# phaistos-networks/Trinity

Hardware: AMD Instinct MI355X
Metric: queries/sec (higher is better)
Workload: dtype u32

## Files before the change

### trinity_amd/csrc/codec_streams.hpp

```cpp
#pragma once
#include "dev_stream.hpp"

constexpr int CODEC_GOOGLE = TRI_CODEC_GOOGLE;
constexpr int CODEC_LUCENE = TRI_CODEC_LUCENE;


__device__ __forceinline__ uint32_t ld32u(const uint8_t *p) {
        const uint32_t *q = (const uint32_t *)((uintptr_t)p & ~(uintptr_t)3);
        return __builtin_amdgcn_alignbyte(q[1], q[0], (uint32_t)((uintptr_t)p & 3u));
}

struct LValStream {
        const uint8_t *wp;
        const uint8_t *epos;
        const uint8_t *ehigh;
        uint64_t win;
        uint32_t width, mask, bitpos, k;
        uint32_t nexc, eb, ecur, next_j, j, sub;
        uint32_t equal_v;
        int mode;
        VbStream vb;

        __device__ __forceinline__ void init_group(const uint8_t *__restrict__ index, const uint32_t group_off, const uint32_t quarter) {
                const uint8_t *g = index + group_off;
                const uint32_t L = g[0];
                j = 0;
                sub = quarter;
                if (!L) {
                        mode = 1;
                        uint32_t len;
                        const uint64_t w = (uint64_t)ld32u(g + 1) | ((uint64_t)ld32u(g + 5) << 32);
                        equal_v = vb_decode(w, len);
                        return;
                }
                mode = 0;
                const uint32_t w0 = ld32u(g + 1);
                width = w0 & 0xffu;
                nexc = (w0 >> 8) & 0xffu;
                eb = (w0 >> 16) & 0xffu;
                mask = width >= 32 ? 0xffffffffu : ((1u << width) - 1u);
                wp = g + 1 + 4 * (1 + quarter * width);
                epos = g + 1 + 4 * (1 + 4 * width);
                ehigh = epos + 4 * ((nexc + 3) / 4);
                bitpos = 0;
                k = 2;
                win = width ? ((uint64_t)ld32u(wp) | ((uint64_t)ld32u(wp + 4) << 32)) : 0;
                ecur = 0;
                while (ecur < nexc && (uint32_t)(epos[ecur] >> 5) < quarter)
                        ++ecur;
                next_j = (ecur < nexc && (uint32_t)(epos[ecur] >> 5) == quarter) ? (epos[ecur] & 31u) : 255u;
        }
        __device__ __forceinline__ void init_tail(const uint8_t *__restrict__ index, const uint32_t off, const bool freqs) {
                mode = freqs ? 3 : 2;
                vb.init(index + off);
        }
        __device__ __forceinline__ uint32_t next() {
                if (mode == 1)
                        return equal_v;
                if (mode == 2) {
                        const uint32_t d = vb.next();
                        (void)vb.next();
                        return d;
                }
                if (mode == 3) {
                        (void)vb.next();
                        return vb.next();
                }
                uint32_t v = 0;
                if (width) {
                        const uint32_t sh = bitpos & 31u;
                        v = (uint32_t)(win >> sh) & mask;
                        const uint32_t nb = bitpos + width;
                        if ((nb >> 5) != (bitpos >> 5)) {
                                win = (win >> 32) | ((uint64_t)ld32u(wp + 4 * k) << 32);
                                ++k;
                        }
                        bitpos = nb;
                }
                if (j == next_j) {
                        const uint32_t eo = ecur * eb;
                        const uint64_t hw = (uint64_t)ld32u(ehigh + 4 * (eo >> 5)) | ((uint64_t)ld32u(ehigh + 4 * (eo >> 5) + 4) << 32);
                        const uint32_t high = (uint32_t)(hw >> (eo & 31u)) & (eb >= 32 ? 0xffffffffu : ((1u << eb) - 1u));
                        v |= width >= 32 ? 0u : (high << width);
                        ++ecur;
                        next_j = (ecur < nexc && (uint32_t)(epos[ecur] >> 5) == sub) ? (epos[ecur] & 31u) : 255u;
                }
                ++j;
                return v;
        }
};

__device__ __forceinline__ uint32_t lucene_group_bytes(const uint8_t *g) {
        const uint32_t L = g[0];
        if (L)
                return 1 + 4 * L;
        const uint32_t b0 = g[1];
        return 1 + (b0 < 0x80 ? 1 : b0 < 0xc0 ? 2 : b0 < 0xe0 ? 3 : b0 < 0xf0 ? 4 : 5);
}

template <int CODEC>
struct DeltaStream;
template <int CODEC>
struct FreqStream;

template <>
struct DeltaStream<CODEC_GOOGLE> {
        VbStream s;
        __device__ __forceinline__ void init(const uint8_t *__restrict__ index, const DevTerm &, const uint32_t, const uint32_t off) { s.init(index + off); }
        __device__ __forceinline__ uint32_t next() { return s.next(); }
};
template <>
struct FreqStream<CODEC_GOOGLE> {
        VbStream s;
        __device__ __forceinline__ void init(const uint8_t *__restrict__, const DevTerm &, const uint32_t, const uint32_t, const DeltaStream<CODEC_GOOGLE> &after_deltas) {
                s = after_deltas.s;
        }
        __device__ __forceinline__ uint32_t next() { return s.next(); }
};

template <>
struct DeltaStream<CODEC_LUCENE> {
        LValStream s;
        __device__ __forceinline__ void init(const uint8_t *__restrict__ index, const DevTerm &t, const uint32_t b, const uint32_t off) {
                if (b < t.npfor)
                        s.init_group(index, off, b & 3u);
                else
                        s.init_tail(index, off, false);
        }
        __device__ __forceinline__ uint32_t next() { return s.next(); }
};
template <>
struct FreqStream<CODEC_LUCENE> {
        LValStream s;
        __device__ __forceinline__ void init(const uint8_t *__restrict__ index, const DevTerm &t, const uint32_t b, const uint32_t off, const DeltaStream<CODEC_LUCENE> &) {
                if (b < t.npfor)
                        s.init_group(index, off + lucene_group_bytes(index + off), b & 3u);
                else
                        s.init_tail(index, off, true);
        }
        __device__ __forceinline__ uint32_t next() { return s.next(); }
};
```

### trinity_amd/csrc/dev_structs.hpp

```cpp
#pragma once
#include <cstdint>
#ifdef __HIPCC__
#define TRI_HD __host__ __device__
#else
#define TRI_HD
#endif

struct DevTerm {
        uint32_t documents;
        uint32_t first_block;
        uint32_t nblocks;
        uint32_t last_n;
        uint32_t win_off;
        uint32_t flags;
        uint32_t npfor;
        uint32_t pad;
};
constexpr uint32_t TERM_FULL_BLOCKS = 1u;
constexpr uint32_t TERM_SPARSE = 2u;

#define TRI_BLOCK_N(t, b, index, off) (((t).flags & TERM_FULL_BLOCKS) ? ((b) + 1 == (t).nblocks ? (t).last_n : 32u) : (uint32_t)(index)[(off)-1])
constexpr uint32_t WIN_MIN_BLOCKS = 128;

constexpr uint32_t QT_GROUP = 0x80000000u;
constexpr uint32_t QT_NOT = 0x40000000u;
constexpr uint32_t QT_TERM = 0x3fffffffu;
constexpr uint32_t MAX_QTERMS = 16;
struct DevQuery {
        uint32_t nterms;
        uint32_t term_base;
        uint64_t out_off;
        uint32_t out_cap;
        uint32_t qid;
        uint32_t first_task, ntasks;
        uint32_t score_base, nscore;
        uint32_t phrase_base, nphrases;
        uint32_t fused_idx, form;
};

constexpr uint32_t RESULT_DOCIDS = 0, RESULT_BITMAP = 1;
constexpr uint32_t MAX_PHRASE_TERMS = 16;
struct DevPhrase {
        uint32_t term_base;
        uint32_t nterms;
        double weight;
};

struct DevTask {
        uint32_t slot;
        uint32_t tile_begin;
        uint32_t tile_end;
        uint32_t kind;
        uint64_t out_off;
};
constexpr uint32_t CAND_QUEUES = 8;
constexpr uint32_t CAND_TICKET_STRIDE = 16;
constexpr uint32_t CAND_HEAVY_TILES = 3;
constexpr uint32_t TASK_CAND = 0;
constexpr uint32_t TASK_DENSE = 1;
constexpr uint32_t TASK_FUSED = 2;
constexpr uint32_t TASK_FUSED16 = 3;

constexpr uint32_t TASK_FUSED_GEN = 4;
constexpr uint32_t TASK_PLANES = 5;
constexpr uint32_t TASK_PLANES8 = 6;
constexpr uint32_t TASK_PSET = 7;
constexpr uint32_t TASK_PROBE = 8;
constexpr uint32_t TASK_TREE = 9;
constexpr uint32_t TASK_KINDS = 10;
constexpr uint32_t PSET_INLINE_TERMS = 4;
#ifndef TRI_PSET_TASK_WINDOWS
#define TRI_PSET_TASK_WINDOWS 4
#endif
constexpr uint32_t PSET_TASK_WINDOWS = TRI_PSET_TASK_WINDOWS;
struct DevPsetUnit {
        uint64_t out_off;
        uint32_t w_begin, w_end;
        uint32_t tix;
        uint32_t nterms;
        uint32_t term_base;
        uint32_t first;
        uint32_t tt[PSET_INLINE_TERMS];
        uint32_t row[PSET_INLINE_TERMS];
};
static_assert(sizeof(DevPsetUnit) == 64, "one cache-line half per unit");
constexpr uint32_t PSET_UNIT_FIRST = 1u, PSET_UNIT_BITMAP = 2u;
constexpr uint32_t PSET_UNIT_ROUND_SHIFT = 4, PSET_UNIT_ROUND_MASK = 15u;
constexpr uint32_t PSET_ROUND_DOCS = 16384, PSET_STAGE_DOCS = 1024;
constexpr uint32_t PSET_UNIT_SCATTER = 4u;
constexpr uint32_t TREE_MAX_NODES = 64;
constexpr uint32_t TREE_HDR_WORDS = 8;
constexpr uint32_t TREE_CHUNK_WORDS = 2048;
constexpr uint32_t TREE_ROW_PHRASE = 0x80000000u;
struct DevTreeNode {
        uint8_t op;
        uint8_t parent;
        uint8_t ord;
        uint8_t thr;
        uint32_t arg;
        uint32_t row;
        uint32_t score;
        uint32_t rmask;
        uint8_t kid0, kid1, pad0, pad1;
        uint64_t kids;
};
static_assert(sizeof(DevTreeNode) == 32, "eight words per node");
constexpr uint32_t TREE_WIDE_MAX_NODES = 1024;
constexpr uint32_t TREE_WIDE_STACK = 64;
constexpr uint32_t TREE_KIND_WIDE = 1;
constexpr uint32_t TREE_NO_PARENT = 0xffffu;
struct DevTreeNodeW {
        uint8_t op;
        uint8_t cbits;
        uint16_t parent;
        uint32_t arg, row, score, rmask;
        uint16_t ord;
        uint16_t nkids;
        uint16_t thr;
        uint8_t pop;
        uint8_t pcbits;
        uint32_t pad;
};
static_assert(sizeof(DevTreeNodeW) == sizeof(DevTreeNode), "a wide record's nodes are eight words each too");
constexpr uint32_t RICH_NARROW_TERMS = 16, RICH_WIDE_TERMS = 64;
struct DevRichWide {
        uint64_t cells;
        uint64_t slots;
        uint32_t stride, pad;
};
static_assert(sizeof(DevRichWide) == 24, "three 8-byte words per plan slot");
TRI_HD constexpr uint32_t tree_counter_planes(const uint32_t nkids) {
        uint32_t b = 0;
        while ((1u << b) <= nkids)
                ++b;
        return b;
}
TRI_HD constexpr bool task_onepass(const uint32_t kind) { return kind >= TASK_FUSED && kind <= TASK_PLANES8; }

constexpr uint32_t PL_W = 32768;
constexpr uint32_t PL_WORDS = PL_W / 32;
constexpr uint32_t PL_NONE = 0xffffffffu;
constexpr uint32_t PL_NESTED = 6;
constexpr uint32_t PL_LEVEL_WORDS = 3;
constexpr uint32_t PL_STORED = 4;
constexpr uint32_t PL_PLANES = PL_STORED + PL_LEVEL_WORDS;
constexpr uint32_t PL_HI = PL_PLANES - 1;
constexpr uint32_t PL_HI_LEVELS = PL_STORED - 1;
constexpr uint32_t PL_RANK_WORDS = 16;
constexpr uint32_t PL_RANK_DOCS = 256;
constexpr uint32_t BLK_HITS_PLAIN = 0x80000000u;
constexpr int TILE_BLOCKS = 256;
constexpr int TILE_CANDS = TILE_BLOCKS * 32;
constexpr uint32_t SPAN_BITS = 1u << 17;
constexpr uint32_t SPAN_WORDS = SPAN_BITS / 32;
constexpr uint32_t CELL_LOG2 = 10;
constexpr uint32_t CELL_DOCS = 1u << CELL_LOG2;
constexpr uint32_t CELLS_PER_SPAN = SPAN_BITS / CELL_DOCS;
#ifndef TRI_FUS_CELLS
#define TRI_FUS_CELLS 14
#endif
constexpr uint32_t FUS_CELLS = TRI_FUS_CELLS;
constexpr uint32_t FUS_W = FUS_CELLS * CELL_DOCS;
constexpr uint32_t PLK_MAX_SPARSE = 6;
constexpr uint32_t PLK_NS_SMALL = 5;
constexpr uint32_t TOPK_MAX = 256;
constexpr uint32_t FUS_MAX_SLOTS = 8;
constexpr uint32_t FUS_MAX_LEAVES = 16;
struct DevFused {
        uint32_t nslots;
        uint32_t fbits;
        uint32_t cap;
        uint32_t nreq;
        uint32_t term[FUS_MAX_SLOTS];
        uint32_t gmask[FUS_MAX_SLOTS];
        uint32_t gslots[FUS_MAX_SLOTS];
        uint32_t nmask;
        uint32_t hw;
        uint32_t mode;
        uint32_t nleaf;
        uint32_t tt[8];
        uint8_t leaf_slot[FUS_MAX_LEAVES];
        uint32_t ctt[FUS_MAX_LEAVES][8];
        uint32_t plane[FUS_MAX_SLOTS];
        uint32_t negslots;
};
constexpr uint32_t FUS_MODE_TT = 1;
constexpr uint32_t FUS_MODE_EMIT = 2;
```

### trinity_amd/csrc/host/plan_host.cpp

```cpp
#include "../planner.hpp"
#include "../lucene_enc_units.hpp"
#include "lucene_encoder.hpp"

#include <cstdlib>
#include <memory>
#include <mutex>

namespace {
        struct HostPlan {
                BatchPlan P;
                uint8_t *block = nullptr;
                ~HostPlan() { free(block); }
        };
        void put_err(char *err, size_t cap, const std::string &s) {
                if (err && cap) {
                        const size_t n = std::min(cap - 1, s.size());
                        memcpy(err, s.data(), n);
                        err[n] = 0;
                }
        }
}

extern "C" {
void *tri_host_index_build(const uint8_t *index, uint64_t len, const uint8_t *hits, uint64_t hits_len, int codec, const uint32_t *terms3, uint64_t nterms,
                           uint32_t docs_cnt, char *err, uint64_t errcap) {
        auto H = std::make_unique<HostIndex>();
        std::string e;
        static_assert(sizeof(tri_term) == 12, "tri_term is three u32");
        if (build_host_index(index, len, hits, hits_len, codec, reinterpret_cast<const tri_term *>(terms3), nterms, docs_cnt, *H, e) != TRI_OK) {
                put_err(err, errcap, e);
                return nullptr;
        }
        return H.release();
}
void tri_host_index_free(void *h) { delete static_cast<HostIndex *>(h); }

void *tri_host_plan(void *hindex, const uint32_t *prog, uint64_t prog_len, const uint32_t *queries2, uint64_t nq, uint32_t flags, uint32_t topk, int similarity,
                    unsigned threads, const char *const *opt_names, const uint64_t *opt_values, unsigned nopt, uint32_t cus, char *err, uint64_t errcap) {
        const HostIndex &H = *static_cast<HostIndex *>(hindex);
        PlanEnv env;
        env.cus = cus ? cus : 256;
        bool use_frag_cache = false;
        for (unsigned i = 0; i < nopt; ++i) {
                const std::string n = opt_names[i];
                if (n == "frag_cache") {
                        use_frag_cache = opt_values[i] != 0;
                        continue;
                }
                tri_options &o = env.opt;
                uint64_t *slot = n == "dense_min_postings" ? &o.dense_min_postings : n == "dense_task_cost" ? &o.dense_task_cost : n == "fused" ? &o.fused
                                 : n == "fused_task_cost" ? &o.fused_task_cost : n == "fused_freq_cap" ? &o.fused_freq_cap : n == "fused_halfwords" ? &o.fused_halfwords
                                 : n == "account_needed_bytes" ? &o.account_needed_bytes : n == "planes" ? &o.planes : n == "planes_split" ? &o.planes_split
                                 : n == "plane_div" ? &o.plane_div : n == "plane_max_bytes" ? &o.plane_max_bytes : n == "probe_max_blocks" ? &o.probe_max_blocks : n == "tree_max_bytes" ? &o.tree_max_bytes : n == "tree_max_nodes" ? &o.tree_max_nodes : n == "tree_wide_min_nodes" ? &o.tree_wide_min_nodes : n == "result_bitmaps" ? &o.result_bitmaps : n == "cand_task_cost" ? &o.cand_task_cost : n == "dense_window_cost" ? &o.dense_window_cost
                                 : n == "cand_xcd" ? &o.cand_xcd : n == "planes_order" ? &o.planes_order : n == "pset_order" ? &o.pset_order : n == "scatter_bitmap_slack" ? &o.scatter_bitmap_slack : n == "phrase_task_div" ? &o.phrase_task_div : n == "plane_amortize" ? &o.plane_amortize : n == "rich_max_terms" ? &o.rich_max_terms : nullptr;
                if (!slot) {
                        put_err(err, errcap, "unknown option " + n);
                        return nullptr;
                }
                *slot = opt_values[i];
        }
        PlanInput in;
        in.prog = prog;
        in.prog_len = prog_len;
        static_assert(sizeof(tri_query) == 8, "tri_query is two u32");
        in.queries = reinterpret_cast<const tri_query *>(queries2);
        in.nq = nq;
        in.flags = flags;
        in.topk = topk;
        in.similarity = similarity;
        auto hp = std::make_unique<HostPlan>();
        std::unique_ptr<HostPool> pool;
        if (threads > 1)
                pool = std::make_unique<HostPool>(threads);
        std::string e;
        static trip::FragCache g_frag_cache;
        static std::mutex g_frag_mu;
        std::unique_lock<std::mutex> frag_lock(g_frag_mu, std::defer_lock);
        if (use_frag_cache)
                frag_lock.lock();
        const int rc = plan_batch(
                H, env, in, pool.get(),
                [&](size_t bytes) {
                        hp->block = static_cast<uint8_t *>(aligned_alloc(64, (bytes + 63) & ~(size_t)63));
                        if (hp->block)
                                memset(hp->block, 0, bytes);
                        return hp->block;
                },
                hp->P, e, use_frag_cache ? &g_frag_cache : nullptr);
        if (rc != TRI_OK) {
                put_err(err, errcap, e);
                return nullptr;
        }
        return hp.release();
}
void tri_host_plan_free(void *p) { delete static_cast<HostPlan *>(p); }

void tri_host_plan_summary(void *p, uint64_t *out , double *ms ) {
        const BatchPlan &P = static_cast<HostPlan *>(p)->P;
        const uint64_t v[] = {P.block_bytes,       P.plan.size(),    P.qterms.size(),      P.tasks.size(),  P.fused.size(),       P.qplane.size(),    P.plane_terms.size(), P.sterms.size(),
                              P.sweights.size(),   P.phrases.size(), P.pterms.size(),      P.ptasks.size(), P.plan.off,           P.qterms.off,       P.tasks.off,          P.sched.off,
                              P.fused.off,         P.qplane.off,     P.plane_terms.off,    P.sterms.off,    P.sweights.off,       P.phrases.off,      P.pterms.off,         P.ptasks.off,
                              P.n_dense,           P.n_cand,         P.n_fused,            P.n_fused16,     P.n_fusedgen,         P.n_planes,         P.n_planes8,          P.plw,
                              P.sparse_cap,        P.out_capacity,   P.term_bytes,         P.term_bytes_dense, P.dense_queries,   P.cand_queries,     P.fused_queries,      P.planes_queries,
                              P.unsupported_queries, P.rich_R,       sizeof(DevQuery),     sizeof(DevTask), sizeof(DevFused),     sizeof(DevPhrase),  P.cand_needed_term_bytes, P.plane_decoded_bytes,
                              P.n_pset,            P.pset_queries,   P.n_probe,            P.probe_queries, P.units.size(),       P.units.off,        P.pset_sched.off,     sizeof(DevPsetUnit),
                              P.n_tree,            P.tree_queries,   P.tree.size(),        P.tree.off,      P.tree_terms.size(),  P.tree_terms.off,   P.tree_hidden.size(), P.tree_hidden.off,
                              P.cand_q.off};
        static_assert(sizeof v / sizeof v[0] == 65, "summary layout");
        memcpy(out, v, sizeof v);
        if (ms)
                memcpy(ms, P.plan_ms, sizeof P.plan_ms);
}
void tri_host_plan_rich_wide(void *p, uint64_t *out ) {
        const BatchPlan &P = static_cast<HostPlan *>(p)->P;
        const uint64_t v[] = {P.rich_wide.size(), P.rich_wide.off, P.rich_sched.off, P.n_rich_wide, P.rich_wide_cells, P.rich_wide_slots, sizeof(DevRichWide)};
        memcpy(out, v, sizeof v);
}
void tri_host_plan_last_unsupported(void *p, char *out, uint64_t cap) { put_err(out, cap, static_cast<HostPlan *>(p)->P.last_unsupported); }
const uint8_t *tri_host_plan_block(void *p) { return static_cast<HostPlan *>(p)->P.block; }
void tri_host_plan_query_maps(void *p, uint32_t *slot_of_query, int32_t *qstatus) {
        const BatchPlan &P = static_cast<HostPlan *>(p)->P;
        memcpy(slot_of_query, P.slot_of_query.data(), P.slot_of_query.size() * 4);
        memcpy(qstatus, P.qstatus.data(), P.qstatus.size() * 4);
}
}

extern "C" {
int tri_host_lucene_encode(const uint32_t *docs, const uint32_t *freqs, const uint16_t *pos, const uint64_t *term_first, uint64_t nterms, uint8_t *index_out, uint64_t icap,
                           uint64_t *ilen, uint8_t *hits_out, uint64_t hcap, uint64_t *hlen, uint32_t *terms3) {
        using namespace trinity_amd::Codecs;
        Lucene::IndexSession sess;
        Lucene::Encoder enc(&sess);
        uint64_t h = 0;
        for (uint64_t t = 0; t < nterms; ++t) {
                enc.begin_term();
                for (uint64_t p = term_first[t]; p < term_first[t + 1]; ++p) {
                        enc.begin_document(docs[p]);
                        for (uint32_t i = 0; i < freqs[p]; ++i)
                                enc.new_hit(pos[h++]);
                        enc.end_document();
                }
                trinity_amd::term_index_ctx tctx;
                enc.end_term(&tctx);
                terms3[3 * t] = tctx.documents, terms3[3 * t + 1] = tctx.offset, terms3[3 * t + 2] = tctx.size;
        }
        *ilen = sess.indexOut.size(), *hlen = sess.positionsOut.size();
        if (*ilen > icap || *hlen > hcap)
                return -1;
        if (*ilen)
                memcpy(index_out, sess.indexOut.data(), *ilen);
        if (*hlen)
                memcpy(hits_out, sess.positionsOut.data(), *hlen);
        return 0;
}
int tri_host_lucene_encode_units(const uint32_t *docs, const uint32_t *freqs, const uint16_t *pos, const uint64_t *term_first, uint64_t nterms, uint8_t *index_out, uint64_t icap,
                                 uint64_t *ilen, uint8_t *hits_out, uint64_t hcap, uint64_t *hlen, uint32_t *terms3) {
        const uint64_t np = term_first[nterms];
        std::vector<uint64_t> hit_off(np + 1, 0), dblk_first(nterms + 1, 0), hblk_first(nterms + 1, 0);
        for (uint64_t p = 0; p < np; ++p)
                hit_off[p + 1] = hit_off[p] + freqs[p];
        for (uint64_t t = 0; t < nterms; ++t) {
                dblk_first[t + 1] = dblk_first[t] + (term_first[t + 1] - term_first[t]) / LENC_BLOCK;
                hblk_first[t + 1] = hblk_first[t] + (hit_off[term_first[t + 1]] - hit_off[term_first[t]]) / LENC_BLOCK;
        }
        std::vector<uint32_t> hdelta(hit_off[np] + 1);
        LencArgs a{docs, freqs, pos, hit_off.data(), term_first, hdelta.data(), dblk_first.data(), hblk_first.data(), nterms};
        for (uint64_t p = 0; p < np; ++p)
                lenc_unit_hdelta(a, p, hdelta.data());
        const uint64_t nd = dblk_first[nterms], nh = hblk_first[nterms];
        std::vector<uint64_t> doff(nd + 1, 0), hoff(nh + 1, 0), term_off(nterms + 1, 0), hterm_off(nterms + 1, 0);
        std::vector<uint32_t> tail_d(nterms + 1), tail_h(nterms + 1);
        for (uint64_t g = 0; g < nd; ++g)
                doff[g + 1] = doff[g] + lenc_unit_dblk_size(a, g);
        for (uint64_t h = 0; h < nh; ++h)
                hoff[h + 1] = hoff[h] + lenc_unit_hblk_size(a, h);
        for (uint64_t t = 0; t < nterms; ++t)
                lenc_unit_tail_size(a, t, &tail_d[t], &tail_h[t]);
        LencPlace pl{doff.data(), hoff.data(), term_off.data(), hterm_off.data(), tail_d.data(), tail_h.data()};
        for (uint64_t t = 0; t < nterms; ++t) {
                term_off[t + 1] = term_off[t] + lenc_term_index_size(a, pl, t);
                hterm_off[t + 1] = hterm_off[t] + lenc_term_hits_size(a, pl, t);
        }
        *ilen = term_off[nterms], *hlen = hterm_off[nterms];
        if (*ilen > icap || *hlen > hcap)
                return -1;
        for (uint64_t g = 0; g < nd; ++g)
                lenc_unit_dblk_write(a, pl, g, index_out);
        for (uint64_t h = 0; h < nh; ++h)
                lenc_unit_hblk_write(a, pl, h, hits_out);
        for (uint64_t t = 0; t < nterms; ++t) {
                lenc_unit_term_write(a, pl, t, index_out, hits_out);
                terms3[3 * t] = (uint32_t)(term_first[t + 1] - term_first[t]), terms3[3 * t + 1] = (uint32_t)term_off[t], terms3[3 * t + 2] = lenc_term_index_size(a, pl, t);
        }
        return 0;
}
}

extern "C" {
void tri_host_pfor128_group(const uint32_t *v, uint8_t *a, uint32_t *alen, uint8_t *b, uint32_t *blen) {
        auto get = [&](uint32_t i) { return v[i]; };
        const Pfor128Plan p = pfor128_plan(get);
        uint8_t *e = pfor128_emit(get, p, a);
        *alen = (uint32_t)(e - a);
        if ((uint32_t)(e - a) != p.bytes)
                *alen = 0xffffffffu;
        std::vector<uint8_t> o;
        trinity_amd::Codecs::Lucene::ints_encode(v, o);
        memcpy(b, o.data(), o.size());
        *blen = (uint32_t)o.size();
}
uint32_t tri_host_fastpfor_encode(const uint32_t *v, uint32_t *out) {
        std::vector<uint32_t> w;
        trif::fastpfor_encode(v, w);
        memcpy(out, w.data(), w.size() * 4);
        return (uint32_t)w.size();
}
int tri_host_fastpfor_decode(const uint32_t *w, uint32_t L, uint32_t *v) { return trif::fastpfor_decode(w, L, v) ? 1 : 0; }
uint32_t tri_host_pool_cpus(uint32_t threads, int32_t *out, uint32_t cap) {
        HostPool pool(threads);
        const std::vector<int> &c = pool.pinned_cpus();
        for (size_t i = 0; i < c.size() && i < cap; ++i)
                out[i] = c[i];
        return (uint32_t)c.size();
}

uint32_t tri_host_cpu_budget() { return host_cpu_budget(); }

void tri_host_index_facts(void *h, uint64_t *info6, uint32_t *per_term3) {
        const HostIndex &H = *static_cast<HostIndex *>(h);
        info6[0] = H.info.postings, info6[1] = H.info.blocks, info6[2] = H.info.doc_bytes, info6[3] = H.info.hit_bytes, info6[4] = H.transcoded_groups, info6[5] = H.dev_index.size();
        for (size_t t = 0; t < H.terms.size(); ++t) {
                per_term3[3 * t] = H.terms[t].documents;
                per_term3[3 * t + 1] = H.terms[t].nblocks;
                per_term3[3 * t + 2] = H.terms[t].nblocks ? H.blk_last[H.terms[t].first_block + H.terms[t].nblocks - 1] : 0;
        }
}
}
```

### trinity_amd/csrc/k_match.hpp

```cpp
#pragma once
#include "codec_streams.hpp"

constexpr int AND_WG = 256;
constexpr int DENSE_WG = 512;
static_assert(TILE_BLOCKS == AND_WG, "the candidate kernel maps one 32-candidate row to each of its 256 lanes");

__device__ __forceinline__ uint32_t uni(uint32_t v) { return (uint32_t)__builtin_amdgcn_readfirstlane((int)v); }
#include "k_filter.hpp"

__device__ __forceinline__ uint32_t phys(uint32_t j) { return (j & ~31u) | ((j + (j >> 5)) & 31u); }

__device__ __forceinline__ uint32_t wave_excl_scan(uint32_t v, uint32_t &total) {
        uint32_t x = v;
        asm volatile("s_nop 1\n\t"
                     "v_add_u32_dpp %0, %0, %0 row_shr:1 row_mask:0xf bank_mask:0xf bound_ctrl:1\n\t"
                     "s_nop 1\n\t"
                     "v_add_u32_dpp %0, %0, %0 row_shr:2 row_mask:0xf bank_mask:0xf bound_ctrl:1\n\t"
                     "s_nop 1\n\t"
                     "v_add_u32_dpp %0, %0, %0 row_shr:4 row_mask:0xf bank_mask:0xf bound_ctrl:1\n\t"
                     "s_nop 1\n\t"
                     "v_add_u32_dpp %0, %0, %0 row_shr:8 row_mask:0xf bank_mask:0xf bound_ctrl:1\n\t"
                     "s_nop 1\n\t"
                     "v_add_u32_dpp %0, %0, %0 row_bcast:15 row_mask:0xa bank_mask:0xf\n\t"
                     "s_nop 1\n\t"
// ... 37 lines not shown
        uint32_t seg_tt[MAX_QTERMS];
        uint32_t seg_wlo[MAX_QTERMS];
        uint32_t seg_whi[MAX_QTERMS];
        uint32_t seg_plane[MAX_QTERMS];
        uint32_t nslow;
};
constexpr uint32_t DENSE_SLOW_CAP = DENSE_WG / 4;

template <int WG = AND_WG>
__device__ uint32_t wg_lower_bound(uint32_t *scan, const uint32_t *__restrict__ a, const uint32_t n, const uint32_t key) {
        const uint32_t tid = threadIdx.x;
        uint32_t lo = 0, hi = n;
        while (hi > lo) {
                const uint32_t len = hi - lo;
                const uint32_t step = (len + WG - 1) / WG;
                const uint32_t pos = lo + (tid + 1) * step - 1;
                const bool ge = pos >= hi ? true : a[pos] >= key;
                const uint64_t m = __ballot(ge);
                scan[tid >> 6] = m ? (tid & ~63u) + (uint32_t)__builtin_ctzll(m) : 0xffffffffu;
                __syncthreads();
                uint32_t first = 0xffffffffu;
#pragma unroll
                for (int wv = 0; wv < WG / 64; ++wv)
                        first = min(first, scan[wv]);
                first = uni(first);
                __syncthreads();
                if (first == 0xffffffffu)
                        return hi;
                const uint32_t nlo = lo + first * step;
                const uint32_t nhi = min(hi, lo + (first + 1) * step - 1);
                lo = nlo;
                hi = step == 1 ? nlo : nhi;
        }
        return lo;
}

typedef uint32_t u32x4_a4 __attribute__((ext_vector_type(4), aligned(4)));
__device__ __forceinline__ void block_bytes32_issue(const uint8_t *__restrict__ p, uint32_t (&r)[9]) {
        const uint8_t *q = p - ((uintptr_t)p & 3u);
        const u32x4_a4 A = *(const u32x4_a4 *)q, B = *(const u32x4_a4 *)(q + 16);
        r[0] = A.x, r[1] = A.y, r[2] = A.z, r[3] = A.w, r[4] = B.x, r[5] = B.y, r[6] = B.z, r[7] = B.w;
        r[8] = *(const uint32_t *)(q + 32);
}
__device__ __forceinline__ bool block_bytes32_finish(const uint8_t *__restrict__ p, const uint32_t (&r)[9], uint32_t (&v)[8]) {
        const uint32_t sk = (uint32_t)((uintptr_t)p & 3u);
#pragma unroll
        for (int i = 0; i < 8; ++i)
                v[i] = __builtin_amdgcn_alignbyte(r[i + 1], r[i], sk);
        return ((v[0] | v[1] | v[2] | v[3] | v[4] | v[5] | v[6] | (v[7] & 0x00ffffffu)) & 0x80808080u) == 0;
}
__device__ __forceinline__ bool load_block_bytes32(const uint8_t *__restrict__ p, uint32_t (&v)[8]) {
        uint32_t r[9];
        block_bytes32_issue(p, r);
        return block_bytes32_finish(p, r, v);
}

__device__ __forceinline__ uint32_t cand_gallop(const AndShared &sh, uint32_t ptr, const uint32_t C, const uint32_t doc) {
        uint32_t step = 1, lo = ptr;
        while (lo + step <= C && sh.cand[phys(lo + step - 1)] < doc) {
                lo += step;
                step <<= 1;
        }
        uint32_t hi = min(lo + step - 1, C);
        while (lo < hi) {
                const uint32_t mid = (lo + hi) >> 1;
                if (sh.cand[phys(mid)] < doc)
                        lo = mid + 1;
                else
                        hi = mid;
        }
        return lo;
}

template <int CODEC, bool PRE>
__device__ __forceinline__ void merge_block(AndShared &sh, const uint8_t *__restrict__ index, const DevTerm &t, const uint32_t b, const uint32_t off,
                                            const uint32_t n, const uint32_t prev, const uint32_t last, uint32_t ptr, uint32_t cv, const uint32_t C,
                                            const uint32_t (&raw)[9]) {
        uint32_t doc = prev;
        uint32_t v[8];
        if (CODEC == CODEC_GOOGLE && n == 32 && (PRE ? block_bytes32_finish(index + off, raw, v) : load_block_bytes32(index + off, v))) {
                uint32_t c[8];
#pragma unroll
                for (int i = 0; i < 8; ++i)
                        c[i] = ptr + i < C ? sh.cand[phys(ptr + i)] : 0xffffffffu;
                if (c[7] > last) {
                        uint32_t at = ptr;
#pragma unroll
                        for (int j = 0; j < 32; ++j) {
                                doc = j < 31 ? doc + ((v[j >> 2] >> ((j & 3) * 8)) & 0xffu) : last;
                                while (c[0] <= doc) {
                                        if (c[0] == doc)
                                                atomicOr(&sh.hit[at >> 5], 1u << (at & 31));
                                        ++at;
#pragma unroll
                                        for (int i = 0; i < 7; ++i)
                                                c[i] = c[i + 1];
                                        c[7] = 0xffffffffu;
                                }
                                if (c[0] > last)
                                        return;
                        }
                        return;
                }
#pragma unroll
                for (int j = 0; j < 32; ++j) {
                        doc = j < 31 ? doc + ((v[j >> 2] >> ((j & 3) * 8)) & 0xffu) : last;
                        if (cv <= doc) {
                                if (cv == doc)
                                        atomicOr(&sh.hit[ptr >> 5], 1u << (ptr & 31));
                                ptr = cand_gallop(sh, ptr + 1, C, doc);
                                cv = ptr < C ? sh.cand[phys(ptr)] : 0xffffffffu;
                                if (cv == doc)
                                        atomicOr(&sh.hit[ptr >> 5], 1u << (ptr & 31));
                                if (cv > last)
                                        return;
                        }
                }
                return;
        }
        DeltaStream<CODEC> s;
        s.init(index, t, b, off);
        for (uint32_t i = 0; i < n; ++i) {
                doc = (i + 1 < n) ? doc + s.next() : last;
                if (cv < doc) {
                        ptr = cand_gallop(sh, ptr + 1, C, doc);
                        cv = ptr < C ? sh.cand[phys(ptr)] : 0xffffffffu;
                }
                if (cv == doc)
                        atomicOr(&sh.hit[ptr >> 5], 1u << (ptr & 31));
                if (cv > last)
                        break;
        }
}

__device__ __forceinline__ uint32_t wave_lower_bound(const uint32_t *__restrict__ a, uint32_t lo, uint32_t hi, const uint32_t key) {
        const uint32_t lane = threadIdx.x & 63u;
        while (hi > lo) {
                const uint32_t len = hi - lo;
                const uint32_t step = (len + 63u) / 64u;
                const uint32_t pos = lo + (lane + 1) * step - 1;
                const bool ge = pos >= hi ? true : a[pos] >= key;
                const uint64_t m = __ballot(ge);
                if (m == 0)
                        return hi;
                const uint32_t first = (uint32_t)__builtin_ctzll(m);
                const uint32_t nlo = lo + first * step;
                const uint32_t nhi = min(hi, lo + (first + 1) * step - 1);
                lo = nlo;
                hi = step == 1 ? nlo : nhi;
        }
        return lo;
}

template <int CODEC>
__device__ void and_filter_tile(AndShared &sh, const uint8_t *__restrict__ index, const uint32_t *__restrict__ blk_last,
                                const uint32_t *__restrict__ blk_off, const uint32_t *__restrict__ win, const DevTerm t, const uint32_t C,
                                const uint32_t lcur_slot, const bool block_driven PROF_ARG) {
        const uint32_t tid = threadIdx.x;
        const uint32_t *bl = blk_last + t.first_block;
        const uint32_t *bo = blk_off + t.first_block;
        const uint32_t cmin = sh.cand[phys(0)], cmax = sh.cand[phys(C - 1)];

        if (block_driven) {
                uint32_t lcur = uni(sh.lcur[lcur_slot]);
                if (lcur == 0xffffffffu)
                        lcur = wg_lower_bound(sh.scan, bl, t.nblocks, cmin);
                for (;;) {
                        const uint32_t b = lcur + tid;
                        const bool below = b < t.nblocks && bl[b] < cmin;
                        const uint64_t m = __ballot(below);
                        const uint32_t lead = m == ~0ull ? 64u : (uint32_t)__builtin_ctzll(~m);
                        sh.scan[tid >> 6] = lead;
                        __syncthreads();
                        uint32_t adv = 0;
                        for (int w = 0; w < AND_WG / 64; ++w) {
                                adv += sh.scan[w];
                                if (sh.scan[w] != 64)
                                        break;
                        }
                        adv = uni(adv);
                        __syncthreads();
                        lcur += adv;
                        if (adv != AND_WG || lcur >= t.nblocks)
                                break;
                }
                sh.lcur[lcur_slot] = lcur;
                PROF_LAP(5);
                TRACE(10, lcur, t.nblocks);
                uint32_t nprev = 0, nlast = 0, noff = 0;
                {
                        const uint32_t b = lcur + tid;
                        if (b < t.nblocks) {
                                nprev = b ? bl[b - 1] : 0;
                                nlast = bl[b];
                                noff = bo[b];
                        }
                }
                for (uint32_t cb = lcur; cb < t.nblocks; cb += AND_WG) {
                        TRACE(11, cb, t.nblocks);
                        const uint32_t b = cb + tid;
                        bool beyond = true;
                        const uint32_t prev = nprev, last = nlast, off = noff;
                        uint32_t raw[9];
                        const bool full = CODEC == CODEC_GOOGLE && b < t.nblocks && prev < cmax && TRI_BLOCK_N(t, b, index, off) == 32;
                        if (full)
                                block_bytes32_issue(index + off, raw);
                        {
                                const uint32_t b2 = b + AND_WG;
                                if (b2 < t.nblocks) {
                                        nprev = bl[b2 - 1];
                                        nlast = bl[b2];
                                        noff = bo[b2];
                                }
                        }
                        if (b < t.nblocks) {
                                beyond = last >= cmax;
                                if (prev < cmax) {
                                        uint32_t lo = 0, hi = C;
                                        while (lo < hi) {
                                                const uint32_t mid = (lo + hi) >> 1;
                                                if (sh.cand[phys(mid)] <= prev)
                                                        lo = mid + 1;
                                                else
                                                        hi = mid;
                                        }
                                        uint32_t ptr = lo;
                                        uint32_t cv = ptr < C ? sh.cand[phys(ptr)] : 0xffffffffu;
                                        PROF_LAP(6);
                                        if (cv <= last) {
                                                if (full)
                                                        merge_block<CODEC, true>(sh, index, t, b, off, 32, prev, last, ptr, cv, C, raw);
                                                else
                                                        merge_block<CODEC, false>(sh, index, t, b, off, TRI_BLOCK_N(t, b, index, off), prev, last, ptr, cv, C, raw);
                                        }
                                        PROF_LAP(7);
                                }
                        }
                        sh.scan[4 + (tid >> 6)] = __ballot(beyond) != 0ull;
                        __syncthreads();
                        const uint32_t any_beyond = uni(sh.scan[4] | sh.scan[5] | sh.scan[6] | sh.scan[7]);
                        __syncthreads();
                        PROF_LAP(8);
                        if (any_beyond)
                                break;
                }
        } else {
                uint32_t carry = 0xffffffffu;
                uint32_t wcur = 0;
                for (uint32_t base = 0; base < C; base += AND_WG) {
                        TRACE(20, base, C);
                        const uint32_t j = base + tid;
                        uint32_t bj = 0xffffffffu;
                        uint32_t cv = 0;
                        const uint32_t wbase = base + (tid & ~63u);
                        uint32_t rlo = 0, rhi = 0;
                        if (t.win_off != 0xffffffffu) {
                                if (j < C) {
                                        const uint32_t c = sh.cand[phys(j)] >> CELL_LOG2;
                                        rlo = win[t.win_off + c];
                                        rhi = win[t.win_off + c + 1];
                                }
                        } else if (wbase < C) {
                                const uint32_t nval = min(64u, C - wbase);
                                const uint32_t klo = sh.cand[phys(wbase)], khi = sh.cand[phys(wbase + nval - 1)];
                                rlo = wave_lower_bound(bl, wcur, t.nblocks, klo);
                                rhi = wave_lower_bound(bl, rlo, t.nblocks, khi);
                                wcur = rlo;
                        }
                        if (j < C) {
                                cv = sh.cand[phys(j)];
                                uint32_t lo = rlo, hi = rhi;
                                while (lo < hi) {
                                        const uint32_t mid = (lo + hi) >> 1;
                                        if (bl[mid] < cv)
                                                lo = mid + 1;
                                        else
                                                hi = mid;
                                }
                                bj = lo;
                        }
                        uint32_t prevb = __shfl_up(bj, 1, 64);
                        if ((tid & 63u) == 0)
                                prevb = carry;
                        carry = __shfl(bj, 63, 64);
                        if (j < C && bj < t.nblocks && bj != prevb) {
                                const uint32_t prev = bj ? bl[bj - 1] : 0;
                                const uint32_t none[9] = {};
                                merge_block<CODEC, false>(sh, index, t, bj, bo[bj], TRI_BLOCK_N(t, bj, index, bo[bj]), prev, bl[bj], j, cv, C, none);
                        }
                }
        }
}

__device__ __forceinline__ void dense_visit(uint32_t *bm, const uint32_t rel) {
        uint32_t w, r, a;
        asm("v_lshrrev_b32 %0, 5, %1" : "=v"(w) : "v"(rel));
        asm("v_lshrrev_b32 %0, 10, %1" : "=v"(r) : "v"(rel));
        asm("v_add_lshl_u32 %0, %1, %2, 2" : "=v"(a) : "v"(w), "v"(r));
        atomicOr((uint32_t *)((uint8_t *)bm + a), 1u << (rel & 31u));
}
__device__ __forceinline__ void dense_visit_clamped(uint32_t *bm, const uint32_t rel, const uint32_t wbase) {
        atomicOr(&bm[bm_pad(min(rel >> 5, SPAN_WORDS) + wbase)], 1u << (rel & 31u));
}

template <int CODEC>
__device__ __forceinline__ void dense_block_stream(const uint8_t *__restrict__ index, const DevTerm &t, const uint32_t b, const uint32_t off,
                                                   const uint32_t n, const uint32_t prev, const uint32_t last, const uint32_t w0, uint32_t *bm,
// ... 404 lines not shown
                                        cur = uni(sh.seg_wlo[k]);
                                        here = cur != uni(sh.seg_whi[k]);
                                } else {
                                        cur = uni(sh.lcur[k]);
                                        if (cur < uni(t.nblocks) && bl[cur] < w * SPAN_BITS)
                                                cur = uni(wave_lower_bound(bl, cur, t.nblocks, w * SPAN_BITS));
                                        sh.lcur[k] = cur;
                                }
                                if (here)
                                        wnext = w;
                                else if (cur < uni(t.nblocks)) {
                                        const uint32_t first_possible = cur ? bl[cur - 1] + 1 : 1;
                                        wnext = min(wnext, max(w, first_possible / SPAN_BITS));
                                }
                        }
                        wnext = uni(wnext);
                        __syncthreads();
                        if (wnext == w || wnext >= task.tile_end) {
                                w = wnext;
                                break;
                        }
                        w = wnext;
                }
                if (w >= task.tile_end)
                        break;
                const uint32_t w0 = w * SPAN_BITS;
                const uint32_t wlast = w0 + (SPAN_BITS - 1);
                uint32_t ngroups = 0, g1 = q.nterms, g2 = q.nterms;
                bool galive = false, neg = false;
                for (uint32_t k = 0; k < q.nterms; ++k) {
                        const uint32_t tt = uni(sh.seg_tt[k]);
                        const DevTerm t = sh.seg_term[k];
                        const uint32_t nblocks = uni(t.nblocks);
                        const uint32_t *bl = blk_last + t.first_block;
                        if (tt & QT_GROUP) {
                                if (k && !galive)
                                        done = true;
                                if (ngroups == 1)
                                        g1 = k;
                                else if (ngroups == 2)
                                        g2 = k;
                                ++ngroups;
                                galive = false;
                                neg = tt & QT_NOT;
                        }
                        uint32_t b_lo, b_hi;
                        if (uni(sh.seg_plane[k]) != PL_NONE) {
                                galive = true;
                                sh.seg_lo[k] = 0;
                                sh.seg_cnt[k] = 0;
                                continue;
                        }
                        if (uni(t.win_off) != 0xffffffffu) {
                                b_lo = uni(sh.seg_wlo[k]);
                                b_hi = min(uni(sh.seg_whi[k]), nblocks - 1);
                        } else {
                                b_lo = uni(sh.lcur[k]);
                                if (b_lo < nblocks && bl[b_lo] < w0)
                                        b_lo = uni(wave_lower_bound(bl, b_lo, nblocks, w0));
                                b_hi = b_lo;
                                if (b_lo < nblocks) {
                                        b_hi = uni(wave_lower_bound(bl, b_lo, nblocks, wlast));
                                        if (b_hi >= nblocks)
                                                b_hi = nblocks - 1;
                                }
                        }
                        if (b_lo < nblocks)
                                galive = true;
                        sh.seg_lo[k] = b_lo;
                        sh.seg_cnt[k] = b_lo < nblocks ? b_hi - b_lo + 1 : 0;
                }
                sh.seg_cnt[q.nterms] = 0xffffffffu;
                if (!galive && !neg)
                        done = true;
                if (done)
                        break;
                PROF_LAP(1);
                __syncthreads();
                PROF_LAP(2);
                dense_pass<WG, CODEC>(sh, index, blk_last, blk_off, 0, g2, g1, w0, planes, plw PROF_PASS);
                for (uint32_t kb = g2; kb < q.nterms;) {
                        uint32_t ke = kb + 1;
                        while (ke < q.nterms && !(qterms[q.term_base + ke] & QT_GROUP))
                                ++ke;
                        for (uint32_t i = tid; i < BM_STRIDE; i += WG) {
                                sh.bm[i] &= sh.bm[BM_STRIDE + i];
                                sh.bm[BM_STRIDE + i] = 0;
                        }
                        __syncthreads();
                        dense_pass<WG, CODEC>(sh, index, blk_last, blk_off, kb, ke, kb, w0, planes, plw PROF_PASS);
                        kb = ke;
                }
                if (as_bitmap) {
                        for (; wdone < w; ++wdone)
                                dense_store_zero<WG>(qout + (size_t)(wdone - task.tile_begin) * SPAN_WORDS);
                        produced += dense_store<WG>(sh, w0, ngroups > 1, neg, masked, qout + (size_t)(w - task.tile_begin) * SPAN_WORDS);
                        wdone = w + 1;
                } else
                        produced += dense_expand<WG>(sh, w0, ngroups > 1, neg, masked, qout, produced PROF_PASS);
                ++w;
        }
        if (as_bitmap)
                for (; wdone < task.tile_end; ++wdone)
                        dense_store_zero<WG>(qout + (size_t)(wdone - task.tile_begin) * SPAN_WORDS);
        __syncthreads();
        if (uni(tid >> 6) == 0)
                *count_out = produced;
        PROF_LAP(8);
}

#ifndef TRI_DENSE_WAVES
#define TRI_DENSE_WAVES 8
#endif
template <int CODEC>
__global__ __launch_bounds__(DENSE_WG, TRI_DENSE_WAVES) void k_and_dense(const uint8_t *__restrict__ index, const uint32_t *__restrict__ blk_last,
                                                        const uint32_t *__restrict__ blk_off, const uint32_t *__restrict__ win,
                                                        const DevTerm *__restrict__ terms, const DevQuery *__restrict__ plan,
                                                        const DevTask *__restrict__ tasks, const uint32_t *__restrict__ sched,
                                                        const uint32_t *__restrict__ qterms, const uint32_t ntasks, uint32_t *__restrict__ ticket,
                                                        uint32_t *__restrict__ out, uint32_t *__restrict__ counts,
                                                        const uint32_t *__restrict__ masked, const uint32_t *__restrict__ qplane,
                                                        const uint32_t *__restrict__ planes, const uint32_t plw TRI_FILTER_ARG) {
        __shared__ DenseShared sh;
        const uint32_t wave = uni(threadIdx.x >> 6);
        PROF_DECL;
        PROF_START();
        for (;;) {
                if (wave == 0) {
                        const uint32_t old = atomicAdd(ticket, 1u);
                        sh.bcast[0] = uni(old) >> 6;
                }
                __syncthreads();
                const uint32_t ticket_no = uni(sh.bcast[0]);
                __syncthreads();
                if (ticket_no >= ntasks)
                        break;
                const uint32_t tix = sched[ticket_no];
                const DevTask task = tasks[tix];
                const DevQuery q = plan[task.slot];
                TRI_FILTER_TASK(task.slot);
                PROF_LAP(0);
                TASKTIME_DENSE(8 * ticket_no);
                dense_task<DENSE_WG, CODEC>(sh, index, blk_last, blk_off, win, terms, qterms, q, task, out, counts + tix, masked, qplane, planes, plw PROF_PASS);
                TASKTIME_DENSE(8 * ticket_no + 1);
        }
        PROF_LAP(9);
        PROF_FLUSH();
}

#ifndef TRI_AND_PROBES
#define TRI_AND_PROBES 8
#endif
constexpr int AND_PROBES = TRI_AND_PROBES;
template <int CODEC>
#ifndef TRI_AND_WAVES
#define TRI_AND_WAVES 4
#endif
__global__ __launch_bounds__(AND_WG, TRI_AND_WAVES) void k_and(const uint8_t *__restrict__ index, const uint32_t *__restrict__ blk_last,
                                                const uint32_t *__restrict__ blk_off, const uint32_t *__restrict__ win,
                                                const DevTerm *__restrict__ terms,
                                                const DevQuery *__restrict__ plan, const DevTask *__restrict__ tasks,
                                                const uint32_t *__restrict__ sched, const uint32_t *__restrict__ qterms,
                                                const uint32_t *__restrict__ cand_q, uint32_t *__restrict__ ticket,
                                                uint32_t *__restrict__ out, uint32_t *__restrict__ counts,
                                                const uint32_t *__restrict__ masked, const uint32_t *__restrict__ qplane,
                                                const uint32_t *__restrict__ planes, const uint32_t plw TRI_FILTER_ARG) {
        __shared__ AndShared sh;
        const uint32_t tid = threadIdx.x;
        const uint32_t wave = uni(tid >> 6);
        const uint32_t home = uni(__builtin_amdgcn_s_getreg(20 | (0 << 6) | (3 << 11))) % CAND_QUEUES;
        uint32_t qdone = 0;
        PROF_DECL;
        PROF_START();
        for (;;) {
                if (wave == 0) {
                        uint32_t got = 0xffffffffu;
                        for (uint32_t t = 0; t < CAND_QUEUES && got == 0xffffffffu; ++t) {
                                const uint32_t x = (home + t) % CAND_QUEUES;
                                if ((qdone >> x) & 1u)
                                        continue;
                                const uint32_t q0 = cand_q[x], qn = cand_q[x + 1] - q0;
                                const uint32_t old = uni(atomicAdd(ticket + x * CAND_TICKET_STRIDE, 1u)) >> 6;
                                if (old < qn)
                                        got = q0 + old;
                                else
                                        qdone |= 1u << x;
                        }
                        sh.bcast[0] = got;
                }
                __syncthreads();
                const uint32_t ticket_no = uni(sh.bcast[0]);
                __syncthreads();
                if (ticket_no == 0xffffffffu)
                        break;
                const uint32_t tix = sched[ticket_no];
                TASKTIME(8 * ticket_no);
                const DevTask task = tasks[tix];
                const uint32_t slot = task.slot;
                const DevQuery q = plan[slot];
                TRI_FILTER_TASK(slot);
                const DevTerm lead = terms[qterms[q.term_base] & QT_TERM];
                TRACE(1, slot, q.nterms);
                uint32_t *qout = out + task.out_off;
                uint32_t produced = 0;
                sh.lcur[tid & 15] = 0xffffffffu;
                const uint32_t tb_end = min(lead.nblocks, task.tile_end * TILE_BLOCKS);
                PROF_LAP(10);

                for (uint32_t tb = task.tile_begin * TILE_BLOCKS; tb < tb_end; tb += TILE_BLOCKS) {
                        const uint32_t nb = min((uint32_t)TILE_BLOCKS, lead.nblocks - tb);
                        uint32_t C = (tb + nb == lead.nblocks) ? (nb - 1) * 32 + lead.last_n : nb * 32;
                        if (tid < nb) {
                                const uint32_t b = tb + tid, gb = lead.first_block + b;
                                const uint32_t off = blk_off[gb];
                                const uint32_t n = TRI_BLOCK_N(lead, b, index, off);
                                const uint32_t last = blk_last[gb];
                                uint32_t doc = b ? blk_last[gb - 1] : 0;
#if defined(TRI_AND_EXP) && TRI_AND_EXP == 2
                                const uint32_t row = tid * 32, step = (last - doc) / 32u + 1u;
                                for (uint32_t i = 0; i + 1 < n; ++i) {
                                        doc += step;
                                        sh.cand[row | ((i + tid) & 31u)] = min(doc, last);
                                }
                                sh.cand[row | ((n - 1 + tid) & 31u)] = last;
                                (void)off;
#else
                                DeltaStream<CODEC> s;
                                s.init(index, lead, b, off);
                                const uint32_t row = tid * 32;
                                for (uint32_t i = 0; i + 1 < n; ++i) {
                                        doc += s.next();
                                        sh.cand[row | ((i + tid) & 31u)] = doc;
                                }
                                sh.cand[row | ((n - 1 + tid) & 31u)] = last;
#endif
                        }
                        __syncthreads();
                        PROF_LAP(11);
                        TASKTIME(8 * ticket_no + 2);
                        TRACE(2, slot, tb);

                        bool gneg = false;
                        for (uint32_t k = 1; k < q.nterms && C; ++k) {
                                const uint32_t tt = qterms[q.term_base + k];
                                const DevTerm t = terms[tt & QT_TERM];
                                if (tt & QT_GROUP) {
                                        sh.hit[tid] = 0;
                                        gneg = tt & QT_NOT;
                                }
                                __syncthreads();
#if defined(TRI_FORCE_CAND)
                                const bool bd = false;
#elif defined(TRI_FORCE_BLOCK)
                                const bool bd = true;
#else
                                const bool bd = t.nblocks <= lead.documents;
#endif
                                TRACE(3, slot, (k << 16) | (bd ? 1 : 0));
                                const uint32_t prow = qplane ? qplane[q.term_base + k] : PL_NONE;
                                if (prow != PL_NONE) {
                                        const uint32_t *pa = planes + (size_t)prow * plw;
                                        for (uint32_t j0 = tid; j0 < C; j0 += AND_WG * AND_PROBES) {
                                                uint32_t doc[AND_PROBES], w[AND_PROBES];
#pragma unroll
                                                for (int u = 0; u < AND_PROBES; ++u) {
                                                        const uint32_t j = j0 + u * AND_WG;
                                                        doc[u] = j < C ? sh.cand[phys(j)] : 0u;
                                                }
#pragma unroll
                                                for (int u = 0; u < AND_PROBES; ++u)
#if defined(TRI_AND_EXP) && TRI_AND_EXP == 1
                                                        w[u] = pa[(doc[u] >> 5) & 0x3ffu];
#else
                                                        w[u] = pa[doc[u] >> 5];
#endif
#pragma unroll
                                                for (int u = 0; u < AND_PROBES; ++u) {
                                                        const uint32_t j = j0 + u * AND_WG;
                                                        if (j < C && ((w[u] >> (doc[u] & 31u)) & 1u))
                                                                atomicOr(&sh.hit[j >> 5], 1u << (j & 31u));
                                                }
                                        }
                                } else
                                and_filter_tile<CODEC>(sh, index, blk_last, blk_off, win, t, C, k - 1, bd PROF_PASS);
                                TRACE(4, slot, C);
                                __syncthreads();
                                TASKTIME(8 * ticket_no + 2 + min(k, 5u));
                                PROF_LAP(bd ? 12 : 13);
                                const bool lastterm = k + 1 == q.nterms;
                                if (!lastterm && !(qterms[q.term_base + k + 1] & QT_GROUP))
                                        continue;
                                uint32_t bits = sh.hit[tid];
                                if (gneg) {
                                        const uint32_t left = C > tid * 32 ? C - tid * 32 : 0u;
                                        bits = ~bits & (left >= 32 ? 0xffffffffu : ((1u << left) - 1u));
                                }
                                if (masked && lastterm)
                                        for (uint32_t m = bits; m;) {
                                                const uint32_t kbit = __builtin_ctz(m);
                                                m &= m - 1;
                                                const uint32_t doc = sh.cand[phys(tid * 32 + kbit)];
                                                if ((masked[doc >> 5] >> (doc & 31u)) & 1u)
                                                        bits &= ~(1u << kbit);
                                        }
                                const uint32_t cnt = __popc(bits);
                                uint32_t wtot;
                                uint32_t ex = wave_excl_scan(cnt, wtot);
                                sh.scan[tid >> 6] = wtot;
                                __syncthreads();
                                uint32_t wbase = 0, total = 0;
                                for (int w = 0; w < AND_WG / 64; ++w) {
                                        if (w < (int)(tid >> 6))
                                                wbase += sh.scan[w];
                                        total += sh.scan[w];
                                }
                                ex += wbase;
                                if (lastterm) {
                                        uint32_t m = bits, o = produced + ex;
                                        while (m) {
                                                const uint32_t kbit = __builtin_ctz(m);
                                                m &= m - 1;
                                                qout[o++] = sh.cand[phys(tid * 32 + kbit)];
                                        }
                                } else {
                                        uint32_t vals[32];
#pragma unroll
                                        for (int kk = 0; kk < 32; ++kk)
                                                vals[kk] = sh.cand[(tid * 32) | ((kk + tid) & 31u)];
                                        __syncthreads();
                                        uint32_t o = ex;
#pragma unroll
                                        for (int kk = 0; kk < 32; ++kk)
                                                if ((bits >> kk) & 1u) {
                                                        sh.cand[phys(o)] = vals[kk];
                                                        ++o;
                                                }
                                }
                                C = uni(total);
                                __syncthreads();
                        }
                        if (q.nterms == 1) {
                                if (!masked) {
                                        for (uint32_t j = tid; j < C; j += AND_WG)
                                                qout[produced + j] = sh.cand[phys(j)];
                                } else {
                                        const uint32_t left = C > tid * 32 ? C - tid * 32 : 0u;
                                        uint32_t bits = left >= 32 ? 0xffffffffu : ((1u << left) - 1u);
                                        for (uint32_t m = bits; m;) {
                                                const uint32_t kbit = __builtin_ctz(m);
                                                m &= m - 1;
                                                const uint32_t doc = sh.cand[phys(tid * 32 + kbit)];
                                                if ((masked[doc >> 5] >> (doc & 31u)) & 1u)
                                                        bits &= ~(1u << kbit);
                                        }
                                        uint32_t wtot;
                                        uint32_t ex = wave_excl_scan(__popc(bits), wtot);
                                        sh.scan[tid >> 6] = wtot;
                                        __syncthreads();
                                        uint32_t wbase = 0, total = 0;
                                        for (int w = 0; w < AND_WG / 64; ++w) {
                                                if (w < (int)(tid >> 6))
                                                        wbase += sh.scan[w];
                                                total += sh.scan[w];
                                        }
                                        uint32_t o = produced + ex + wbase;
                                        for (uint32_t m = bits; m;) {
                                                const uint32_t kbit = __builtin_ctz(m);
                                                m &= m - 1;
                                                qout[o++] = sh.cand[phys(tid * 32 + kbit)];
                                        }
                                        C = uni(total);
                                }
                        }
                        produced += C;
                        __syncthreads();
                        PROF_LAP(14);
                }
                if (wave == 0)
                        counts[tix] = produced;
                TASKTIME(8 * ticket_no + 1);
                TRACE(5, slot, produced);
        }
        PROF_LAP(15);
        PROF_FLUSH();
        TRACE(6, 0, 0);
}
```

### trinity_amd/csrc/planner.hpp

```cpp
#pragma once
#include "planner_lower.hpp"
#include "planner_tasks.hpp"

namespace trip {
        struct RowQ {
                uint8_t n = 0, q[CAND_QUEUES] = {}, sub[CAND_QUEUES] = {};
        };
        struct LapTimer {
                const bool on;
                std::chrono::steady_clock::time_point t0 = std::chrono::steady_clock::now();
                std::string line;
                void lap(const char *what) {
                        if (!on)
                                return;
                        char buf[64];
                        snprintf(buf, sizeof buf, " %s %.3f", what, ms_since(t0));
                        line += buf;
                }
        };

        struct PlanState {
                const HostIndex &ix;
                const PlanEnv &env;
                const tri_options &opt;
                HostPool *pool;
                BatchPlan &P;
                std::string &err;
                Ctx C;
                LapTimer dbg;
                FragCache *cache = nullptr;
                std::vector<Frag> frags;
                SectionCounts n;
                uint64_t cand_queries_all = 0;
                std::vector<uint64_t> benefit, cand_row;
                std::vector<uint32_t> tree_terms;
                std::vector<uint32_t> chosen;
                std::vector<uint32_t> row_of_rank;
                bool cand_rows = false;
                std::vector<RowQ> rowq;
                uint32_t pset_ranges = 0;
                uint32_t cand_first = 0, cand_qat[CAND_QUEUES] = {};
                std::vector<uint32_t> unit_of_task;
                ~PlanState() {
                        if (!cache)
                                return;
                        if (cache->frags.size() < frags.size())
                                cache->frags.resize(frags.size());
                        for (size_t k = 0; k < frags.size(); ++k)
                                cache->frags[k] = std::move(frags[k]);
                }
                template <class Fn>
                void run(Fn &&fn) {
                        if (pool && frags.size() > 1)
                                pool->run((unsigned)frags.size(), fn);
                        else
                                for (unsigned k = 0; k < frags.size(); ++k)
                                        fn(k);
                }
                int first_error() {
                        for (Frag &f : frags)
                                if (f.rc != TRI_OK) {
                                        err = f.err;
                                        return f.rc;
                                }
                        return TRI_OK;
                }
                template <class Fn>
                int run_pass(const char *name, const char *doing, Fn &&fn) {
                        run([&](unsigned k) {
                                Frag &f = frags[k];
                                try {
                                        f.rc = fn(f);
                                } catch (const std::bad_alloc &) {
                                        f.rc = herr(f.err, TRI_ERR_NOMEM, "tri_batch_create: out of host memory while %s", doing);
                                } catch (...) {
                                        f.rc = herr(f.err, TRI_ERR_INVALID, "tri_batch_create: unexpected exception while %s", doing);
                                }
                        });
                        dbg.lap(name);
                        return first_error();
                }
        };

        inline void eligible_planes(PlanState &S) {
                const HostIndex &ix = S.ix;
                const tri_options &opt = S.opt;
                S.P.plw = ((ix.max_doc >> 17) + 2u) * (SPAN_BITS / 32u);
                S.C.plw = S.P.plw;
                if (opt.planes && opt.plane_div && !ix.df_sorted.empty()) {
                        const uint64_t min_df = std::max<uint64_t>(1, ix.info.docs_cnt / opt.plane_div);
                        const size_t n = (size_t)(std::partition_point(ix.df_sorted.begin(), ix.df_sorted.end(), [&](uint32_t d) { return d && d >= min_df; }) - ix.df_sorted.begin());
                        const uint64_t row_bytes = (uint64_t)PL_PLANES * S.P.plw * 4;
                        S.C.n_ok = (uint32_t)std::min<uint64_t>(n, std::max<uint64_t>(1, opt.plane_max_bytes / std::max<uint64_t>(1, row_bytes)));
                }
        }

        inline void take_fragments(PlanState &S, FragCache *cache) {
                const size_t nq = S.C.in.nq;
                const unsigned nthreads = S.pool ? std::min<unsigned>(S.pool->size(), (unsigned)std::max<size_t>(1, nq / 512)) : 1u;
                const size_t nfrag = nthreads <= 1 ? 1 : std::min<size_t>(2 * nthreads, std::max<size_t>(1, nq / 256));
                S.frags.resize(nfrag);
                S.cache = cache;
                for (size_t k = 0; k < nfrag; ++k) {
                        if (cache && k < cache->frags.size()) {
                                S.frags[k] = std::move(cache->frags[k]);
                                S.frags[k].recycle();
                        }
                        S.frags[k].q_lo = nq * k / nfrag;
                        S.frags[k].q_hi = nq * (k + 1) / nfrag;
                }
        }

        inline void settle_batch_knobs(PlanState &S) {
                const tri_options &opt = S.opt;
                const PlanEnv &env = S.env;
                Ctx &C = S.C;
                uint64_t onepass_queries = 0, fused_postings = 0, phrase_queries = 0;
                for (const Frag &f : S.frags) {
                        onepass_queries += f.onepass_queries;
                        fused_postings += f.fused_postings;
                        phrase_queries += f.phrase_queries;
                }
                C.phrase_task_div = opt.phrase_task_div ? opt.phrase_task_div : !phrase_queries ? 1 : phrase_queries <= 8ull * env.cus ? 4 : phrase_queries <= 16ull * env.cus ? 2 : 1;
                C.planes_split = opt.planes_split ? opt.planes_split : (2 * onepass_queries >= 4ull * (uint64_t)env.cus * env.plk_wgs_per_cu ? 2 : 3) ;
                C.fused_task_cost = opt.fused_task_cost;
                if (!C.fused_task_cost) {
                        const uint64_t want_tasks = 2ull * (uint64_t)env.cus * env.fus_wgs_per_cu;
                        C.fused_task_cost = std::min<uint64_t>(8u << 20, std::max<uint64_t>(256u << 10, fused_postings / std::max<uint64_t>(1, want_tasks)));
                }
        }

        inline int place_fragments(PlanState &S) {
                BatchPlan &P = S.P;
                SectionCounts &n = S.n;
                const uint32_t n_ok = S.C.n_ok;
                uint64_t off = 0;
                S.benefit.assign(n_ok, 0), S.cand_row.assign(n_ok, 0);
                for (Frag &f : S.frags) {
                        f.b_plan = n.plan, f.b_qterms = n.qterms, f.b_sterms = n.sterms, f.b_phrases = n.phrases, f.b_pterms = n.pterms, f.b_tasks = n.tasks, f.b_fused = n.fused,
                        f.b_ptasks = n.ptasks, f.b_off = off, f.b_units = n.units, f.b_tree = n.tree, f.b_hidden = n.tree_hidden;
                        n.plan += f.tmp.size(), n.qterms += f.qterms.size(), n.sterms += f.sterms.size(), n.phrases += f.phrases.size(), n.pterms += f.pterms.size(),
                                n.tasks += f.tasks.size(), n.fused += f.fused.size(), n.ptasks += f.ptasks.size(), n.units += f.units.size(), n.tree += f.treepool.size(),
                                n.tree_hidden += f.n_hidden, off += f.off;
                        S.tree_terms.insert(S.tree_terms.end(), f.tree_terms.begin(), f.tree_terms.end());
                        P.merge(f);
                        for (uint32_t r = 0; r < n_ok; ++r)
                                S.benefit[r] += f.benefit[r], S.cand_row[r] += f.cand_row[r];
                        for (const size_t qi : f.left_out) {
                                P.qstatus[qi] = TRI_ERR_UNSUPPORTED;
                                ++P.unsupported_queries;
                        }
                        if (!f.left_out.empty())
                                P.last_unsupported = f.err;
                }
                S.cand_queries_all = P.cand_queries + P.probe_queries;
                if (n.qterms > 0xfffffff0ull || n.sterms > 0xfffffff0ull || n.tasks > 0xfffffff0ull || n.pterms > 0xfffffff0ull)
                        return herr(S.err, TRI_ERR_UNSUPPORTED, "tri_batch_create: the batch exceeds 2^32 terms or tasks: split it");
                P.out_capacity = off;
                if (P.rich_wide_queries)
                        n.rich_wide = n.plan, n.rich_sched = n.tasks;
                std::sort(S.tree_terms.begin(), S.tree_terms.end());
                S.tree_terms.erase(std::unique(S.tree_terms.begin(), S.tree_terms.end()), S.tree_terms.end());
                n.tree_terms = S.tree_terms.size();
                P.tree_scratch_bytes = ((uint64_t)n.tree_terms * PL_PLANES + n.tree_hidden + P.tree_queries) * P.plw * 4;
                if (P.tree_scratch_bytes > S.opt.tree_max_bytes)
                        return herr(S.err, TRI_ERR_NOMEM, "tri_batch_create: the batch's %llu tree queries need %llu bytes of bitmap scratch (%zu distinct term leaves, %zu phrase leaves; option tree_max_bytes = %llu): split the batch",
                                    (unsigned long long)P.tree_queries, (unsigned long long)P.tree_scratch_bytes, n.tree_terms, n.tree_hidden, (unsigned long long)S.opt.tree_max_bytes);
                return TRI_OK;
        }

        inline void choose_planes(PlanState &S) {
                const HostIndex &ix = S.ix;
                const uint32_t n_ok = S.C.n_ok;
                std::vector<uint32_t> rank_term(n_ok, UINT32_MAX);
                std::vector<uint8_t> forced(n_ok, 0);
                for (const Frag &f : S.frags) {
                        for (const QUse &u : f.quses)
                                rank_term[ix.df_rank[u.term]] = u.term;
                        for (const QUse &u : f.suses)
                                rank_term[ix.df_rank[u.term]] = u.term;
                        for (const FUse &u : f.fuses)
                                rank_term[ix.df_rank[u.term]] = u.term, forced[ix.df_rank[u.term]] = 1;
                }
                for (uint32_t r = 0; r < n_ok; ++r)
                        if (rank_term[r] != UINT32_MAX && (forced[r] || S.benefit[r] * std::max<uint64_t>(1, S.opt.plane_amortize) >= ix.terms[rank_term[r]].documents))
                                S.chosen.push_back(rank_term[r]);
                std::sort(S.chosen.begin(), S.chosen.end());
                S.row_of_rank.assign(n_ok, PL_NONE);
                for (const uint32_t term : S.chosen) {
                        S.row_of_rank[ix.df_rank[term]] = ix.df_rank[term];
                        S.P.plane_decoded_bytes += ix.docbytes[term];
                }
                S.P.plane_rows = n_ok;
                S.n.plane_terms = S.chosen.size();
                S.n.qplane = S.chosen.empty() ? 0 : S.n.qterms;
                S.n.splane = (S.chosen.empty() || !S.C.scored) ? 0 : S.n.sterms;
                S.n.sweights = S.C.scored ? S.n.sterms : 0;
        }

        inline void assign_cand_rows(PlanState &S) {
                const BatchPlan &P = S.P;
                const uint32_t n_ok = S.C.n_ok;
                const std::vector<uint64_t> &cand_row = S.cand_row;
                S.pset_ranges = ((S.ix.max_doc >> 17) + 1u + PSET_TASK_WINDOWS - 1) / PSET_TASK_WINDOWS;
                S.cand_rows = S.opt.cand_xcd && !S.chosen.empty() && S.cand_queries_all && P.cand_lead_docs >= CAND_ROWS_MIN_LEAD * S.cand_queries_all && P.cand_terms <= 3 * S.cand_queries_all;
                S.rowq.assign(S.cand_rows ? n_ok : 0, RowQ{});
                if (S.cand_rows) {
                        uint64_t total = 0, load[CAND_QUEUES] = {};
                        uint32_t placed[CAND_QUEUES] = {};
                        std::vector<uint32_t> rows;
                        for (uint32_t r = 0; r < n_ok; ++r)
                                if (cand_row[r] && S.row_of_rank[r] != PL_NONE)
                                        rows.push_back(r), total += cand_row[r];
                        std::sort(rows.begin(), rows.end(), [&](uint32_t a, uint32_t b) { return cand_row[a] != cand_row[b] ? cand_row[a] > cand_row[b] : a < b; });
                        const uint64_t cap = std::max<uint64_t>(1, total / (2 * CAND_QUEUES));
                        for (const uint32_t r : rows) {
                                RowQ &z = S.rowq[r];
                                z.n = (uint8_t)std::min<uint64_t>(CAND_QUEUES, (cand_row[r] + cap - 1) / cap);
                                for (uint32_t k = 0; k < z.n; ++k) {
                                        const uint32_t x = (uint32_t)(std::min_element(load, load + CAND_QUEUES) - load);
                                        load[x] += cand_row[r] / z.n;
                                        z.q[k] = (uint8_t)x;
                                        z.sub[k] = (uint8_t)(CAND_COST_SUBS + placed[x]++ % (CAND_SUBS - CAND_COST_SUBS - 1));
                                }
                        }
                }
                if (S.dbg.on) {
                        char buf[96];
                        snprintf(buf, sizeof buf, " [cand queries %llu lead docs %llu terms %llu rows %d]", (unsigned long long)S.cand_queries_all, (unsigned long long)P.cand_lead_docs, (unsigned long long)P.cand_terms, (int)S.cand_rows);
                        S.dbg.line += buf;
                }
        }

        inline int layout_block(PlanState &S, const std::function<uint8_t *(size_t)> &alloc_block) {
                BatchPlan &P = S.P;
                P.block_bytes = layout_sections(P, S.n);
                S.dbg.lap("sums+planes+layout");
                P.block = alloc_block(P.block_bytes);
                S.dbg.lap("alloc_block");
                if (!P.block)
                        return herr(S.err, TRI_ERR_NOMEM, "tri_batch_create: no host memory for the plan (%zu bytes)", P.block_bytes);
                point_sections(P, S.n);
                std::copy(S.tree_terms.begin(), S.tree_terms.end(), P.tree_terms.p);
                S.unit_of_task.assign(S.n.units ? S.n.tasks : 0, 0u);
                std::copy(S.chosen.begin(), S.chosen.end(), P.plane_terms.p);
                S.dbg.lap("spans");
                return TRI_OK;
        }

        inline int fill_fragment(PlanState &S, Frag &f) {
                const HostIndex &ix = S.ix;
                BatchPlan &P = S.P;
                const std::vector<uint32_t> &row_of_rank = S.row_of_rank;
                for (size_t i = 0; i < f.tmp.size(); ++i) {
                        DevQuery q = f.tmp[i].q;
                        q.term_base += (uint32_t)f.b_qterms;
                        q.score_base += (uint32_t)f.b_sterms;
                        q.phrase_base += (uint32_t)f.b_phrases;
                        q.first_task += (uint32_t)f.b_tasks;
                        q.out_off += f.b_off;
                        if (f.tmp[i].fuse)
                                q.fused_idx += (uint32_t)f.b_fused;
                        if (f.tmp[i].tree)
                                q.fused_idx += (uint32_t)f.b_tree;
                        if (f.tmp[i].hidden) {
                                q.qid = 0xffffffffu;
                                P.tree_hidden[f.b_hidden + f.tmp[i].hidden_ord] = (uint32_t)(f.b_plan + i);
                        } else
                                P.slot_of_query[q.qid] = (uint32_t)(f.b_plan + i);
                        P.plan[f.b_plan + i] = q;
                }
                if (!f.treepool.empty()) {
                        memcpy(&P.tree[f.b_tree], f.treepool.data(), f.treepool.size() * 4);
                        for (size_t i = 0; i < f.tmp.size(); ++i) {
                                if (!f.tmp[i].tree)
                                        continue;
                                uint32_t *rec = &P.tree[f.b_tree + f.tmp[i].q.fused_idx];
                                DevTreeNode *tn = reinterpret_cast<DevTreeNode *>(rec + TREE_HDR_WORDS);
                                for (uint32_t k = 0; k < rec[0]; ++k)
                                        if (tn[k].op == TRI_OP_TERM)
                                                tn[k].row = (uint32_t)(std::lower_bound(P.tree_terms.begin(), P.tree_terms.end(), tn[k].arg) - P.tree_terms.begin());
                                        else if (tn[k].op == TRI_OP_PHRASE) {
                                                tn[k].arg += (uint32_t)f.b_plan;
                                                tn[k].row += (uint32_t)f.b_hidden;
                                        }
                        }
                }
                for (size_t i = 0; i < f.tasks.size(); ++i) {
                        DevTask t = f.tasks[i];
                        t.slot += (uint32_t)f.b_plan;
                        t.out_off += f.b_off;
                        P.tasks[f.b_tasks + i] = t;
                }
                if (!f.qterms.empty())
                        memcpy(&P.qterms[f.b_qterms], f.qterms.data(), f.qterms.size() * 4);
                if (!f.sterms.empty())
                        memcpy(&P.sterms[f.b_sterms], f.sterms.data(), f.sterms.size() * 4);
                if (S.C.scored && !f.sweights.empty())
                        memcpy(&P.sweights[f.b_sterms], f.sweights.data(), f.sweights.size() * 8);
                for (size_t i = 0; i < f.phrases.size(); ++i) {
                        DevPhrase ph = f.phrases[i];
                        ph.term_base += (uint32_t)f.b_pterms;
                        P.phrases[f.b_phrases + i] = ph;
                }
                if (!f.pterms.empty())
                        memcpy(&P.pterms[f.b_pterms], f.pterms.data(), f.pterms.size() * 4);
                for (size_t i = 0; i < f.ptasks.size(); ++i)
                        P.ptasks[f.b_ptasks + i] = f.ptasks[i] + (uint32_t)f.b_tasks;
                for (size_t i = 0; i < f.fused.size(); ++i)
                        P.fused[f.b_fused + i] = f.fused[i];
                for (const FUse &u : f.fuses)
                        P.fused[f.b_fused + u.fidx].plane[u.slot] = row_of_rank[ix.df_rank[u.term]];
                for (size_t i = 0; i < f.units.size(); ++i) {
                        DevPsetUnit u = f.units[i];
                        u.out_off += f.b_off;
                        u.tix += (uint32_t)f.b_tasks;
                        u.term_base += (uint32_t)f.b_qterms;
                        const bool is_probe = f.tasks[f.units[i].tix].kind == TASK_PROBE;
                        bool rows = true;
                        for (uint32_t k = is_probe ? 1u : 0u; k < u.nterms; ++k) {
                                const uint32_t term = (k < PSET_INLINE_TERMS ? u.tt[k] : f.qterms[f.units[i].term_base + k]) & QT_TERM;
                                const uint32_t rank = ix.df_rank[term];
                                const uint32_t row = rank < row_of_rank.size() ? row_of_rank[rank] : PL_NONE;
                                rows &= row != PL_NONE;
                                if (k < PSET_INLINE_TERMS)
                                        u.row[k] = row;
                                if (row == PL_NONE && (u.first & PSET_UNIT_SCATTER) && u.w_begin == 0)
                                        f.pscatter_docs += ix.terms[term].documents;
                        }
                        if (is_probe && !rows) {
                                P.tasks[u.tix].kind = TASK_CAND;
                                if (u.first & PSET_UNIT_FIRST) {
                                        ++f.probe_demoted;
                                        f.probe_demoted_bytes += distinct_docbytes(ix, &f.qterms[f.units[i].term_base], u.nterms, f.S.seen);
                                }
                        }
                        P.units[f.b_units + i] = u;
                        S.unit_of_task[u.tix] = (uint32_t)(f.b_units + i);
                }
                if (S.n.splane) {
                        std::fill(&P.splane.p[f.b_sterms], &P.splane.p[f.b_sterms] + f.sterms.size(), PL_NONE);
                        for (const QUse &u : f.suses)
                                P.splane[f.b_sterms + u.qpos] = row_of_rank[ix.df_rank[u.term]];
                }
                if (S.n.qplane) {
                        std::fill(&P.qplane.p[f.b_qterms], &P.qplane.p[f.b_qterms] + f.qterms.size(), PL_NONE);
                        for (const QUse &u : f.quses)
                                P.qplane[f.b_qterms + u.qpos] = row_of_rank[ix.df_rank[u.term]];
                }
                return TRI_OK;
        }

        inline uint32_t key_planes_order(const PlanState &S, const Frag &f, const size_t i, const DevTask &tk) {
                const DevQuery &q = S.P.plan[tk.slot];
                const DevFused &z = S.P.fused[q.fused_idx];
                uint32_t minrow = PL_NONE;
                for (uint32_t sidx = 0; sidx < z.nslots; ++sidx)
                        minrow = std::min(minrow, z.plane[sidx]);
                const uint32_t ord = (uint32_t)(f.b_tasks + i) - q.first_task, per = SCHED_NB / 4;
                return SCHED_RANK[tk.kind] * SCHED_NB + (S.opt.planes_order == 2 ? std::min(minrow, per - 1) * 4 + std::min(ord, 3u) : std::min(ord, 3u) * per + std::min(minrow, per - 1));
        }
        inline uint32_t key_pset_order(const PlanState &S, const Frag &f, const size_t i) {
                const uint32_t range = (uint32_t)(f.tcost[i] & 0xffffffffull) / PSET_TASK_WINDOWS;
                const uint32_t rb = S.pset_ranges <= PSET_RANGE_BKS ? std::min(range, PSET_RANGE_BKS - 1) : (uint32_t)std::min<uint64_t>((uint64_t)range * PSET_RANGE_BKS / S.pset_ranges, PSET_RANGE_BKS - 1);
                return PSET_KEY0 + rb * PSET_SUBS + pset_sub((uint32_t)(f.tcost[i] >> 32));
        }
        inline uint32_t key_cand_rows(const PlanState &S, const Frag &f, const size_t i, const DevTask &tk) {
                const DevQuery &q = S.P.plan[tk.slot];
                uint32_t row = PL_NONE;
                for (uint32_t k = 1; k < q.nterms && row == PL_NONE; ++k)
                        row = S.P.qplane[q.term_base + k];
                uint32_t queue, sub;
                if (tk.tile_end - tk.tile_begin > CAND_HEAVY_TILES || row == PL_NONE)
                        queue = (uint32_t)(f.b_tasks + i) % CAND_QUEUES, sub = (sched_key(TASK_CAND, f.tcost[i]) % SCHED_NB) / (SCHED_NB / CAND_COST_SUBS);
                else if (row < S.rowq.size() && S.rowq[row].n) {
                        const RowQ &z = S.rowq[row];
                        const uint32_t piece = (uint32_t)(f.b_tasks + i) % z.n;
                        queue = z.q[piece], sub = z.sub[piece];
                } else
                        queue = row % CAND_QUEUES, sub = CAND_SUBS - 1;
                return CAND_KEY0 + queue * CAND_SUBS + sub;
        }
        inline uint32_t schedule_key(const PlanState &S, const Frag &f, const size_t i) {
                const DevTask &tk = S.P.tasks[f.b_tasks + i];
                switch (tk.kind) {
                        case TASK_PLANES:
                        case TASK_PLANES8:
                                if (S.opt.planes_order)
                                        return key_planes_order(S, f, i, tk);
                                break;
                        case TASK_PSET:
                                if (S.opt.pset_order)
                                        return key_pset_order(S, f, i);
                                break;
                        case TASK_CAND:
                                if (S.cand_rows)
                                        return key_cand_rows(S, f, i, tk);
                                break;
                }
                return sched_key(tk.kind, f.tcost[i]);
        }
        inline int key_fragment(const PlanState &S, Frag &f) {
                f.keys.resize(f.tasks.size());
                f.hist.assign(SCHED_KEYS, 0u);
                for (size_t i = 0; i < f.tasks.size(); ++i)
                        ++f.hist[f.keys[i] = schedule_key(S, f, i)];
                return TRI_OK;
        }

        inline void place_schedule(PlanState &S) {
                BatchPlan &P = S.P;
                uint32_t at = 0;
                for (uint32_t r = 0; r < TASK_KINDS; ++r) {
                        const uint32_t before = at;
                        if (r == SCHED_RANK[TASK_CAND])
                                S.cand_first = at;
                        auto place = [&](const uint32_t bk) {
                                for (Frag &f : S.frags) {
                                        const uint32_t c = f.hist[bk];
                                        f.hist[bk] = at;
                                        at += c;
                                }
                        };
                        for (uint32_t bk = r * SCHED_NB; bk < (r + 1) * SCHED_NB; ++bk)
                                place(bk);
                        if (r == SCHED_RANK[TASK_PSET] && S.opt.pset_order)
                                for (uint32_t bk = PSET_KEY0; bk < PSET_KEY0 + std::min(S.pset_ranges, PSET_RANGE_BKS) * PSET_SUBS; ++bk)
                                        place(bk);
                        if (r == SCHED_RANK[TASK_CAND])
                                for (uint32_t bk = CAND_KEY0; bk < PSET_KEY0; ++bk) {
                                        if ((bk - CAND_KEY0) % CAND_SUBS == 0)
                                                S.cand_qat[(bk - CAND_KEY0) / CAND_SUBS] = at;
                                        place(bk);
                                }
                        for (uint32_t k = 0; k < TASK_KINDS; ++k)
                                if (SCHED_RANK[k] == r)
                                        P.*SCHED_COUNT[k] = at - before;
                }
                const uint32_t units_first = sched_first(P, TASK_PSET), n_units_run = P.n_pset + P.n_probe;
                S.run([&](unsigned k) {
                        Frag &f = S.frags[k];
                        for (size_t i = 0; i < f.tasks.size(); ++i) {
                                const uint32_t pos = f.hist[f.keys[i]]++, ti = (uint32_t)(f.b_tasks + i);
                                P.sched[pos] = ti;
                                if (pos >= units_first && pos - units_first < n_units_run)
                                        P.pset_sched[pos - units_first] = S.unit_of_task[ti];
                        }
                });
        }

        inline void split_tree_section(BatchPlan &P) {
                if (!P.n_tree)
                        return;
                uint32_t *const ts = P.sched.p + sched_first(P, TASK_TREE);
                auto narrow = [&](const uint32_t ti) { return P.tree[P.plan[P.tasks[ti].slot].fused_idx + 1] != TREE_KIND_WIDE; };
                P.n_tree_wide = P.n_tree - (uint32_t)std::count_if(ts, ts + P.n_tree, narrow);
                if (P.n_tree_wide && P.n_tree_wide < P.n_tree)
                        std::stable_partition(ts, ts + P.n_tree, narrow);
        }

        inline void place_rich_wide(BatchPlan &P) {
                if (P.rich_wide.empty())
                        return;
                uint64_t cells = 0, slots = 0;
                for (size_t i = 0; i < P.plan.size(); ++i) {
                        const DevQuery &q = P.plan[i];
                        DevRichWide w{};
                        if (q.nscore > RICH_NARROW_TERMS) {
                                w.cells = cells, w.slots = slots, w.stride = (q.nscore + 7u) & ~7u;
                                cells += (uint64_t)q.out_cap * w.stride, slots += q.out_cap;
                                P.n_rich_wide += q.ntasks;
                        }
                        P.rich_wide[i] = w;
                }
                P.rich_wide_cells = cells, P.rich_wide_slots = slots;
                std::copy(P.sched.begin(), P.sched.end(), P.rich_sched.begin());
                std::stable_partition(P.rich_sched.begin(), P.rich_sched.end(), [&](const uint32_t ti) { return P.rich_wide[P.tasks[ti].slot].stride == 0; });
        }

        inline void deal_cand_queues(PlanState &S) {
                BatchPlan &P = S.P;
                const uint32_t nc = P.n_cand;
                uint32_t *const sc = P.sched.p + S.cand_first;
                if (S.cand_rows) {
                        for (uint32_t x = 0; x <= CAND_QUEUES; ++x)
                                P.cand_q[x] = x < CAND_QUEUES ? S.cand_qat[x] - S.cand_first : nc;
                } else {
                        const std::vector<uint32_t> was(sc, sc + nc);
                        uint32_t pos = 0;
                        for (uint32_t x = 0; x < CAND_QUEUES; ++x) {
                                P.cand_q[x] = pos;
                                for (uint32_t i = x; i < nc; i += CAND_QUEUES)
                                        sc[pos++] = was[i];
                        }
                        P.cand_q[CAND_QUEUES] = pos;
                }
        }

        inline void order_phrase_tasks(BatchPlan &P) {
                if (P.ptasks.size() <= 1)
                        return;
                const size_t np = P.ptasks.size();
                std::vector<uint32_t> key(np), sorted(np);
                uint32_t hist[SCHED_NB + 1] = {};
                for (size_t i = 0; i < np; ++i) {
                        const uint32_t ti = P.ptasks[i];
                        const DevTask &tk = P.tasks[ti];
                        const DevQuery &q = P.plan[tk.slot];
                        const uint64_t end = ti + 1 < q.first_task + q.ntasks ? P.tasks[ti + 1].out_off : q.out_off + q.out_cap;
                        key[i] = SCHED_NB - 1 - cost_bucket(end - tk.out_off);
                        ++hist[key[i] + 1];
                }
                for (uint32_t bk = 0; bk < SCHED_NB; ++bk)
                        hist[bk + 1] += hist[bk];
                for (size_t i = 0; i < np; ++i)
                        sorted[hist[key[i]]++] = P.ptasks[i];
                std::copy(sorted.begin(), sorted.end(), P.ptasks.p);
        }

        inline void account_distinct_bytes(const HostIndex &ix, const Ctx &C, BatchPlan &P) {
                std::vector<uint8_t> seen(ix.terms.size(), 0);
                std::vector<uint8_t> seen_hits(ix.terms.size(), 0);
                for (size_t sidx = 0; sidx < P.plan.size(); ++sidx) {
                        const DevQuery &q = P.plan[sidx];
                        const uint32_t kind = P.tasks[q.first_task].kind;
                        auto touch = [&](uint32_t term) {
                                if (!(seen[term] & 0x80u))
                                        P.distinct_bytes += ix.docbytes[term];
                                if (!(seen[term] & (1u << kind)))
                                        P.distinct_bytes_kind[kind] += ix.docbytes[term];
                                seen[term] |= (uint8_t)(0x80u | (1u << kind));
                        };
                        if (kind == TASK_TREE) {
                                const uint32_t *rec = &P.tree[q.fused_idx];
                                const DevTreeNode *tn = reinterpret_cast<const DevTreeNode *>(rec + TREE_HDR_WORDS);
                                for (uint32_t k = 0; k < rec[0]; ++k)
                                        if (tn[k].op == TRI_OP_TERM)
                                                touch(tn[k].arg);
                        } else if (task_onepass(kind)) {
                                const DevFused &z = P.fused[q.fused_idx];
                                for (uint32_t k = 0; k < z.nslots; ++k)
                                        touch(z.term[k]);
                        } else {
                                for (uint32_t k = 0; k < q.nterms; ++k)
                                        touch(P.qterms[q.term_base + k] & QT_TERM);
                                if (C.mode != TRI_FLAG_DOCUMENTS_ONLY)
                                        for (uint32_t k = 0; k < q.nscore; ++k)
                                                touch(P.sterms[q.score_base + k]);
                        }
                        auto touch_hits = [&](uint32_t term, bool phrase) {
                                if (!(seen_hits[term] & 1u))
                                        P.distinct_bytes += ix.hitbytes[term];
                                if (phrase && !(seen_hits[term] & 2u))
                                        P.distinct_bytes_kind[TASK_KINDS] += ix.hitbytes[term];
                                seen_hits[term] |= (uint8_t)(1u | (phrase ? 2u : 0u));
                        };
                        for (uint32_t ph = 0; ph < q.nphrases; ++ph)
                                for (uint32_t k = 0; k < P.phrases[q.phrase_base + ph].nterms; ++k)
                                        touch_hits(P.pterms[P.phrases[q.phrase_base + ph].term_base + k], true);
                        if (C.rich)
                                for (uint32_t k = 0; k < q.nscore; ++k)
                                        touch_hits(P.sterms[q.score_base + k], false);
                }
        }
}

inline int plan_batch(const HostIndex &ix, const PlanEnv &env, const PlanInput &in, HostPool *pool, const std::function<uint8_t *(size_t)> &alloc_block,
                      BatchPlan &P, std::string &err, trip::FragCache *frag_cache = nullptr) {
        using namespace trip;
        auto t0 = std::chrono::steady_clock::now();
        static const bool dbg_plan = getenv("TRINITY_DEBUG_PLAN") != nullptr;
        const uint32_t mode = in.flags & (TRI_FLAG_DOCUMENTS_ONLY | TRI_FLAG_ACCUMULATED_SCORE | TRI_FLAG_MATCHED_TERMS);
        PlanState S{ix, env, env.opt, pool, P, err, Ctx{ix, env, in, mode == TRI_FLAG_ACCUMULATED_SCORE, mode == TRI_FLAG_MATCHED_TERMS, mode}, LapTimer{dbg_plan}};
        if (env.opt.tree_max_nodes < TREE_MAX_NODES || env.opt.tree_max_nodes > TREE_WIDE_MAX_NODES)
                return herr(err, TRI_ERR_INVALID, "tri_batch_create: option tree_max_nodes = %llu (%u .. %u)", (unsigned long long)env.opt.tree_max_nodes, TREE_MAX_NODES, TREE_WIDE_MAX_NODES);
        if (env.opt.rich_max_terms < RICH_NARROW_TERMS || env.opt.rich_max_terms > RICH_WIDE_TERMS)
                return herr(err, TRI_ERR_INVALID, "tri_batch_create: option rich_max_terms = %llu (%u .. %u)", (unsigned long long)env.opt.rich_max_terms, RICH_NARROW_TERMS, RICH_WIDE_TERMS);
        P.slot_of_query.assign(in.nq, UINT32_MAX);
        P.qstatus.assign(in.nq, TRI_OK);
        eligible_planes(S);
        take_fragments(S, frag_cache);
        S.dbg.lap("setup");
        if (const int rc = S.run_pass("LOWER", "lowering the batch", [&](Frag &f) { return lower_range(S.C, f); }))
                return rc;
        settle_batch_knobs(S);
        S.dbg.lap("glue0");
        P.plan_ms[0] = ms_since(t0);
        if (const int rc = S.run_pass("TASKS", "cutting the batch into tasks", [&](Frag &f) { return task_range(S.C, f); }))
                return rc;
        P.plan_ms[1] = ms_since(t0);
        if (const int rc = place_fragments(S))
                return rc;
        choose_planes(S);
        assign_cand_rows(S);
        if (const int rc = layout_block(S, alloc_block))
                return rc;
        if (const int rc = S.run_pass("FILL", "filling the plan", [&](Frag &f) {
                    fill_fragment(S, f);
                    return key_fragment(S, f);
            }))
                return rc;
        for (const Frag &f : S.frags) {
                P.pscatter_docs += f.pscatter_docs;
                P.probe_queries -= f.probe_demoted, P.cand_queries += f.probe_demoted;
                P.term_bytes_probe -= f.probe_demoted_bytes;
        }
        P.plan_ms[2] = ms_since(t0);
        place_schedule(S);
        deal_cand_queues(S);
        split_tree_section(P);
        place_rich_wide(P);
        order_phrase_tasks(P);
        P.sparse_cap = (P.sparse_cap + 63u) & ~63u;
        S.dbg.lap("sched+rest");
        if (dbg_plan)
                fprintf(stderr, "[tri plan] nq %zu frags %zu:%s\n", in.nq, S.frags.size(), S.dbg.line.c_str());
        P.plan_ms[3] = ms_since(t0);
        if (env.opt.account_needed_bytes && !ix.terms.empty())
                account_distinct_bytes(ix, S.C, P);
        return TRI_OK;
}
```

### trinity_amd/csrc/planner_types.hpp

```cpp
#pragma once
#include "host_pool.hpp"
#include "index_host.hpp"

#include <array>
#include <chrono>
#include <cmath>
#include <memory>
#include <numeric>

struct tri_options {
        uint64_t dense_min_postings = 512 * 1024;
        uint64_t dense_task_cost = 192 * 1024;
        uint64_t dense_window_cost = 16 * 1024;
        uint64_t cand_task_cost = 32 * 1024;
        uint64_t fused = 1;
        uint64_t fused_task_cost = 0;
        uint64_t fused_freq_cap = 0;
        uint64_t account_needed_bytes = 0;
        uint64_t fused_halfwords = 1;
        uint64_t overlap_dense_wgs = 0, overlap_cand_wgs = 0;
        uint64_t overlap = 0;
        uint64_t planes = 7;
        uint64_t planes_split = 0;
        uint64_t plane_div = 1024;
        uint64_t plane_amortize = 1;
        uint64_t plane_max_bytes = 8ull << 30;
        uint64_t planes_rebuild = 0;
        uint64_t phrase_task_div = 0;
        uint64_t planes_order = 1;
        uint64_t scatter_bitmap_slack = 4;
        uint64_t pset_order = 1;
        uint64_t cand_xcd = 1;
        uint64_t plan_threads = 0;
        uint64_t plan_hot_us = 300;
        uint64_t plan_pin = 2;
        uint64_t result_bitmaps = 1;
        uint64_t tree_max_bytes = 16ull << 30;
        uint64_t tree_max_nodes = 64;
        uint64_t tree_wide_min_nodes = 65;
        uint64_t rich_max_terms = 16;
        uint64_t probe_max_blocks = 0;
};

struct PlanEnv {
        tri_options opt;
        uint32_t cus = 256;
        uint32_t fus_wgs_per_cu = 2;
        uint32_t plk_wgs_per_cu = 2;
};

template <class T>
struct Span {
        T *p = nullptr;
        size_t n = 0;
        size_t off = 0;
        size_t size() const { return n; }
        bool empty() const { return !n; }
        T *data() { return p; }
        const T *data() const { return p; }
        T &operator[](size_t i) { return p[i]; }
        const T &operator[](size_t i) const { return p[i]; }
        T *begin() { return p; }
        T *end() { return p + n; }
        const T *begin() const { return p; }
        const T *end() const { return p + n; }
};

struct PlanInput {
        const uint32_t *prog = nullptr;
        size_t prog_len = 0;
        const tri_query *queries = nullptr;
        size_t nq = 0;
        const double *weights = nullptr;
        uint32_t flags = 0, topk = 0;
        int similarity = TRI_SIM_BM25;
};

namespace trip {
        struct PlanCounters {
                uint64_t term_bytes = 0, term_bytes_dense = 0, term_bytes_fused = 0, term_bytes_planes = 0, term_bytes_phrase_hits = 0, term_bytes_pset = 0, term_bytes_probe = 0,
                         cand_needed_term_bytes = 0;
                uint64_t dense_queries = 0, pset_queries = 0, probe_queries = 0, cand_queries = 0, fused_queries = 0, planes_queries = 0, tree_queries = 0;
                uint64_t bitmap_queries = 0;
                uint64_t pscatter_queries = 0, pscatter_docs = 0;
                uint64_t cand_lead_docs = 0, cand_terms = 0;
                uint64_t probe_demoted = 0, probe_demoted_bytes = 0;
                uint32_t sparse_cap = 0;
                uint32_t rich_R = 0;
                uint64_t rich_wide_queries = 0;
                bool rich_allow = false;
                void merge(const PlanCounters &o) {
                        term_bytes += o.term_bytes, term_bytes_dense += o.term_bytes_dense, term_bytes_fused += o.term_bytes_fused, term_bytes_planes += o.term_bytes_planes;
                        term_bytes_phrase_hits += o.term_bytes_phrase_hits, term_bytes_pset += o.term_bytes_pset, term_bytes_probe += o.term_bytes_probe;
                        cand_needed_term_bytes += o.cand_needed_term_bytes;
                        dense_queries += o.dense_queries, pset_queries += o.pset_queries, probe_queries += o.probe_queries, cand_queries += o.cand_queries;
                        fused_queries += o.fused_queries, planes_queries += o.planes_queries, tree_queries += o.tree_queries;
                        bitmap_queries += o.bitmap_queries, pscatter_queries += o.pscatter_queries, pscatter_docs += o.pscatter_docs;
                        cand_lead_docs += o.cand_lead_docs, cand_terms += o.cand_terms;
                        probe_demoted += o.probe_demoted, probe_demoted_bytes += o.probe_demoted_bytes;
                        sparse_cap = std::max(sparse_cap, o.sparse_cap);
                        rich_R = std::max(rich_R, o.rich_R);
                        rich_wide_queries += o.rich_wide_queries;
                        rich_allow |= o.rich_allow;
                }
        };
}

struct BatchPlan : trip::PlanCounters {
        uint8_t *block = nullptr;
        size_t block_bytes = 0;
        Span<DevQuery> plan;
        Span<uint32_t> qterms;
        Span<DevTask> tasks;
        Span<uint32_t> sched;
        Span<DevFused> fused;
        Span<uint32_t> qplane;
        Span<uint32_t> plane_terms;
        Span<uint32_t> splane;
        Span<uint32_t> sterms;
        Span<double> sweights;
        Span<DevPhrase> phrases;
        Span<uint32_t> pterms, ptasks;
        Span<DevPsetUnit> units;
        Span<uint32_t> pset_sched;
        Span<uint32_t> cand_q;
        Span<uint32_t> tree;
        Span<uint32_t> tree_terms;
        Span<uint32_t> tree_hidden;
        Span<DevRichWide> rich_wide;
        Span<uint32_t> rich_sched;
        uint32_t n_rich_wide = 0;
        uint64_t rich_wide_cells = 0, rich_wide_slots = 0;
        uint32_t n_tree = 0;
        uint32_t n_tree_wide = 0;
        uint64_t tree_scratch_bytes = 0;
        std::vector<uint32_t> slot_of_query;
        std::vector<int32_t> qstatus;
        uint32_t n_dense = 0, n_pset = 0, n_probe = 0, n_cand = 0, n_fused = 0, n_fused16 = 0, n_fusedgen = 0, n_planes = 0, n_planes8 = 0;
        uint32_t plw = 0;
        uint32_t plane_rows = 0;
        uint64_t out_capacity = 0;
        uint64_t plane_decoded_bytes = 0, unsupported_queries = 0;
        uint64_t distinct_bytes = 0, distinct_bytes_kind[TASK_KINDS + 1] = {};
        std::string last_unsupported;
        double plan_ms[4] = {0, 0, 0, 0};
};

namespace trip {
        constexpr size_t SECTION_ALIGN = 64;
        struct SectionCounts {
                size_t plan = 0, qterms = 0, tasks = 0, fused = 0, qplane = 0, plane_terms = 0, splane = 0, sterms = 0, sweights = 0, phrases = 0, pterms = 0, ptasks = 0, units = 0,
                       tree = 0, tree_terms = 0, tree_hidden = 0, rich_wide = 0, rich_sched = 0;
        };
        template <class Plan, class Fn>
        inline void for_each_section(Plan &P, const SectionCounts &n, Fn &&fn) {
                fn(P.plan, n.plan);
                fn(P.qterms, n.qterms);
                fn(P.tasks, n.tasks);
                fn(P.sched, n.tasks);
                fn(P.fused, n.fused);
                fn(P.qplane, n.qplane);
                fn(P.plane_terms, n.plane_terms);
                fn(P.splane, n.splane);
                fn(P.sterms, n.sterms);
                fn(P.sweights, n.sweights);
                fn(P.phrases, n.phrases);
                fn(P.pterms, n.pterms);
                fn(P.ptasks, n.ptasks);
                fn(P.units, n.units);
                fn(P.pset_sched, n.units);
                fn(P.cand_q, (size_t)CAND_QUEUES + 1);
                fn(P.tree, n.tree);
                fn(P.tree_terms, n.tree_terms);
                fn(P.tree_hidden, n.tree_hidden);
                if (n.rich_wide) {
                        fn(P.rich_wide, n.rich_wide);
                        fn(P.rich_sched, n.rich_sched);
                }
        }
        inline size_t layout_sections(BatchPlan &P, const SectionCounts &n) {
                size_t bytes = 0;
                for_each_section(P, n, [&](auto &s, const size_t count) {
                        s.off = bytes;
                        s.n = count;
                        bytes += (count * sizeof(*s.p) + SECTION_ALIGN + SECTION_ALIGN - 1) & ~(SECTION_ALIGN - 1);
                });
                return bytes;
        }
        inline void point_sections(BatchPlan &P, const SectionCounts &n) {
                for_each_section(P, n, [&](auto &s, size_t) { s.p = reinterpret_cast<std::remove_reference_t<decltype(*s.p)> *>(P.block + s.off); });
        }

        constexpr uint32_t SCHED_NB = 64 * 4;
        constexpr uint32_t CAND_SUBS = 128, CAND_COST_SUBS = 16;
        constexpr uint32_t PSET_RANGE_BKS = 64, PSET_SUBS = 64;
        constexpr uint32_t CAND_KEY0 = TASK_KINDS * SCHED_NB, PSET_KEY0 = CAND_KEY0 + CAND_QUEUES * CAND_SUBS, SCHED_KEYS = PSET_KEY0 + PSET_RANGE_BKS * PSET_SUBS;
        inline uint32_t pset_sub(const uint32_t rank) { return rank < PSET_SUBS / 2 ? rank : std::min(PSET_SUBS / 2 + (rank - PSET_SUBS / 2) / 8, PSET_SUBS - 1); }
        constexpr uint64_t CAND_ROWS_MIN_LEAD = 1024;
        constexpr uint32_t SCHED_RANK[TASK_KINDS] = {3, 0, 4, 5, 6, 7, 8, 1, 2, 9};
        constexpr uint32_t BatchPlan::*const SCHED_COUNT[TASK_KINDS] = {&BatchPlan::n_cand, &BatchPlan::n_dense, &BatchPlan::n_fused, &BatchPlan::n_fused16, &BatchPlan::n_fusedgen,
                                                                        &BatchPlan::n_planes, &BatchPlan::n_planes8, &BatchPlan::n_pset, &BatchPlan::n_probe, &BatchPlan::n_tree};
        inline uint32_t sched_first(const BatchPlan &P, const uint32_t kind) {
                uint32_t at = 0;
                for (uint32_t k = 0; k < TASK_KINDS; ++k)
                        if (SCHED_RANK[k] < SCHED_RANK[kind])
                                at += P.*SCHED_COUNT[k];
                return at;
        }
        inline uint32_t cost_bucket(const uint64_t cost) {
                const uint64_t c = std::max<uint64_t>(1, cost);
                const uint32_t lg = 63u - (uint32_t)__builtin_clzll(c);
                const uint32_t frac = lg >= 2 ? (uint32_t)((c >> (lg - 2)) & 3u) : (uint32_t)((c << (2 - lg)) & 3u);
                return lg * 4 + frac;
        }
        inline uint32_t sched_key(const uint32_t kind, const uint64_t cost) {
                if (kind == TASK_PSET)
                        return SCHED_RANK[TASK_PSET] * SCHED_NB + (uint32_t)std::min<uint64_t>((cost & 0xffffffffull) / PSET_TASK_WINDOWS, SCHED_NB - 1);
                return SCHED_RANK[kind] * SCHED_NB + (SCHED_NB - 1 - cost_bucket(cost));
        }

        struct PNode {
                uint32_t op = 0, term = 0;
                uint32_t tok = 0;
                uint32_t kid_off = 0, kid_n = 0;
                uint64_t cost = 0;
                bool empty = false;
        };

        struct Scratch {
                std::vector<PNode> nodes;
                std::vector<int> kidpool, st, tmpk;
                std::vector<uint64_t> cs;
                std::vector<uint32_t> gt, gs;
                std::vector<uint32_t> gorder, leaves, leaf_tok, negs, opts, opt_tok, ts, ts_tok, u, uniq, rt, seen, phterms, slots;
                struct PhraseTmp {
                        uint32_t t0, n;
                        double weight;
                };
                std::vector<PhraseTmp> qphrases;
                std::vector<std::pair<uint32_t, double>> sc;
                const int *kids(const PNode &x) const { return kidpool.data() + x.kid_off; }
        };

        struct Tmp {
                DevQuery q;
                uint64_t cost;
                uint32_t nlead;
                int32_t fz;
                bool truth;
                bool tree;
                bool hidden;
                uint64_t tree_ub;
                bool tree_wide;
                uint32_t hidden_ord;
                uint64_t sumdf, lead_docs;
                uint32_t last_doc;
                bool dense, fuse;
        };

        struct QUse {
                uint32_t qpos, term;
        };
        struct FUse {
                uint32_t fidx, slot, term;
        };

        struct Frag : PlanCounters {
                size_t q_lo = 0, q_hi = 0;
                Scratch S;
                std::vector<Tmp> tmp;
                std::vector<uint32_t> qterms, pterms, sterms;
                std::vector<double> sweights;
                std::vector<DevPhrase> phrases;
                std::vector<DevFused> fz;
                std::vector<size_t> left_out;
                uint64_t onepass_queries = 0, fused_postings = 0, phrase_queries = 0;
                std::vector<DevTask> tasks;
                std::vector<uint64_t> tcost;
                std::vector<DevFused> fused;
                std::vector<uint32_t> ptasks;
                std::vector<DevPsetUnit> units;
                std::vector<QUse> quses, suses;
                std::vector<FUse> fuses;
                std::vector<uint64_t> benefit;
                std::vector<uint64_t> cand_row;
                std::vector<uint32_t> keys, hist;
                std::vector<uint32_t> treepool;
                std::vector<uint32_t> tree_terms;
                uint32_t n_hidden = 0;
                uint64_t off = 0;
                size_t b_plan = 0, b_qterms = 0, b_sterms = 0, b_phrases = 0, b_pterms = 0, b_tasks = 0, b_fused = 0, b_ptasks = 0, b_units = 0, b_tree = 0, b_hidden = 0;
                uint64_t b_off = 0;
                int rc = TRI_OK;
                std::string err;
                void recycle() {
                        Frag fresh;
                        auto keep = [](auto &dst, auto &src) {
                                src.clear();
                                dst = std::move(src);
                        };
                        keep(fresh.S.nodes, S.nodes), keep(fresh.S.kidpool, S.kidpool), keep(fresh.S.st, S.st), keep(fresh.S.tmpk, S.tmpk), keep(fresh.S.cs, S.cs);
                        keep(fresh.S.gt, S.gt), keep(fresh.S.gs, S.gs), keep(fresh.S.gorder, S.gorder), keep(fresh.S.leaves, S.leaves), keep(fresh.S.leaf_tok, S.leaf_tok);
                        keep(fresh.S.negs, S.negs), keep(fresh.S.opts, S.opts), keep(fresh.S.opt_tok, S.opt_tok), keep(fresh.S.ts, S.ts), keep(fresh.S.ts_tok, S.ts_tok);
                        keep(fresh.S.u, S.u), keep(fresh.S.uniq, S.uniq), keep(fresh.S.rt, S.rt), keep(fresh.S.seen, S.seen), keep(fresh.S.phterms, S.phterms);
                        keep(fresh.S.slots, S.slots), keep(fresh.S.qphrases, S.qphrases), keep(fresh.S.sc, S.sc);
                        keep(fresh.tmp, tmp), keep(fresh.qterms, qterms), keep(fresh.pterms, pterms), keep(fresh.sterms, sterms), keep(fresh.sweights, sweights);
                        keep(fresh.phrases, phrases), keep(fresh.fz, fz), keep(fresh.left_out, left_out), keep(fresh.tasks, tasks), keep(fresh.tcost, tcost);
                        keep(fresh.fused, fused), keep(fresh.ptasks, ptasks), keep(fresh.units, units), keep(fresh.quses, quses), keep(fresh.suses, suses);
                        keep(fresh.fuses, fuses), keep(fresh.benefit, benefit), keep(fresh.cand_row, cand_row), keep(fresh.keys, keys), keep(fresh.hist, hist), keep(fresh.treepool, treepool);
                        keep(fresh.tree_terms, tree_terms);
                        *this = std::move(fresh);
                }
        };
        struct FragCache {
                std::vector<Frag> frags;
        };

        struct Ctx {
                const HostIndex &ix;
                const PlanEnv &env;
                const PlanInput &in;
                bool scored, rich;
                uint32_t mode;
                uint32_t n_ok = 0;
                bool plane_ok(uint32_t term) const { return ix.df_rank[term] < n_ok; }
                uint64_t planes_split = 2, fused_task_cost = 0, phrase_task_div = 1;
                uint32_t plw = 0;
                double term_weight(const uint32_t df) const {
                        if (in.similarity == TRI_SIM_TFIDF)
                                return std::log((double)((uint64_t)ix.info.docs_cnt + 1) / (double)(df + 1)) + 1.0;
                        if (in.similarity == TRI_SIM_TRIVIAL)
                                return 0.0;
                        const float num = (float)((uint64_t)ix.info.docs_cnt - (uint64_t)df) + 0.5f;
                        const float den = (float)df + 0.5f;
                        return (double)std::log(1 + num / den);
                }
                uint32_t first_block_ge(const DevTerm &t, const uint64_t key) const {
                        if (t.win_off != 0xffffffffu && !ix.win.empty() && !(key & (CELL_DOCS - 1)) && (key >> CELL_LOG2) < ix.nwin)
                                return ix.win[t.win_off + (key >> CELL_LOG2)];
                        const uint32_t *lb = &ix.blk_last[t.first_block];
                        return (uint32_t)(std::lower_bound(lb, lb + t.nblocks, (uint32_t)std::min<uint64_t>(key, 0xffffffffull)) - lb);
                }
        };

        inline uint64_t distinct_docbytes(const HostIndex &ix, const uint32_t *terms, const size_t n, std::vector<uint32_t> &seen) {
                uint64_t bytes = 0;
                seen.clear();
// ... 47 lines not shown
```

### trinity_amd/csrc/trinity_hip.hip

```cpp
#include "../../include/trinity_hip.h"
#include <chrono>
#include <hip/hip_runtime.h>

#include <algorithm>
#include <array>
#include <cmath>
#include <cstdarg>
#include <cstdio>
#include <cstring>
#include <ctime>
#include <unistd.h>
#include <dlfcn.h>
#include <memory>
#include <mutex>
#include <numeric>
#include <string>
#include <thread>
#include <unordered_map>
#include <functional>
#include <vector>

static thread_local char g_err[512] = "";
static int fail(int code, const char *fmt, ...) {
        va_list ap;
        va_start(ap, fmt);
        vsnprintf(g_err, sizeof g_err, fmt, ap);
        va_end(ap);
        return code;
}
#define HIP_TRY(expr)                                                                                       \
        do {                                                                                                \
                hipError_t e_ = (expr);                                                                     \
                if (e_ != hipSuccess)                                                                       \
                        return fail(e_ == hipErrorOutOfMemory ? TRI_ERR_NOMEM : TRI_ERR_DEVICE, "%s: %s (%s:%d)", #expr, hipGetErrorString(e_), __FILE__, __LINE__); \
        } while (0)

extern "C" const char *tri_last_error(void) { return g_err; }
extern "C" int tri_abi_version(void) { return TRI_ABI_VERSION; }

#include "planner.hpp"

struct tri_dev {
        int device;
        hipStream_t stream, stream2;
        hipStream_t stream_up;
        hipStream_t stream_rb;
        hipEvent_t ev_fork, ev_join;
        int cus;
        tri_options opt;
        int refs = 0;
        bool closing = false;
        struct Pool {
                std::vector<std::pair<size_t, void *>> idle;
                std::unordered_map<void *, size_t> size_of;
                size_t idle_bytes = 0;
        } pool;
        std::vector<std::pair<size_t, void *>> pinned_idle;
        std::vector<hipEvent_t> events_idle;
        static constexpr unsigned PLAN_CTXS = 2;
        struct PlanCtx {
                std::mutex mu;
                std::unique_ptr<HostPool> pool;
                trip::FragCache frag_cache;
        } planners[PLAN_CTXS];
        int plan_anchor = -1;
        std::recursive_mutex mu;
};
using DevLock = std::lock_guard<std::recursive_mutex>;
constexpr size_t TICKET_DENSE_WORD = 16;
constexpr size_t TICKET_PSET_WORD = 20;
constexpr size_t TICKET_PROBE_WORD = 22;
constexpr size_t TICKET_PLANES_WORD = 24;
constexpr size_t TICKET_SCORE_WORD = 32;
constexpr size_t TICKET_RICH_COUNT_WORD = TICKET_SCORE_WORD;
constexpr size_t TICKET_RICH_WRITE_WORD = 40;
constexpr size_t TICKET_RICH_WIDE = 2;
constexpr size_t TICKET_SCAT_WORD = 44;
constexpr size_t TICKET_PHRASE_WORD = 48;
constexpr size_t TICKET_FUSED_WORD = 56;
constexpr size_t TICKET_CAND_WORD = 64;
static_assert(std::max({TICKET_DENSE_WORD, TICKET_PSET_WORD, TICKET_PROBE_WORD, TICKET_PLANES_WORD + 2, TICKET_SCORE_WORD, TICKET_RICH_COUNT_WORD + TICKET_RICH_WIDE, TICKET_RICH_WRITE_WORD + TICKET_RICH_WIDE,
                        TICKET_SCAT_WORD + 1, TICKET_PHRASE_WORD, TICKET_FUSED_WORD + 2 * 2}) < TICKET_CAND_WORD,
              "every kernel's ticket word lies below k_and's queues");
constexpr size_t TICKET_BYTES = (TICKET_CAND_WORD + CAND_QUEUES * CAND_TICKET_STRIDE) * 4;
constexpr size_t POOL_MIN_BYTES = 64u << 10;
constexpr size_t POOL_IDLE_CAP = 64ull << 30;
constexpr size_t PINNED_IDLE_MAX = 16;

static void dev_destroy(tri_dev *d) {
        hipSetDevice(d->device);
        for (auto &pc : d->planners)
                pc.pool.reset();
        hipEventDestroy(d->ev_fork);
        hipEventDestroy(d->ev_join);
        for (hipEvent_t e : d->events_idle)
                hipEventDestroy(e);
        hipStreamDestroy(d->stream_up);
        hipStreamDestroy(d->stream_rb);
        hipStreamDestroy(d->stream2);
        hipStreamDestroy(d->stream);
        for (auto &b : d->pool.idle)
                hipFree(b.second);
        for (auto &b : d->pinned_idle)
                hipHostFree(b.second);
        delete d;
}
static void dev_retain(tri_dev *d) {
        DevLock g(d->mu);
        ++d->refs;
}
static void dev_release(tri_dev *d) {
        if (!d)
                return;
        bool last;
        {
                DevLock g(d->mu);
                last = --d->refs == 0 && d->closing;
        }
        if (last)
                dev_destroy(d);
}

static hipError_t pool_alloc(tri_dev *dev, void **out, const size_t bytes) {
        if (bytes < POOL_MIN_BYTES)
                return hipMalloc(out, bytes);
        DevLock g(dev->mu);
        auto &P = dev->pool;
        size_t best = SIZE_MAX;
        for (size_t i = 0; i < P.idle.size(); ++i)
                if (P.idle[i].first >= bytes && P.idle[i].first <= 2 * bytes && (best == SIZE_MAX || P.idle[i].first < P.idle[best].first))
                        best = i;
        if (best != SIZE_MAX) {
                *out = P.idle[best].second;
                P.idle_bytes -= P.idle[best].first;
                P.idle.erase(P.idle.begin() + (ptrdiff_t)best);
                return hipSuccess;
        }
        const size_t gran = bytes >= (8u << 20) ? (2u << 20) : (64u << 10);
        const size_t rounded = (bytes + gran - 1) & ~(gran - 1);
        static const bool dbg_pool = getenv("TRINITY_DEBUG_CREATE") != nullptr;
        if (dbg_pool) {
                std::string have;
                for (const auto &b : P.idle)
                        have += " " + std::to_string(b.first >> 20);
                fprintf(stderr, "[tri pool_alloc] COLD hipMalloc of %zu MB (idle buffers, MB:%s)\n", rounded >> 20, have.c_str());
        }
        hipError_t e = hipMalloc(out, rounded);
        if (e != hipSuccess && !P.idle.empty()) {
                (void)hipGetLastError();
                for (auto &b : P.idle) {
                        P.size_of.erase(b.second);
                        hipFree(b.second);
                }
                P.idle.clear();
                P.idle_bytes = 0;
                e = hipMalloc(out, rounded);
        }
        if (e == hipSuccess)
                P.size_of[*out] = rounded;
        return e;
}
static void pool_free(tri_dev *dev, void *p) {
        if (!p)
                return;
        if (!dev) {
                hipFree(p);
                return;
        }
        DevLock g(dev->mu);
        auto &P = dev->pool;
        const auto it = P.size_of.find(p);
        if (it == P.size_of.end()) {
                hipFree(p);
                return;
        }
        P.idle.emplace_back(it->second, p);
        P.idle_bytes += it->second;
        while (P.idle_bytes > POOL_IDLE_CAP) {
                size_t big = 0;
                for (size_t i = 1; i < P.idle.size(); ++i)
                        if (P.idle[i].first > P.idle[big].first)
                                big = i;
                P.idle_bytes -= P.idle[big].first;
                P.size_of.erase(P.idle[big].second);
                hipFree(P.idle[big].second);
                P.idle.erase(P.idle.begin() + (ptrdiff_t)big);
        }
}
static uint8_t *pinned_alloc(tri_dev *dev, const size_t bytes, size_t *cap) {
        DevLock g(dev->mu);
        auto &I = dev->pinned_idle;
        size_t best = SIZE_MAX;
        for (size_t i = 0; i < I.size(); ++i)
                if (I[i].first >= bytes && I[i].first <= 4 * bytes + (1u << 20) && (best == SIZE_MAX || I[i].first < I[best].first))
                        best = i;
        if (best != SIZE_MAX) {
                void *p = I[best].second;
                *cap = I[best].first;
                I.erase(I.begin() + (ptrdiff_t)best);
                return static_cast<uint8_t *>(p);
        }
        const size_t rounded = (bytes + bytes / 4 + (256u << 10)) & ~(size_t)((64u << 10) - 1);
        void *p = nullptr;
        if (hipHostMalloc(&p, rounded, hipHostMallocDefault) != hipSuccess) {
                (void)hipGetLastError();
                return nullptr;
        }
        *cap = rounded;
        return static_cast<uint8_t *>(p);
}
static void pinned_free(tri_dev *dev, void *p, const size_t cap) {
        if (!p)
                return;
        if (!dev) {
                hipHostFree(p);
                return;
        }
        DevLock g(dev->mu);
        if (dev->pinned_idle.size() >= PINNED_IDLE_MAX) {
                hipHostFree(dev->pinned_idle.front().second);
                dev->pinned_idle.erase(dev->pinned_idle.begin());
        }
        dev->pinned_idle.emplace_back(cap, p);
}
static void event_put(tri_dev *dev, hipEvent_t e) {
        if (!e)
                return;
        DevLock g(dev->mu);
        dev->events_idle.push_back(e);
}
static hipError_t event_get(tri_dev *dev, hipEvent_t *e) {
        DevLock g(dev->mu);
        if (!dev->events_idle.empty()) {
                *e = dev->events_idle.back();
                dev->events_idle.pop_back();
                return hipSuccess;
        }
// ... 98 lines not shown
        uint32_t *d_scat_off = nullptr, *d_scat_cnt = nullptr, *d_scat_docs = nullptr;
        uint32_t scat_cap = 0;
        bool ran = false;
        bool planes_hi = false;
        uint32_t *d_out = nullptr;
        uint32_t *d_counts = nullptr;
        uint32_t *d_ticket = nullptr;
        uint32_t *d_rich_allow = nullptr;
        uint64_t *d_hashes = nullptr;
        uint64_t *d_qcounts = nullptr;
        uint32_t *d_part_docs = nullptr, *d_part_counts = nullptr, *d_top_docs = nullptr, *d_top_counts = nullptr;
        double *d_part_scores = nullptr;
        float *d_top_scores = nullptr;
        double *d_all_scores = nullptr;
        uint32_t *d_rich_present = nullptr, *d_task_hits = nullptr;
        uint16_t *d_rich_freq = nullptr, *d_rich_pool = nullptr;
        uint16_t *d_rich_freq_wide = nullptr;
        uint32_t *d_rich_present_hi = nullptr, *d_rich_allow_hi = nullptr;
        uint8_t *d_rich_plen = nullptr;
        uint64_t *d_rich_payload = nullptr;
        uint64_t *d_task_pos_base = nullptr;
        std::vector<uint64_t> h_task_pos_base;
        size_t rich_pool_cap = 0;
        double *d_pscore = nullptr;
        std::vector<uint32_t> h_counts;
        std::vector<uint64_t> h_query_counts;
        bool synced = false;
        std::vector<const tri_filter *> filter_rows;
        uint8_t *d_filter_tab = nullptr;
        uint32_t *d_filter_rows = nullptr;
        size_t filter_rows_cap = 0;
        tri_batch_info info{};
        ~tri_batch() {
                if (dev) {
                        hipSetDevice(dev->device);
                        if (ran && !synced)
                                hipStreamSynchronize(dev->stream);
                        if (ev[EV_UP])
                                hipEventSynchronize(ev[EV_UP]);
                }
                for (hipEvent_t e : ev)
                        if (dev)
                                event_put(dev, e);
                        else if (e)
                                hipEventDestroy(e);
                pinned_free(dev, block, block_cap);
                pool_free(dev, d_arena);
                pool_free(dev, d_sparse);
                pool_free(dev, d_out);
                pool_free(dev, d_rich_allow);
                hipFree(d_hashes);
                pool_free(dev, d_part_docs);
                pool_free(dev, d_part_scores);
                pool_free(dev, d_all_scores);
                pool_free(dev, d_rich_present);
                pool_free(dev, d_rich_freq);
                pool_free(dev, d_rich_freq_wide);
                pool_free(dev, d_rich_present_hi);
                pool_free(dev, d_rich_allow_hi);
                hipFree(d_rich_pool);
                hipFree(d_rich_plen);
                hipFree(d_rich_payload);
                pool_free(dev, d_pscore);
                pool_free(dev, d_tree_scratch);
                pool_free(dev, d_tree_scores);
                pool_free(dev, d_scat_docs);
                pool_free(dev, d_filter_tab);
                pool_free(dev, d_filter_rows);
                dev_release(dev);
        }
};


#include "dev_stream.hpp"
#include "k_decode.hpp"
#include "k_match.hpp"
#include "k_score.hpp"
#include "k_fused.hpp"
#include "k_planes.hpp"
#include "k_psets.hpp"
#include "k_probe.hpp"
#include "k_encode.hpp"
#include "k_phrase.hpp"
#include "k_rich.hpp"
#include "k_tree.hpp"
#include "k_tree_wide.hpp"
#include "k_commit.hpp"
#include "k_lencode.hpp"
#include "filtered_kernels.hpp"

template <class Pick, class... Args>
static void tri_launch(const int codec, Pick pick, const dim3 grid, const dim3 block, const hipStream_t stream, Args... args) {
        if (codec == TRI_CODEC_LUCENE)
                hipLaunchKernelGGL(pick(std::integral_constant<int, CODEC_LUCENE>()), grid, block, 0, stream, args...);
        else
                hipLaunchKernelGGL(pick(std::integral_constant<int, CODEC_GOOGLE>()), grid, block, 0, stream, args...);
}
#define TRI_LAUNCH(K, codec, grid, block, stream, ...) tri_launch(codec, [](auto c_) { return K<c_.value>; }, grid, block, stream, __VA_ARGS__)

extern "C" int tri_dev_open(int device, tri_dev **out) {
        if (!out)
                return fail(TRI_ERR_INVALID, "tri_dev_open: null out");
        int n = 0;
        HIP_TRY(hipGetDeviceCount(&n));
        if (device < 0 || device >= n)
                return fail(TRI_ERR_INVALID, "tri_dev_open: device %d out of range (%d devices)", device, n);
        HIP_TRY(hipSetDevice(device));
        auto d = std::make_unique<tri_dev>();
        d->device = device;
        HIP_TRY(hipStreamCreateWithFlags(&d->stream, hipStreamNonBlocking));
        HIP_TRY(hipStreamCreateWithFlags(&d->stream2, hipStreamNonBlocking));
        HIP_TRY(hipStreamCreateWithFlags(&d->stream_up, hipStreamNonBlocking));
        HIP_TRY(hipStreamCreateWithFlags(&d->stream_rb, hipStreamNonBlocking));
        HIP_TRY(hipEventCreateWithFlags(&d->ev_fork, hipEventDisableTiming));
        HIP_TRY(hipEventCreateWithFlags(&d->ev_join, hipEventDisableTiming));
        hipDeviceProp_t prop;
        HIP_TRY(hipGetDeviceProperties(&prop, device));
        d->cus = prop.multiProcessorCount;
        *out = d.release();
        return TRI_OK;
}

extern "C" void tri_dev_close(tri_dev *d) {
        if (!d)
                return;
        if (d->refs > 0) {
                d->closing = true;
                return;
        }
        dev_destroy(d);
}

namespace {
        uint64_t *option_slot(tri_options &o, const char *name) {
                static const struct {
                        const char *name;
                        uint64_t tri_options::*field;
                } table[] = {{"dense_min_postings", &tri_options::dense_min_postings}, {"dense_task_cost", &tri_options::dense_task_cost},
                             {"fused", &tri_options::fused},
                             {"fused_task_cost", &tri_options::fused_task_cost},
                             {"fused_freq_cap", &tri_options::fused_freq_cap},
                             {"fused_halfwords", &tri_options::fused_halfwords},
                             {"account_needed_bytes", &tri_options::account_needed_bytes},
                             {"overlap_dense_wgs", &tri_options::overlap_dense_wgs},
                             {"overlap_cand_wgs", &tri_options::overlap_cand_wgs},
                             {"overlap", &tri_options::overlap},
                             {"planes", &tri_options::planes},
                             {"plane_div", &tri_options::plane_div},
                             {"planes_split", &tri_options::planes_split},
                             {"plane_max_bytes", &tri_options::plane_max_bytes},
                             {"plane_amortize", &tri_options::plane_amortize},
                             {"planes_rebuild", &tri_options::planes_rebuild},
                             {"cand_xcd", &tri_options::cand_xcd},
                             {"plan_threads", &tri_options::plan_threads},
                             {"probe_max_blocks", &tri_options::probe_max_blocks}, {"phrase_task_div", &tri_options::phrase_task_div}, {"plan_hot_us", &tri_options::plan_hot_us}, {"plan_pin", &tri_options::plan_pin}, {"planes_order", &tri_options::planes_order}, {"pset_order", &tri_options::pset_order}, {"scatter_bitmap_slack", &tri_options::scatter_bitmap_slack}, {"tree_max_bytes", &tri_options::tree_max_bytes}, {"tree_max_nodes", &tri_options::tree_max_nodes}, {"tree_wide_min_nodes", &tri_options::tree_wide_min_nodes}, {"rich_max_terms", &tri_options::rich_max_terms}, {"result_bitmaps", &tri_options::result_bitmaps}, {"cand_task_cost", &tri_options::cand_task_cost}, {"dense_window_cost", &tri_options::dense_window_cost}};
                for (const auto &e : table)
                        if (!strcmp(e.name, name))
                                return &(o.*(e.field));
                return nullptr;
        }
}

extern "C" int tri_dev_set_option(tri_dev *d, const char *name, uint64_t value) {
        if (!d || !name)
                return fail(TRI_ERR_INVALID, "tri_dev_set_option: null argument");
        uint64_t *slot = option_slot(d->opt, name);
        if (!slot)
                return fail(TRI_ERR_INVALID, "tri_dev_set_option: unknown option '%s'", name);
        *slot = value;
        return TRI_OK;
}

extern "C" int tri_dev_get_option(tri_dev *d, const char *name, uint64_t *value) {
        if (!d || !name || !value)
                return fail(TRI_ERR_INVALID, "tri_dev_get_option: null argument");
        const uint64_t *slot = option_slot(d->opt, name);
        if (!slot)
                return fail(TRI_ERR_INVALID, "tri_dev_get_option: unknown option '%s'", name);
        *value = *slot;
        return TRI_OK;
}

extern "C" int tri_dev_memory(tri_dev *d, tri_dev_memory_info *out) {
        if (!d || !out)
                return fail(TRI_ERR_INVALID, "tri_dev_memory: null argument");
        HIP_TRY(hipSetDevice(d->device));
        size_t fr = 0, total = 0;
        HIP_TRY(hipMemGetInfo(&fr, &total));
        DevLock g(d->mu);
        uint64_t all = 0, pinned = 0;
        for (const auto &kv : d->pool.size_of)
                all += kv.second;
        for (const auto &pb : d->pinned_idle)
                pinned += pb.first;
        out->pool_idle_bytes = d->pool.idle_bytes;
        out->pool_in_use_bytes = all - d->pool.idle_bytes;
        out->pinned_idle_bytes = pinned;
        out->device_free_bytes = fr;
        out->device_total_bytes = total;
        return TRI_OK;
}

extern "C" int tri_dev_sync(tri_dev *d) {
        if (!d)
                return fail(TRI_ERR_INVALID, "null dev");
        HIP_TRY(hipStreamSynchronize(d->stream));
        return TRI_OK;
}

extern "C" void *tri_dev_stream(tri_dev *d) { return d ? (void *)d->stream : nullptr; }

namespace {
        template <class T>
        int dev_upload(T **dst, const std::vector<T> &src, size_t extra = 0) {
                HIP_TRY(hipMalloc((void **)dst, (src.size() + extra) * sizeof(T) + 16));
                if (!src.empty())
                        HIP_TRY(hipMemcpy(*dst, src.data(), src.size() * sizeof(T), hipMemcpyHostToDevice));
                return TRI_OK;
        }
}

extern "C" int tri_index_upload(tri_dev *dev, const uint8_t *index, size_t len, const uint8_t *hits, size_t hits_len, int codec,
                                const tri_term *terms, size_t nterms, uint32_t docs_cnt, tri_index **out) {
        if (!dev || !out || (!index && len) || (!terms && nterms) || (!hits && hits_len))
                return fail(TRI_ERR_INVALID, "tri_index_upload: null argument");
        HIP_TRY(hipSetDevice(dev->device));
        auto ix = std::make_unique<tri_index>();
        {
                std::string err;
                if (const int rc = build_host_index(index, len, hits, hits_len, codec, terms, nterms, docs_cnt, *ix, err))
                        return fail(rc, "%s", err.c_str());
        }
        ix->dev = dev;
        dev_retain(dev);
        if (!ix->dev_index.empty()) {
                index = ix->dev_index.data();
                len = ix->dev_index.size();
                hits = ix->dev_hits.empty() ? nullptr : ix->dev_hits.data();
                hits_len = ix->dev_hits.size();
        }
        int rc;
        if ((rc = dev_upload(&ix->d_win, ix->win, 3 * CELLS_PER_SPAN + 8)))
                return rc;
        HIP_TRY(hipMemset(ix->d_win + ix->win.size(), 0, (3 * CELLS_PER_SPAN + 8) * sizeof(uint32_t)));
        HIP_TRY(hipMalloc((void **)&ix->d_index, len + 256));
        HIP_TRY(hipMemset(ix->d_index, 0, len + 256));
        if (len)
                HIP_TRY(hipMemcpy(ix->d_index, index, len, hipMemcpyHostToDevice));
        if ((rc = dev_upload(&ix->d_blk_last, ix->blk_last)) || (rc = dev_upload(&ix->d_blk_off, ix->blk_off)) || (rc = dev_upload(&ix->d_terms, ix->terms)))
                return rc;
        if (codec == TRI_CODEC_GOOGLE) {
                ix->blk_doff.push_back((uint32_t)ix->dstream.size() + 1);
                ix->dstream.resize(ix->dstream.size() + 256, 0);
                if ((rc = dev_upload(&ix->d_dstream, ix->dstream)) || (rc = dev_upload(&ix->d_blk_doff, ix->blk_doff)))
                        return rc;
        }
        if (hits_len) {
                HIP_TRY(hipMalloc((void **)&ix->d_hits, hits_len + 256));
                HIP_TRY(hipMemset(ix->d_hits, 0, hits_len + 256));
                HIP_TRY(hipMemcpy(ix->d_hits, hits, hits_len, hipMemcpyHostToDevice));
                if (ix->has_hdir && ((rc = dev_upload(&ix->d_blk_hits, ix->blk_hits)) || (rc = dev_upload(&ix->d_hdir, ix->hdir))))
                        return rc;
        }
        if (codec == TRI_CODEC_GOOGLE && (rc = dev_upload(&ix->d_blk_hits, ix->blk_hits)))
                return rc;
        if (codec == TRI_CODEC_LUCENE) {
                static_assert(sizeof(RowRec) == sizeof(uint4), "row records are read as uint4");
                HIP_TRY(hipMalloc((void **)&ix->d_blk_rec, ix->blk_rec.size() * sizeof(uint4) + 16));
                if (!ix->blk_rec.empty())
                        HIP_TRY(hipMemcpy(ix->d_blk_rec, ix->blk_rec.data(), ix->blk_rec.size() * sizeof(uint4), hipMemcpyHostToDevice));
        }
        ix->release_device_columns();
        *out = ix.release();
        return TRI_OK;
}


extern "C" int tri_index_set_masked(tri_index *ix, const uint32_t *docids, size_t n) {
        if (!ix || (!docids && n))
                return fail(TRI_ERR_INVALID, "tri_index_set_masked: null argument");
        HIP_TRY(hipSetDevice(ix->dev->device));
        HIP_TRY(hipStreamSynchronize(ix->dev->stream));
        if (!n) {
                hipFree(ix->d_masked);
                ix->d_masked = nullptr;
                return TRI_OK;
        }
        const size_t words = ((size_t)ix->max_doc / SPAN_BITS + 2) * (SPAN_BITS / 32);
        std::vector<uint32_t> bm(words, 0);
        for (size_t i = 0; i < n; ++i)
                if (docids[i] <= ix->max_doc)
                        bm[docids[i] >> 5] |= 1u << (docids[i] & 31);
        if (!ix->d_masked)
                HIP_TRY(hipMalloc((void **)&ix->d_masked, words * 4));
        HIP_TRY(hipMemcpy(ix->d_masked, bm.data(), words * 4, hipMemcpyHostToDevice));
        return TRI_OK;
}

extern "C" void tri_index_destroy(tri_index *ix) {
        delete ix;
}

extern "C" int tri_index_get_info(const tri_index *ix, tri_index_info *info) {
        if (!ix || !info)
                return fail(TRI_ERR_INVALID, "null argument");
        *info = ix->info;
// ... 385 lines not shown
        for (uint32_t kind = 0; kind < TASK_KINDS; ++kind)
                b->info.launches += kind != TASK_TREE && b.get()->*trip::SCHED_COUNT[kind];
        b->info.create_plan_ms = (float)(b->plan_ms[0] + b->plan_ms[1] + b->plan_ms[2] + b->plan_ms[3]);
        b->info.create_ms = (float)std::chrono::duration<double, std::milli>(std::chrono::steady_clock::now() - t_create).count();
        if (dbg_create)
                fprintf(stderr, "[tri create] nq %zu: plan %.3f  arena+copy %.3f  planes/sparse %.3f  out(%.1f MB) %.3f  rest %.3f  total %.3f ms\n", nq, dbg_t[0], dbg_t[1] - dbg_t[0],
                        dbg_t[2] - dbg_t[1], (double)off * 4 / 1e6, dbg_t[3] - dbg_t[2], b->info.create_ms - dbg_t[3], b->info.create_ms);
        *out = b.release();
        return TRI_OK;
}

extern "C" void tri_batch_destroy(tri_batch *b) {
        delete b;
}


static FilterSel filter_sel(const tri_batch *b) {
        if (b->filter_rows.empty())
                return FilterSel{nullptr, nullptr, nullptr, 0u};
        return FilterSel{b->d_filter_rows, (const uint32_t *)b->d_filter_tab, b->dev_at(b->tasks), (uint32_t)filter_words(b->ix)};
}
template <class F>
struct FilteredKernel;
template <class... A>
struct FilteredKernel<void (*)(A...)> {
        using type = void (*)(A..., FilterSel);
};
template <class Pick, class... Args>
static void tri_launch_matching(const tri_batch *b, const int kernel, const int variant, Pick pick, const dim3 grid, const dim3 block, const hipStream_t stream, Args... args) {
        const FilterSel fsel = filter_sel(b);
        if (!fsel.rows)
                return tri_launch(b->ix->codec, pick, grid, block, stream, args...);
        using Plain = decltype(+pick(std::integral_constant<int, CODEC_GOOGLE>()));
        const auto twin = reinterpret_cast<typename FilteredKernel<Plain>::type>(const_cast<void *>(filtered_kernel(kernel, b->ix->codec == TRI_CODEC_LUCENE ? CODEC_LUCENE : CODEC_GOOGLE, variant)));
        hipLaunchKernelGGL(twin, grid, block, 0, stream, args..., fsel);
}
static size_t filter_tab_ptrs_off(const tri_batch *b) { return (b->plan.size() * 4 + 15) & ~(size_t)15; }

static int run_filter_rows(tri_batch *b) {
        if (b->filter_rows.empty())
                return TRI_OK;
        tri_dev *dev = b->dev;
        const size_t n4 = filter_words(b->ix) / 4;
        const uint32_t nrows = (uint32_t)b->filter_rows.size();
        for (uint32_t y0 = 0; y0 < nrows; y0 += 65535u) {
                hipLaunchKernelGGL(k_filter_rows, dim3((unsigned)std::min<size_t>((n4 + FILTER_WG - 1) / FILTER_WG, 1024), std::min(65535u, nrows - y0)), dim3(FILTER_WG), 0, dev->stream,
                                   (const uint4 *const *)(b->d_filter_tab + filter_tab_ptrs_off(b)) + y0, (const uint4 *)b->ix->d_masked, (uint4 *)b->d_filter_rows + (size_t)y0 * n4, n4);
                HIP_TRY(hipGetLastError());
        }
        return TRI_OK;
}

static int run_plane_rows(tri_batch *b) {
        tri_dev *dev = b->dev;
        tri_index *ix = b->ix;
        b->info.term_planes_decoded_bytes = 0;
        if (!b->plane_terms.empty()) {
                std::vector<uint32_t> build;
                const uint8_t needs = b->planes_hi ? 3u : 1u;
                for (const uint32_t term : b->plane_terms) {
                        const uint32_t row = ix->df_rank[term];
                        if (row < ix->pc_cap && ((ix->pc_built[row] & needs) != needs || dev->opt.planes_rebuild)) {
                                build.push_back(term);
                                build.push_back(row);
                                b->info.term_planes_decoded_bytes += ix->docbytes[term];
                        }
                }
                if (!build.empty()) {
                        HIP_TRY(hipMemcpyAsync(b->d_build, build.data(), build.size() * 4, hipMemcpyHostToDevice, dev->stream));
                        const uint32_t nrows = (uint32_t)(build.size() / 2), nwin = b->plw / PL_WORDS;
                        for (uint32_t y0 = 0; y0 < nrows; y0 += 65535u) {
                                const uint32_t ny = std::min(65535u, nrows - y0);
                                if (b->planes_hi)
                                        TRI_LAUNCH(k_term_planes, ix->codec, dim3(nwin, ny), dim3(AND_WG), dev->stream, ix->d_index, ix->d_blk_last, ix->d_blk_off, ix->d_blk_rec,
                                                   ix->d_blk_doff, ix->d_win, ix->d_terms, (const uint32_t *)b->d_build + 2 * (size_t)y0, ix->d_pcache, (size_t)b->plw, ix->d_pcache_hi,
                                                   (size_t)PL_HI * b->plw, b->plw, (uint32_t *)nullptr);
                                else
                                        TRI_LAUNCH(k_term_plane0, ix->codec, dim3((nwin + P0_GROUP - 1) / P0_GROUP, ny), dim3(AND_WG), dev->stream, ix->d_index, ix->d_blk_last, ix->d_blk_off,
                                                   ix->d_blk_rec, ix->d_blk_doff, ix->d_win, ix->d_terms, (const uint32_t *)b->d_build + 2 * (size_t)y0, ix->d_pcache, b->plw, (uint32_t *)nullptr);
                                HIP_TRY(hipGetLastError());
                        }
                        for (size_t i = 1; i < build.size(); i += 2)
                                ix->pc_built[build[i]] |= needs;
                }
        }
        HIP_TRY(hipEventRecord(b->ev[EV_PLANE_ROWS], dev->stream));
        return TRI_OK;
}

static int run_matching(tri_batch *b) {
        tri_dev *dev = b->dev;
        tri_index *ix = b->ix;
        const uint8_t *match_bytes = ix->codec == TRI_CODEC_GOOGLE ? ix->d_dstream : ix->d_index;
        const uint32_t *match_off = ix->codec == TRI_CODEC_GOOGLE ? ix->d_blk_doff : ix->d_blk_off;
        uint32_t dense_wgs = TRI_DENSE_WAVES * 256 / DENSE_WG, cand_wgs = 4;
        bool overlap = false;
        if (dev->opt.overlap_dense_wgs && dev->opt.overlap_cand_wgs && (b->n_dense || b->n_pset) && b->n_cand) {
                overlap = true;
                dense_wgs = (uint32_t)dev->opt.overlap_dense_wgs;
                cand_wgs = (uint32_t)dev->opt.overlap_cand_wgs;
        } else if (dev->opt.overlap && b->n_cand && trip::sched_first(*b, TASK_CAND))
                overlap = true;
        hipStream_t cand_stream = dev->stream;
        if (overlap) {
                HIP_TRY(hipEventRecord(dev->ev_fork, dev->stream));
                HIP_TRY(hipStreamWaitEvent(dev->stream2, dev->ev_fork, 0));
                cand_stream = dev->stream2;
        }
        const DevPsetUnit *units = b->dev_at(b->units);
        const uint32_t *pset_sched = b->dev_at(b->pset_sched);
        const FilterSel fsel = filter_sel(b);
        const bool prep = b->n_pset && b->pscatter_queries, prep_forked = prep && !overlap && b->n_dense;
        if (prep) {
                if (prep_forked) {
                        HIP_TRY(hipEventRecord(dev->ev_fork, dev->stream));
                        HIP_TRY(hipStreamWaitEvent(dev->stream2, dev->ev_fork, 0));
                }
                hipStream_t prep_stream = prep_forked ? dev->stream2 : dev->stream;
                const uint32_t nunits = b->n_pset + b->n_probe, nscat = (uint32_t)b->pscatter_queries;
                hipLaunchKernelGGL(k_psets_prep_list, dim3((nunits + 255) / 256), dim3(256), 0, prep_stream, units, nunits, b->d_ticket + TICKET_SCAT_WORD + 1, b->d_scat_list, nscat);
                HIP_TRY(hipGetLastError());
                TRI_LAUNCH(k_psets_prep, ix->codec, dim3(nscat), dim3(PSCAT_WG), prep_stream, units, (const uint32_t *)b->d_scat_list, (const uint32_t *)(b->d_ticket + TICKET_SCAT_WORD + 1),
                           b->dev_at(b->plan), b->dev_at(b->tasks), (const uint32_t *)b->dev_at(b->qterms), (const uint32_t *)b->dev_opt(b->qplane), ix->d_masked, ix->d_index, ix->d_blk_last, ix->d_blk_off, ix->d_blk_rec,
                           ix->d_blk_doff, ix->d_terms, b->d_ticket + TICKET_SCAT_WORD, b->d_scat_off, b->d_scat_cnt, b->d_scat_docs, b->scat_cap, fsel);
                HIP_TRY(hipGetLastError());
                if (prep_forked)
                        HIP_TRY(hipEventRecord(dev->ev_join, dev->stream2));
        }
        if (b->n_dense) {
                tri_launch_matching(b, FK_AND_DENSE, 0, [](auto c) { return k_and_dense<c.value>; }, dim3(std::min<uint32_t>(b->n_dense, (uint32_t)dev->cus * dense_wgs)), dim3(DENSE_WG), dev->stream, match_bytes, ix->d_blk_last,
                           match_off, ix->d_win, ix->d_terms, b->dev_at(b->plan), b->dev_at(b->tasks), b->dev_at(b->sched) + trip::sched_first(*b, TASK_DENSE), b->dev_at(b->qterms), b->n_dense,
                           b->d_ticket + TICKET_DENSE_WORD, b->d_out, b->d_counts, ix->d_masked, (const uint32_t *)b->dev_opt(b->qplane), (const uint32_t *)ix->d_pcache, b->plw);
                HIP_TRY(hipGetLastError());
        }
        HIP_TRY(hipEventRecord(b->ev[EV_DENSE], dev->stream));
        if (prep_forked)
                HIP_TRY(hipStreamWaitEvent(dev->stream, dev->ev_join, 0));
        if (b->n_pset) {
                const uint32_t pset_wgs = TRI_PSET_WAVES * 256 / PSET_WG;
                tri_launch_matching(b, FK_PSETS, 0, [](auto c) { return k_psets<c.value>; }, dim3(std::min<uint32_t>(b->n_pset, (uint32_t)dev->cus * (overlap && dev->opt.overlap_dense_wgs ? std::min<uint32_t>(dense_wgs, pset_wgs) : pset_wgs))),
                           dim3(PSET_WG), dev->stream, units, pset_sched, b->n_pset, b->d_ticket + TICKET_PSET_WORD, (const uint32_t *)b->dev_at(b->qterms), (const uint32_t *)b->dev_opt(b->qplane), b->d_out,
                           b->d_counts, ix->d_masked, (const uint32_t *)ix->d_pcache, b->plw, (const uint32_t *)b->d_scat_off, (const uint32_t *)b->d_scat_cnt,
                           (const uint32_t *)b->d_scat_docs);
                HIP_TRY(hipGetLastError());
        }
        HIP_TRY(hipEventRecord(b->ev[EV_PSET], dev->stream));
        if (b->n_probe) {
                tri_launch_matching(b, FK_PROBE, 0, [](auto c) { return k_probe<c.value>; }, dim3(std::min<uint32_t>((b->n_probe + PROBE_WG / 64 - 1) / (PROBE_WG / 64), (uint32_t)dev->cus * (TRI_PROBE_WAVES * 256 / PROBE_WG))),
                           dim3(PROBE_WG), dev->stream, match_bytes, ix->d_blk_last, match_off, ix->d_terms, units, pset_sched + b->n_pset, b->n_probe, b->d_ticket + TICKET_PROBE_WORD,
                           (const uint32_t *)b->dev_at(b->qterms), (const uint32_t *)b->dev_opt(b->qplane), b->d_out, b->d_counts, ix->d_masked, (const uint32_t *)ix->d_pcache, b->plw);
                HIP_TRY(hipGetLastError());
        }
        HIP_TRY(hipEventRecord(b->ev[EV_PROBE], dev->stream));
        if (b->n_cand)
                tri_launch_matching(b, FK_AND, 0, [](auto c) { return k_and<c.value>; }, dim3(std::min<uint32_t>(b->n_cand, (uint32_t)dev->cus * cand_wgs)), dim3(AND_WG), cand_stream, match_bytes, ix->d_blk_last, match_off,
                           ix->d_win, ix->d_terms, b->dev_at(b->plan), b->dev_at(b->tasks), b->dev_at(b->sched) + trip::sched_first(*b, TASK_CAND), b->dev_at(b->qterms), b->dev_at(b->cand_q),
                           b->d_ticket + TICKET_CAND_WORD, b->d_out, b->d_counts, ix->d_masked, (const uint32_t *)b->dev_opt(b->qplane), (const uint32_t *)ix->d_pcache, b->plw);
        HIP_TRY(hipGetLastError());
        if (overlap) {
                HIP_TRY(hipEventRecord(dev->ev_join, dev->stream2));
                HIP_TRY(hipStreamWaitEvent(dev->stream, dev->ev_join, 0));
        }
        HIP_TRY(hipEventRecord(b->ev[EV_CAND], dev->stream));
        return TRI_OK;
}

static int run_fused(tri_batch *b) {
        tri_dev *dev = b->dev;
        tri_index *ix = b->ix;
        for (uint32_t kind = TASK_FUSED; kind <= TASK_FUSED_GEN; ++kind) {
                const uint32_t nf = b->*trip::SCHED_COUNT[kind], variant = kind - TASK_FUSED;
                if (!nf)
                        continue;
                tri_launch_matching(b, FK_FUSED, (int)variant, [&](auto c) { return std::array{k_fused<c.value, 0, 0>, k_fused<c.value, 1, 0>, k_fused<c.value, 0, 1>}[variant]; },
                           dim3(std::min<uint32_t>(nf, (uint32_t)dev->cus * FUS_WGS_PER_CU)), dim3(FUS_WG), dev->stream, ix->d_index, ix->d_blk_last, ix->d_blk_off, ix->d_blk_rec,
                           ix->d_blk_doff, ix->d_win, ix->d_terms, b->dev_at(b->plan), b->dev_at(b->fused), b->dev_at(b->tasks), (const uint32_t *)b->dev_at(b->sched) + trip::sched_first(*b, kind), b->dev_at(b->sterms),
                           b->dev_at(b->sweights), nf, b->d_ticket + TICKET_FUSED_WORD + 2 * variant, b->d_counts, b->topk, b->d_part_docs, b->d_part_scores, b->d_part_counts, ix->d_masked,
                           b->similarity, b->d_out, b->d_all_scores, b->d_rich_allow);
                HIP_TRY(hipGetLastError());
        }
        HIP_TRY(hipEventRecord(b->ev[EV_FUSED], dev->stream));
        return TRI_OK;
}

static int run_planes(tri_batch *b) {
        tri_dev *dev = b->dev;
        tri_index *ix = b->ix;
        if (b->d_qthr)
                HIP_TRY(hipMemsetAsync(b->d_qthr, 0, (b->plan.size() + 1) * 8, dev->stream));
        for (uint32_t kind = TASK_PLANES; kind <= TASK_PLANES8; ++kind) {
                const uint32_t np = b->*trip::SCHED_COUNT[kind], wide = kind - TASK_PLANES;
                if (!np)
                        continue;
                tri_launch_matching(b, FK_PLANES, (int)wide, [&](auto c) { return wide ? k_planes<c.value, FUS_MAX_SLOTS> : k_planes<c.value, PLK_NS_SMALL>; },
                           dim3(std::min<uint32_t>(np, (uint32_t)dev->cus * PLK_WGS_PER_CU)), dim3(PLK_WG), dev->stream, ix->d_index, ix->d_blk_last, ix->d_blk_off, ix->d_blk_rec,
                           ix->d_blk_doff, ix->d_win, ix->d_terms, b->dev_at(b->plan), b->dev_at(b->fused), b->dev_at(b->tasks), (const uint32_t *)b->dev_at(b->sched) + trip::sched_first(*b, kind), b->dev_at(b->sterms),
                           b->dev_at(b->sweights), np, b->d_ticket + TICKET_PLANES_WORD + 2 * wide, b->d_counts, b->topk, b->d_part_docs, b->d_part_scores, b->d_part_counts, ix->d_masked,
                           b->similarity, (const uint32_t *)ix->d_pcache, (const uint32_t *)ix->d_pcache_hi, b->plw, ix->pc_cap, b->d_sparse, b->sparse_cap, b->d_qthr);
                HIP_TRY(hipGetLastError());
        }
        HIP_TRY(hipEventRecord(b->ev[EV_PLANES], dev->stream));
        return TRI_OK;
}

static int run_phrases(tri_batch *b) {
        tri_dev *dev = b->dev;
        tri_index *ix = b->ix;
        if (!b->ptasks.empty() && ix->codec == TRI_CODEC_GOOGLE && ix->d_prank && ix->pc_cap) {
                std::vector<uint32_t> hits_build, hits_only;
                uint32_t max_blocks = 0;
                for (size_t i = 0; i < b->pterms.size(); ++i) {
                        const uint32_t term = b->pterms[i], r = ix->df_rank[term];
                        if (r >= ix->pc_cap || ix->ph_built[r])
                                continue;
                        const DevTerm &t = ix->terms[term];
                        if (!(t.flags & TERM_FULL_BLOCKS) || !t.documents)
                                continue;
                        ix->ph_built[r] = 1;
                        max_blocks = std::max(max_blocks, t.nblocks);
                        std::vector<uint32_t> &dst = (ix->pc_built[r] & 4u) ? hits_only : hits_build;
                        ix->pc_built[r] |= 5u;
                        dst.push_back(term);
                        dst.push_back(r);
                }
                const uint32_t nrows_build = (uint32_t)(hits_build.size() / 2);
                hits_build.insert(hits_build.end(), hits_only.begin(), hits_only.end());
                if (!hits_build.empty()) {
                        uint32_t *d_pairs = ix->d_ph_pairs + 2 * ix->ph_pairs_n;
                        HIP_TRY(hipMemcpyAsync(d_pairs, hits_build.data(), hits_build.size() * 4, hipMemcpyHostToDevice, dev->stream));
                        ix->ph_pairs_n += hits_build.size() / 2;
                        for (uint32_t y0 = 0; y0 < nrows_build; y0 += 65535u) {
                                const dim3 grid((b->plw / PL_WORDS + P0_GROUP - 1) / P0_GROUP, std::min(65535u, nrows_build - y0));
                                TRI_LAUNCH(k_term_plane0, ix->codec, grid, dim3(AND_WG), dev->stream, ix->d_index, ix->d_blk_last, ix->d_blk_off, ix->d_blk_rec, ix->d_blk_doff, ix->d_win,
                                           ix->d_terms, (const uint32_t *)d_pairs + 2 * (size_t)y0, ix->d_pcache, b->plw, ix->d_prank);
                                HIP_TRY(hipGetLastError());
                        }
                        const uint32_t npairs = (uint32_t)(hits_build.size() / 2);
                        for (uint32_t y0 = 0; y0 < npairs; y0 += 65535u) {
                                hipLaunchKernelGGL(k_term_hits, dim3((max_blocks + 255) / 256, std::min(65535u, npairs - y0)), dim3(256), 0, dev->stream, ix->d_index, ix->d_blk_off,
                                                   ix->d_blk_hits, ix->d_terms, (const uint32_t *)d_pairs + 2 * (size_t)y0, (const uint64_t *)ix->d_hs_off, ix->d_phs, ix->d_term_row);
                                HIP_TRY(hipGetLastError());
                        }
                }
        }
        if (!b->ptasks.empty()) {
                const uint32_t np = (uint32_t)b->ptasks.size();
                TRI_LAUNCH(k_phrase, ix->codec, dim3(std::min<uint32_t>(np, (uint32_t)dev->cus * PHRASE_WGS_PER_CU)), dim3(AND_WG), dev->stream, ix->d_index, ix->d_hits,
                           ix->d_blk_hits, ix->d_hdir, ix->d_blk_last, ix->d_blk_off, ix->d_win, ix->d_terms, b->dev_at(b->plan), b->dev_at(b->tasks), b->dev_at(b->ptasks), np, b->dev_at(b->phrases), b->dev_at(b->pterms),
                           b->d_ticket + TICKET_PHRASE_WORD, b->d_out, b->d_counts, b->d_pscore,
                           (b->flags & TRI_FLAG_ACCUMULATED_SCORE) ? 65535u : 1u,
                           b->similarity, (const uint32_t *)ix->d_pcache, ix->pc_plw, (const uint32_t *)ix->d_prank, (const unsigned long long *)ix->d_phs,
                           (const uint64_t *)ix->d_hs_off, (const uint32_t *)(ix->codec == TRI_CODEC_GOOGLE ? ix->d_term_row : nullptr));
                HIP_TRY(hipGetLastError());
        }
        HIP_TRY(hipEventRecord(b->ev[EV_PHRASE], dev->stream));
        return TRI_OK;
}

static int run_trees(tri_batch *b) {
        tri_dev *dev = b->dev;
        tri_index *ix = b->ix;
        if (b->n_tree) {
                const uint32_t plw = b->plw, nterms = (uint32_t)b->tree_terms.size(), nhid = (uint32_t)b->tree_hidden.size();
                const uint32_t nchunks = (plw + TREE_CHUNK_WORDS - 1) / TREE_CHUNK_WORDS;
                const uint32_t *tsched = b->dev_at(b->sched) + trip::sched_first(*b, TASK_TREE);
                const uint32_t *d_tree = b->dev_at(b->tree);
                for (uint32_t y0 = 0; y0 < nterms; y0 += 65535u) {
                        const dim3 grid(plw / PL_WORDS, std::min(65535u, nterms - y0));
                        TRI_LAUNCH(k_term_planes, ix->codec, grid, dim3(AND_WG), dev->stream, ix->d_index, ix->d_blk_last, ix->d_blk_off, ix->d_blk_rec, ix->d_blk_doff, ix->d_win,
                                   ix->d_terms, (const uint32_t *)b->d_tree_build + 2 * (size_t)y0, b->d_tree_rows, (size_t)PL_PLANES * plw, b->d_tree_rows + plw,
                                   (size_t)PL_PLANES * plw, plw, (uint32_t *)nullptr);
                        HIP_TRY(hipGetLastError());
                }
                if (nhid) {
                        HIP_TRY(hipMemsetAsync(b->d_tree_prows, 0, (size_t)nhid * plw * 4, dev->stream));
                        hipLaunchKernelGGL(k_tree_gather, dim3(nhid), dim3(TREE_WG), 0, dev->stream, b->dev_at(b->plan), b->dev_at(b->tasks), b->dev_at(b->tree_hidden), b->d_out,
                                           b->d_counts, b->d_pscore, b->d_tree_prows, plw);
                        HIP_TRY(hipGetLastError());
                }
                const bool scored_run = b->flags & TRI_FLAG_ACCUMULATED_SCORE, rich_run = b->flags & TRI_FLAG_MATCHED_TERMS;
                double *tscores = scored_run ? (b->topk ? b->d_tree_scores : b->d_all_scores) : nullptr;
                const uint32_t n_narrow = b->n_tree - b->n_tree_wide;
                for (uint32_t y0 = 0; y0 < b->n_tree;) {
                        const bool wide = y0 >= n_narrow;
                        const uint32_t ny = std::min(65535u, (wide ? b->n_tree : n_narrow) - y0);
                        const dim3 grid(nchunks, ny);
                        uint32_t *qbits = b->d_tree_qbits + (size_t)y0 * plw, *cc = b->d_tree_cc + (size_t)y0 * nchunks;
#define TREE_EVAL_ARGS b->dev_at(b->plan), b->dev_at(b->tasks), tsched + y0, d_tree, (const uint32_t *)b->d_tree_rows, (const uint32_t *)b->d_tree_prows, (const uint32_t *)ix->d_masked, qbits, cc, plw, filter_sel(b)
                        if (wide)
                                hipLaunchKernelGGL(k_tree_eval_wide, grid, dim3(TREE_WG), 0, dev->stream, TREE_EVAL_ARGS);
                        else
                                hipLaunchKernelGGL(k_tree_eval, grid, dim3(TREE_WG), 0, dev->stream, TREE_EVAL_ARGS);
#undef TREE_EVAL_ARGS
                        hipLaunchKernelGGL(k_tree_expand, grid, dim3(TREE_WG), 0, dev->stream, b->dev_at(b->plan), b->dev_at(b->tasks), tsched + y0, (const uint32_t *)qbits, (const uint32_t *)cc,
                                           b->d_out, b->d_counts, plw);
                        if (scored_run || rich_run) {
#define TREE_LEAVES_ARGS                                                                                                                                                                   \
        ix->d_index, ix->d_blk_last, ix->d_blk_off, ix->d_terms, b->dev_at(b->plan), b->dev_at(b->tasks), tsched + y0, d_tree, (const uint32_t *)b->d_tree_rows,                          \
                (const uint32_t *)b->d_tree_prows, (const uint32_t *)cc, (const uint32_t *)b->d_out, (const uint32_t *)b->d_counts, (const double *)b->dev_at(b->sweights),               \
                (const double *)b->d_pscore, tscores, rich_run ? b->d_rich_allow : nullptr, plw, b->similarity, b->d_rich_allow_hi,                                                     \
                (const DevRichWide *)b->dev_opt(b->rich_wide)
                                if (wide)
                                        TRI_LAUNCH(k_tree_leaves_wide, ix->codec, grid, dim3(TREE_WG), dev->stream, TREE_LEAVES_ARGS);
                                else
                                        TRI_LAUNCH(k_tree_leaves, ix->codec, grid, dim3(TREE_WG), dev->stream, TREE_LEAVES_ARGS);
#undef TREE_LEAVES_ARGS
                        }
                        HIP_TRY(hipGetLastError());
                        y0 += ny;
                }
// ... 1298 lines not shown
```

### trinity_amd/hostplan.py

```python
import ctypes as C

import numpy as np

from .engine import TrinityError, flatten, host_lib

_SUMMARY = ["block_bytes", "n_plan", "n_qterms", "n_tasks", "n_fused_maps", "n_qplane", "n_plane_terms", "n_sterms", "n_sweights", "n_phrases", "n_pterms", "n_ptasks",
            "off_plan", "off_qterms", "off_tasks", "off_sched", "off_fused", "off_qplane", "off_plane_terms", "off_sterms", "off_sweights", "off_phrases", "off_pterms", "off_ptasks",
            "n_dense", "n_cand", "n_fused", "n_fused16", "n_fusedgen", "n_planes", "n_planes8", "plw", "sparse_cap", "out_capacity", "term_bytes", "term_bytes_dense",
            "dense_queries", "cand_queries", "fused_queries", "planes_queries", "unsupported_queries", "rich_R", "sizeof_query", "sizeof_task", "sizeof_fused", "sizeof_phrase",
            "cand_needed_term_bytes", "plane_decoded_bytes", "n_pset", "pset_queries", "n_probe", "probe_queries", "n_units", "off_units", "off_unit_sched", "sizeof_unit",
            "n_tree", "tree_queries", "n_tree_words", "off_tree", "n_tree_terms", "off_tree_terms", "n_tree_hidden", "off_tree_hidden", "off_cand_q"]

DEV_QUERY = np.dtype([("nterms", "<u4"), ("term_base", "<u4"), ("out_off", "<u8"), ("out_cap", "<u4"), ("qid", "<u4"), ("first_task", "<u4"), ("ntasks", "<u4"),
                      ("score_base", "<u4"), ("nscore", "<u4"), ("phrase_base", "<u4"), ("nphrases", "<u4"), ("fused_idx", "<u4"), ("form", "<u4")])
DEV_TASK = np.dtype([("slot", "<u4"), ("begin", "<u4"), ("end", "<u4"), ("kind", "<u4"), ("out_off", "<u8")])
TASK_CAND, TASK_DENSE, TASK_FUSED, TASK_FUSED16, TASK_FUSED_GEN, TASK_PLANES, TASK_PLANES8, TASK_PSET, TASK_PROBE, TASK_TREE = range(10)
DEV_TREE_NODE = np.dtype([("op", "u1"), ("parent", "u1"), ("ord", "u1"), ("thr", "u1"), ("arg", "<u4"), ("row", "<u4"), ("score", "<u4"), ("rmask", "<u4"),
                          ("kid0", "u1"), ("kid1", "u1"), ("pad", "u1", 2), ("kids", "<u8")])
TREE_HDR_WORDS = 8
DEV_TREE_NODE_WIDE = np.dtype([("op", "u1"), ("cbits", "u1"), ("parent", "<u2"), ("arg", "<u4"), ("row", "<u4"), ("score", "<u4"), ("rmask", "<u4"),
                               ("ord", "<u2"), ("nkids", "<u2"), ("thr", "<u2"), ("pop", "u1"), ("pcbits", "u1"), ("pad", "<u4")])
TREE_KIND_NARROW, TREE_KIND_WIDE = 0, 1
DEV_RICH_WIDE = np.dtype([("cells", "<u8"), ("slots", "<u8"), ("stride", "<u4"), ("pad", "<u4")])
_RICH_WIDE = ["n_rich_wide_tab", "off_rich_wide", "off_rich_sched", "n_rich_wide", "rich_wide_cells", "rich_wide_slots", "sizeof_rich_wide"]
TREE_NO_PARENT = 0xFFFF
DEV_UNIT = np.dtype([("out_off", "<u8"), ("begin", "<u4"), ("end", "<u4"), ("tix", "<u4"), ("nterms", "<u4"), ("term_base", "<u4"), ("first", "<u4"), ("tt", "<u4", 4), ("row", "<u4", 4)])
SCHED_ORDER = [TASK_DENSE, TASK_PSET, TASK_PROBE, TASK_CAND, TASK_FUSED, TASK_FUSED16, TASK_FUSED_GEN, TASK_PLANES, TASK_PLANES8, TASK_TREE]


def _lib():
    L = host_lib()
    if not hasattr(L, "_plan_ready"):
        vp = C.c_void_p
        L.tri_host_index_build.restype = vp
        L.tri_host_index_build.argtypes = [vp, C.c_uint64, vp, C.c_uint64, C.c_int, vp, C.c_uint64, C.c_uint32, C.c_char_p, C.c_uint64]
        L.tri_host_index_free.argtypes = [vp]
        L.tri_host_plan.restype = vp
        L.tri_host_plan.argtypes = [vp, vp, C.c_uint64, vp, C.c_uint64, C.c_uint32, C.c_uint32, C.c_int, C.c_uint, vp, vp, C.c_uint, C.c_uint32, C.c_char_p, C.c_uint64]
        L.tri_host_plan_free.argtypes = [vp]
        L.tri_host_plan_summary.argtypes = [vp, vp, vp]
        L.tri_host_plan_block.restype = C.POINTER(C.c_uint8)
        L.tri_host_plan_block.argtypes = [vp]
        L.tri_host_plan_query_maps.argtypes = [vp, vp, vp]
        L.tri_host_plan_last_unsupported.argtypes = [vp, C.c_char_p, C.c_uint64]
        L.tri_host_plan_last_unsupported.restype = None
        L.tri_host_plan_rich_wide.argtypes = [vp, vp]
        L.tri_host_plan_rich_wide.restype = None
        L.tri_host_pfor128_group.argtypes = [vp, vp, C.POINTER(C.c_uint32), vp, C.POINTER(C.c_uint32)]
        L.tri_host_pfor128_group.restype = None
        for f in (L.tri_host_lucene_encode, L.tri_host_lucene_encode_units):
            f.argtypes = [vp, vp, vp, vp, C.c_uint64, vp, C.c_uint64, C.POINTER(C.c_uint64), vp, C.c_uint64, C.POINTER(C.c_uint64), vp]
        L._plan_ready = True
    return L


class HostIndex:
    def __init__(self, index_bytes, terms, docs_cnt, codec=1, hits=None):
        b = np.ascontiguousarray(index_bytes, dtype=np.uint8)
        t = np.ascontiguousarray(terms, dtype=np.uint32).reshape(-1, 3)
        h = np.ascontiguousarray(hits, dtype=np.uint8) if hits is not None and len(hits) else None
        err = C.create_string_buffer(600)
        self.h = _lib().tri_host_index_build(b.ctypes.data, b.size, h.ctypes.data if h is not None else None, h.size if h is not None else 0, codec, t.ctypes.data, t.shape[0],
                                             docs_cnt, err, 600)
        if not self.h:
            raise TrinityError(err.value.decode())

    @classmethod
    def from_segment(cls, seg):
        return cls(seg.index, seg.terms, seg.docs_cnt, codec=seg.codec, hits=seg.hits)

    def close(self):
        if self.h:
            _lib().tri_host_index_free(self.h)
            self.h = None

    def __del__(self):
        self.close()


class HostPlan:

    def __init__(self, hindex, programs, flags, topk=0, similarity=0, threads=1, options=None, cus=256, flat=None):
        self.nq = len(programs) if flat is None else flat[1].shape[0]
        prog, q = flatten(programs) if flat is None else flat
        options = options or {}
        names = (C.c_char_p * max(1, len(options)))(*[k.encode() for k in options])
        values = np.array(list(options.values()) or [0], dtype=np.uint64)
        err = C.create_string_buffer(600)
        self.h = _lib().tri_host_plan(hindex.h, prog.ctypes.data, prog.size, q.ctypes.data, self.nq, flags, topk, similarity, threads, names, values.ctypes.data, len(options), cus,
                                      err, 600)
        if not self.h:
            raise TrinityError(err.value.decode())
        out = np.zeros(len(_SUMMARY), dtype=np.uint64)
        ms = np.zeros(4, dtype=np.float64)
        _lib().tri_host_plan_summary(self.h, out.ctypes.data, ms.ctypes.data)
        self.s = {k: int(v) for k, v in zip(_SUMMARY, out)}
        self.ms = ms
        wide = np.zeros(len(_RICH_WIDE), dtype=np.uint64)
        _lib().tri_host_plan_rich_wide(self.h, wide.ctypes.data)
        self.s.update({k: int(v) for k, v in zip(_RICH_WIDE, wide)})
        assert self.s["sizeof_rich_wide"] == DEV_RICH_WIDE.itemsize
        assert self.s["sizeof_query"] == DEV_QUERY.itemsize and self.s["sizeof_task"] == DEV_TASK.itemsize
        p = _lib().tri_host_plan_block(self.h)
        self.block = np.ctypeslib.as_array(p, shape=(max(1, self.s["block_bytes"]),)).copy()
        self.slot_of_query = np.zeros(max(1, self.nq), dtype=np.uint32)
        self.qstatus = np.zeros(max(1, self.nq), dtype=np.int32)
        _lib().tri_host_plan_query_maps(self.h, self.slot_of_query.ctypes.data, self.qstatus.ctypes.data)
        why = C.create_string_buffer(600)
        _lib().tri_host_plan_last_unsupported(self.h, why, 600)
        self.last_unsupported = why.value.decode()

    def _view(self, off, n, dtype):
        dt = np.dtype(dtype)
        return self.block[self.s[off] : self.s[off] + n * dt.itemsize].view(dt)

    @property
    def plan(self):
        return self._view("off_plan", self.s["n_plan"], DEV_QUERY)

    @property
    def tasks(self):
        return self._view("off_tasks", self.s["n_tasks"], DEV_TASK)

    @property
    def sched(self):
        return self._view("off_sched", self.s["n_tasks"], "<u4")

    @property
    def units(self):
        return self._view("off_units", self.s["n_units"], DEV_UNIT)

    @property
    def unit_sched(self):
        return self._view("off_unit_sched", self.s["n_pset"] + self.s["n_probe"], "<u4")

    @property
    def cand_q(self):
        return self._view("off_cand_q", 9, "<u4")

    @property
    def qterms(self):
        return self._view("off_qterms", self.s["n_qterms"], "<u4")

    @property
    def qplane(self):
        return self._view("off_qplane", self.s["n_qplane"], "<u4")

    @property
    def plane_terms(self):
        return self._view("off_plane_terms", self.s["n_plane_terms"], "<u4")

    @property
    def tree_terms(self):
        return self._view("off_tree_terms", self.s["n_tree_terms"], "<u4")

    @property
    def tree_hidden(self):
        return self._view("off_tree_hidden", self.s["n_tree_hidden"], "<u4")

    @property
    def rich_wide(self):
        return self._view("off_rich_wide", self.s["n_rich_wide_tab"], DEV_RICH_WIDE)

    @property
    def rich_sched(self):
        return self._view("off_rich_sched", self.s["n_tasks"] if self.s["n_rich_wide_tab"] else 0, "<u4")

    def leaf_report_mask(self, slot, node):
        if self.tree_kind(slot)[0] == TREE_KIND_WIDE:
            nd = self.tree_nodes_wide(slot)[node]
            return int(nd["rmask"]) | (int(nd["pad"]) << 32)
        nd = self.tree_nodes(slot)[node]
        return int(nd["rmask"]) | ((int(nd["kids"]) & 0xFFFFFFFF) << 32)

    def tree_nodes(self, slot):
        words = self._view("off_tree", self.s["n_tree_words"], "<u4")
        at = int(self.plan[slot]["fused_idx"])
        n = int(words[at])
        return words[at + TREE_HDR_WORDS : at + TREE_HDR_WORDS + 8 * n].view(DEV_TREE_NODE)

    def tree_kind(self, slot):
        words = self._view("off_tree", self.s["n_tree_words"], "<u4")
        at = int(self.plan[slot]["fused_idx"])
        return int(words[at + 1]), int(words[at])

    def tree_header(self, slot):
        words = self._view("off_tree", self.s["n_tree_words"], "<u4")
        at = int(self.plan[slot]["fused_idx"])
        return words[at : at + TREE_HDR_WORDS]

    def tree_nodes_wide(self, slot):
        assert self.tree_kind(slot)[0] == TREE_KIND_WIDE
        return self.tree_nodes(slot).view(DEV_TREE_NODE_WIDE)

    def close(self):
        if self.h:
            self.block = None
            _lib().tri_host_plan_free(self.h)
            self.h = None

    def __del__(self):
        self.close()


def pfor128_group_pair(v):
    v = np.ascontiguousarray(v, dtype=np.uint32)
    assert v.size == 128
    a, b = np.zeros(700, dtype=np.uint8), np.zeros(700, dtype=np.uint8)
    al, bl = C.c_uint32(), C.c_uint32()
    _lib().tri_host_pfor128_group(v.ctypes.data, a.ctypes.data, C.byref(al), b.ctypes.data, C.byref(bl))
    return a[: al.value] if al.value != 0xFFFFFFFF else None, b[: bl.value]


def lucene_encode(docs, freqs, positions, term_first, units=False):
    d = np.ascontiguousarray(docs, dtype=np.uint32)
    f = np.ascontiguousarray(freqs, dtype=np.uint32)
    p = np.ascontiguousarray(positions, dtype=np.uint16)
    tf = np.ascontiguousarray(term_first, dtype=np.uint64)
    n = tf.size - 1
    icap, hcap = 128 + 16 * n + 12 * d.size, 128 + 6 * p.size + 8 * n
    io, ho, t3 = np.zeros(icap, dtype=np.uint8), np.zeros(hcap, dtype=np.uint8), np.zeros((max(n, 1), 3), dtype=np.uint32)
    il, hl = C.c_uint64(), C.c_uint64()
    fn = _lib().tri_host_lucene_encode_units if units else _lib().tri_host_lucene_encode
    if fn(d.ctypes.data, f.ctypes.data, p.ctypes.data, tf.ctypes.data, n, io.ctypes.data, icap, C.byref(il), ho.ctypes.data, hcap, C.byref(hl), t3.ctypes.data):
        raise TrinityError("lucene_encode: buffer too small")
    return io[: il.value], ho[: hl.value], t3[:n]


def cpu_budget():
    L = host_lib()
    L.tri_host_cpu_budget.restype = C.c_uint32
    return int(L.tri_host_cpu_budget())


def pool_cpus(threads=16):
    L = host_lib()
    L.tri_host_pool_cpus.restype = C.c_uint32
    L.tri_host_pool_cpus.argtypes = [C.c_uint32, C.c_void_p, C.c_uint32]
    out = np.zeros(256, dtype=np.int32)
    n = L.tri_host_pool_cpus(threads, out.ctypes.data, out.size)
    return out[:n].tolist()
```

Baseline: 14.57 million.

## Add dedicated pair-AND kernel for two-term candidate queries behind and_pairs option

Adds a k_and_pair kernel for two-term AND queries. It decodes 128 lead blocks at once into shared memory, one lane per block, then probes a plane bitmap for the second term and compacts the hits with a workgroup scan. The planner splits pair tasks into separate queue ranges and sub-keys, and k_and skips those ranges. A new and_pairs option defaults to 0, so the new path likely stays inactive unless enabled. That adds an extra launch and planning complexity.

```diff
diff --git a/trinity_amd/csrc/codec_streams.hpp b/trinity_amd/csrc/codec_streams.hpp
--- a/trinity_amd/csrc/codec_streams.hpp
+++ b/trinity_amd/csrc/codec_streams.hpp
@@ -140,3 +140,34 @@
         }
         __device__ __forceinline__ uint32_t next() { return s.next(); }
 };
+
+template <int CODEC, class Fn>
+__device__ __forceinline__ void block_deltas(const uint8_t *__restrict__ index, const DevTerm &t, const uint32_t b, const uint32_t off, const uint32_t cnt, Fn &&fn) {
+        if constexpr (CODEC == CODEC_LUCENE) {
+                if (b < t.npfor) {
+                        LValStream s;
+                        s.init_group(index, off, b & 3u);
+                        if (s.mode == 1) {
+                                for (uint32_t i = 0; i < cnt; ++i)
+                                        fn(i, s.equal_v);
+                        } else {
+                                s.mode = 0;
+                                for (uint32_t i = 0; i < cnt; ++i)
+                                        fn(i, s.next());
+                        }
+                } else {
+                        VbStream vb;
+                        vb.init(index + off);
+                        for (uint32_t i = 0; i < cnt; ++i) {
+                                const uint32_t d = vb.next();
+                                (void)vb.next();
+                                fn(i, d);
+                        }
+                }
+        } else {
+                DeltaStream<CODEC> s;
+                s.init(index, t, b, off);
+                for (uint32_t i = 0; i < cnt; ++i)
+                        fn(i, s.next());
+        }
+}
diff --git a/trinity_amd/csrc/dev_structs.hpp b/trinity_amd/csrc/dev_structs.hpp
--- a/trinity_amd/csrc/dev_structs.hpp
+++ b/trinity_amd/csrc/dev_structs.hpp
@@ -56,6 +56,8 @@
 constexpr uint32_t CAND_QUEUES = 8;
 constexpr uint32_t CAND_TICKET_STRIDE = 16;
 constexpr uint32_t CAND_HEAVY_TILES = 3;
+constexpr uint32_t CAND_PAIR_WORD = CAND_QUEUES + 1;
+constexpr uint32_t CAND_Q_WORDS = CAND_PAIR_WORD + 2 * CAND_QUEUES;
 constexpr uint32_t TASK_CAND = 0;
 constexpr uint32_t TASK_DENSE = 1;
 constexpr uint32_t TASK_FUSED = 2;
diff --git a/trinity_amd/csrc/host/plan_host.cpp b/trinity_amd/csrc/host/plan_host.cpp
--- a/trinity_amd/csrc/host/plan_host.cpp
+++ b/trinity_amd/csrc/host/plan_host.cpp
@@ -43,6 +43,10 @@
         bool use_frag_cache = false;
         for (unsigned i = 0; i < nopt; ++i) {
                 const std::string n = opt_names[i];
+                if (n == "filters") {
+                        env.filters = opt_values[i] != 0;
+                        continue;
+                }
                 if (n == "frag_cache") {
                         use_frag_cache = opt_values[i] != 0;
                         continue;
@@ -52,7 +56,7 @@
                                  : n == "fused_task_cost" ? &o.fused_task_cost : n == "fused_freq_cap" ? &o.fused_freq_cap : n == "fused_halfwords" ? &o.fused_halfwords
                                  : n == "account_needed_bytes" ? &o.account_needed_bytes : n == "planes" ? &o.planes : n == "planes_split" ? &o.planes_split
                                  : n == "plane_div" ? &o.plane_div : n == "plane_max_bytes" ? &o.plane_max_bytes : n == "probe_max_blocks" ? &o.probe_max_blocks : n == "tree_max_bytes" ? &o.tree_max_bytes : n == "tree_max_nodes" ? &o.tree_max_nodes : n == "tree_wide_min_nodes" ? &o.tree_wide_min_nodes : n == "result_bitmaps" ? &o.result_bitmaps : n == "cand_task_cost" ? &o.cand_task_cost : n == "dense_window_cost" ? &o.dense_window_cost
-                                 : n == "cand_xcd" ? &o.cand_xcd : n == "planes_order" ? &o.planes_order : n == "pset_order" ? &o.pset_order : n == "scatter_bitmap_slack" ? &o.scatter_bitmap_slack : n == "phrase_task_div" ? &o.phrase_task_div : n == "plane_amortize" ? &o.plane_amortize : n == "rich_max_terms" ? &o.rich_max_terms : nullptr;
+                                 : n == "cand_xcd" ? &o.cand_xcd : n == "and_pairs" ? &o.and_pairs : n == "planes_order" ? &o.planes_order : n == "pset_order" ? &o.pset_order : n == "scatter_bitmap_slack" ? &o.scatter_bitmap_slack : n == "phrase_task_div" ? &o.phrase_task_div : n == "plane_amortize" ? &o.plane_amortize : n == "rich_max_terms" ? &o.rich_max_terms : nullptr;
                 if (!slot) {
                         put_err(err, errcap, "unknown option " + n);
                         return nullptr;
@@ -105,8 +109,8 @@
                               P.unsupported_queries, P.rich_R,       sizeof(DevQuery),     sizeof(DevTask), sizeof(DevFused),     sizeof(DevPhrase),  P.cand_needed_term_bytes, P.plane_decoded_bytes,
                               P.n_pset,            P.pset_queries,   P.n_probe,            P.probe_queries, P.units.size(),       P.units.off,        P.pset_sched.off,     sizeof(DevPsetUnit),
                               P.n_tree,            P.tree_queries,   P.tree.size(),        P.tree.off,      P.tree_terms.size(),  P.tree_terms.off,   P.tree_hidden.size(), P.tree_hidden.off,
-                              P.cand_q.off};
-        static_assert(sizeof v / sizeof v[0] == 65, "summary layout");
+                              P.cand_q.off,        P.n_cand_pair};
+        static_assert(sizeof v / sizeof v[0] == 66, "summary layout");
         memcpy(out, v, sizeof v);
         if (ms)
                 memcpy(ms, P.plan_ms, sizeof P.plan_ms);
diff --git a/trinity_amd/csrc/k_match.hpp b/trinity_amd/csrc/k_match.hpp
--- a/trinity_amd/csrc/k_match.hpp
+++ b/trinity_amd/csrc/k_match.hpp
@@ -213,7 +213,7 @@
         return lo;
 }
 
-template <int CODEC>
+template <int CODEC, bool PAIRS = false>
 __device__ void and_filter_tile(AndShared &sh, const uint8_t *__restrict__ index, const uint32_t *__restrict__ blk_last,
                                 const uint32_t *__restrict__ blk_off, const uint32_t *__restrict__ win, const DevTerm t, const uint32_t C,
                                 const uint32_t lcur_slot, const bool block_driven PROF_ARG) {
@@ -924,7 +924,7 @@
 #define TRI_AND_PROBES 8
 #endif
 constexpr int AND_PROBES = TRI_AND_PROBES;
-template <int CODEC>
+template <int CODEC, bool PAIRS = false>
 #ifndef TRI_AND_WAVES
 #define TRI_AND_WAVES 4
 #endif
@@ -951,10 +951,18 @@
                                 const uint32_t x = (home + t) % CAND_QUEUES;
                                 if ((qdone >> x) & 1u)
                                         continue;
-                                const uint32_t q0 = cand_q[x], qn = cand_q[x + 1] - q0;
+                                uint32_t q0 = cand_q[x], qn = cand_q[x + 1] - q0;
+                                uint32_t pb = 0, pn = 0;
+                                if constexpr (PAIRS) {
+                                        pb = cand_q[CAND_PAIR_WORD + 2 * x], pn = cand_q[CAND_PAIR_WORD + 2 * x + 1] - pb;
+                                        qn -= pn;
+                                }
                                 const uint32_t old = uni(atomicAdd(ticket + x * CAND_TICKET_STRIDE, 1u)) >> 6;
-                                if (old < qn)
+                                if (old < qn) {
                                         got = q0 + old;
+                                        if constexpr (PAIRS)
+                                                got += pn && got >= pb ? pn : 0u;
+                                }
                                 else
                                         qdone |= 1u << x;
                         }
@@ -1054,7 +1062,7 @@
                                                 }
                                         }
                                 } else
-                                and_filter_tile<CODEC>(sh, index, blk_last, blk_off, win, t, C, k - 1, bd PROF_PASS);
+                                and_filter_tile<CODEC, PAIRS>(sh, index, blk_last, blk_off, win, t, C, k - 1, bd PROF_PASS);
                                 TRACE(4, slot, C);
                                 __syncthreads();
                                 TASKTIME(8 * ticket_no + 2 + min(k, 5u));
@@ -1157,3 +1165,140 @@
         PROF_FLUSH();
         TRACE(6, 0, 0);
 }
+
+
+#ifndef TRI_PAIR_BLOCKS
+#define TRI_PAIR_BLOCKS 128
+#endif
+constexpr uint32_t PAIR_BLOCKS = TRI_PAIR_BLOCKS;
+constexpr uint32_t PAIR_CANDS = PAIR_BLOCKS * 32;
+constexpr uint32_t PAIR_PER = PAIR_CANDS / AND_WG;
+static_assert(PAIR_BLOCKS >= 64 && PAIR_BLOCKS <= AND_WG && (PAIR_BLOCKS & (PAIR_BLOCKS - 1)) == 0, "a lane per lead block; a lane's candidates within one hit word");
+struct PairShared {
+        uint32_t cand[PAIR_CANDS];
+        alignas(8) uint32_t hit[PAIR_BLOCKS];
+        uint32_t scan[AND_WG / 64];
+        uint32_t bcast[4];
+};
+static_assert(PAIR_BLOCKS > 128 || sizeof(PairShared) < 20480, "eight workgroups per CU");
+#ifndef TRI_PAIR_WAVES
+#define TRI_PAIR_WAVES 8
+#endif
+template <int CODEC>
+__global__ __launch_bounds__(AND_WG, TRI_PAIR_WAVES) void k_and_pair(const uint8_t *__restrict__ index, const uint32_t *__restrict__ blk_last,
+                                                     const uint32_t *__restrict__ blk_off, const DevTerm *__restrict__ terms,
+                                                     const DevQuery *__restrict__ plan, const DevTask *__restrict__ tasks,
+                                                     const uint32_t *__restrict__ sched, const uint32_t *__restrict__ qterms,
+                                                     const uint32_t *__restrict__ pair_q, uint32_t *__restrict__ ticket,
+                                                     uint32_t *__restrict__ out, uint32_t *__restrict__ counts,
+                                                     const uint32_t *__restrict__ masked, const uint32_t *__restrict__ qplane,
+                                                     const uint32_t *__restrict__ planes, const uint32_t plw) {
+        __shared__ PairShared sh;
+        const uint32_t tid = threadIdx.x;
+        const uint32_t wave = uni(tid >> 6);
+        const uint32_t home = uni(__builtin_amdgcn_s_getreg(20 | (0 << 6) | (3 << 11))) % CAND_QUEUES;
+        uint32_t qdone = 0;
+        for (;;) {
+                if (wave == 0) {
+                        uint32_t got = 0xffffffffu;
+                        for (uint32_t t = 0; t < CAND_QUEUES && got == 0xffffffffu; ++t) {
+                                const uint32_t x = (home + t) % CAND_QUEUES;
+                                if ((qdone >> x) & 1u)
+                                        continue;
+                                const uint32_t q0 = pair_q[2 * x], qn = pair_q[2 * x + 1] - q0;
+                                const uint32_t old = qn ? uni(atomicAdd(ticket + x * CAND_TICKET_STRIDE, 1u)) >> 6 : 0u;
+                                if (old < qn)
+                                        got = q0 + old;
+                                else
+                                        qdone |= 1u << x;
+                        }
+                        sh.bcast[0] = got;
+                }
+                __syncthreads();
+                const uint32_t ticket_no = uni(sh.bcast[0]);
+                __syncthreads();
+                if (ticket_no == 0xffffffffu)
+                        break;
+                const uint32_t tix = sched[ticket_no];
+                const DevTask task = tasks[tix];
+                const DevQuery q = plan[task.slot];
+                const DevTerm lead = terms[qterms[q.term_base] & QT_TERM];
+                const bool neg = qterms[q.term_base + 1] & QT_NOT;
+                const uint32_t *pa = planes + (size_t)qplane[q.term_base + 1] * plw;
+                uint32_t *qout = out + task.out_off;
+                uint32_t produced = 0;
+                const uint32_t tb_end = min(lead.nblocks, task.tile_end * TILE_BLOCKS);
+                for (uint32_t tb = task.tile_begin * TILE_BLOCKS; tb < tb_end; tb += PAIR_BLOCKS) {
+                        const uint32_t nb = min(PAIR_BLOCKS, tb_end - tb);
+                        const uint32_t C = (tb + nb == lead.nblocks) ? (nb - 1) * 32 + lead.last_n : nb * 32;
+                        if (tid < nb) {
+                                const uint32_t b = tb + tid, gb = lead.first_block + b;
+                                const uint32_t off = blk_off[gb];
+                                const uint32_t n = TRI_BLOCK_N(lead, b, index, off);
+                                const uint32_t last = blk_last[gb];
+                                uint32_t doc = b ? blk_last[gb - 1] : 0;
+                                const uint32_t row = tid * 32;
+                                block_deltas<CODEC>(index, lead, b, off, n - 1, [&](const uint32_t i, const uint32_t delta) {
+                                        doc += delta;
+                                        sh.cand[row | ((i + tid) & 31u)] = doc;
+                                });
+                                sh.cand[row | ((n - 1 + tid) & 31u)] = last;
+                        }
+                        __syncthreads();
+                        const uint32_t lane = tid & 63u;
+                        for (uint32_t w0 = wave * 64; w0 < C; w0 += AND_WG * AND_PROBES) {
+                                uint32_t doc[AND_PROBES], w[AND_PROBES];
+#pragma unroll
+                                for (int u = 0; u < AND_PROBES; ++u) {
+                                        const uint32_t j = w0 + u * AND_WG + lane;
+                                        doc[u] = j < C ? sh.cand[phys(j)] : 0u;
+                                }
+#pragma unroll
+                                for (int u = 0; u < AND_PROBES; ++u)
+                                        w[u] = pa[doc[u] >> 5];
+#pragma unroll
+                                for (int u = 0; u < AND_PROBES; ++u) {
+                                        const uint32_t jw = w0 + u * AND_WG;
+                                        const uint64_t m = __ballot(jw + lane < C && ((w[u] >> (doc[u] & 31u)) & 1u));
+                                        if (jw < C && lane == 0)
+                                                *reinterpret_cast<uint64_t *>(&sh.hit[jw >> 5]) = m;
+                                }
+                        }
+                        __syncthreads();
+                        const uint32_t c0 = tid * PAIR_PER;
+                        const uint32_t left = C > c0 ? min(C - c0, PAIR_PER) : 0u;
+                        const uint32_t valid = left >= 32 ? 0xffffffffu : ((1u << left) - 1u);
+                        uint32_t bits = sh.hit[c0 >> 5] >> (c0 & 31u);
+                        bits = (neg ? ~bits : bits) & valid;
+                        if (masked)
+                                for (uint32_t m = bits; m;) {
+                                        const uint32_t kbit = __builtin_ctz(m);
+                                        m &= m - 1;
+                                        const uint32_t doc = sh.cand[phys(c0 + kbit)];
+                                        if ((masked[doc >> 5] >> (doc & 31u)) & 1u)
+                                                bits &= ~(1u << kbit);
+                                }
+                        uint32_t wtot;
+                        uint32_t ex = wave_excl_scan(__popc(bits), wtot);
+                        sh.scan[tid >> 6] = wtot;
+                        __syncthreads();
+                        uint32_t wbase = 0, total = 0;
+#pragma unroll
+                        for (int w = 0; w < AND_WG / 64; ++w) {
+                                if (w < (int)(tid >> 6))
+                                        wbase += sh.scan[w];
+                                total += sh.scan[w];
+                        }
+                        uint32_t o = produced + ex + wbase;
+                        for (uint32_t m = bits; m;) {
+                                const uint32_t kbit = __builtin_ctz(m);
+                                m &= m - 1;
+                                qout[o++] = sh.cand[phys(c0 + kbit)];
+                        }
+                        produced += uni(total);
+                        __syncthreads();
+                }
+                if (wave == 0)
+                        counts[tix] = produced;
+        }
+}
diff --git a/trinity_amd/csrc/planner.hpp b/trinity_amd/csrc/planner.hpp
--- a/trinity_amd/csrc/planner.hpp
+++ b/trinity_amd/csrc/planner.hpp
@@ -39,7 +39,7 @@
                 bool cand_rows = false;
                 std::vector<RowQ> rowq;
                 uint32_t pset_ranges = 0;
-                uint32_t cand_first = 0, cand_qat[CAND_QUEUES] = {};
+                uint32_t cand_first = 0, cand_qat[CAND_QUEUES] = {}, cand_pat[CAND_QUEUES] = {};
                 std::vector<uint32_t> unit_of_task;
                 ~PlanState() {
                         if (!cache)
@@ -221,7 +221,7 @@
                                         const uint32_t x = (uint32_t)(std::min_element(load, load + CAND_QUEUES) - load);
                                         load[x] += cand_row[r] / z.n;
                                         z.q[k] = (uint8_t)x;
-                                        z.sub[k] = (uint8_t)(CAND_COST_SUBS + placed[x]++ % (CAND_SUBS - CAND_COST_SUBS - 1));
+                                        z.sub[k] = (uint8_t)(CAND_COST_SUBS + placed[x]++ % (CAND_ROW_SUBS - CAND_COST_SUBS - 1));
                                 }
                         }
                 }
@@ -365,6 +365,10 @@
                 const uint32_t rb = S.pset_ranges <= PSET_RANGE_BKS ? std::min(range, PSET_RANGE_BKS - 1) : (uint32_t)std::min<uint64_t>((uint64_t)range * PSET_RANGE_BKS / S.pset_ranges, PSET_RANGE_BKS - 1);
                 return PSET_KEY0 + rb * PSET_SUBS + pset_sub((uint32_t)(f.tcost[i] >> 32));
         }
+        inline bool cand_pair_task(const PlanState &S, const DevQuery &q, const DevTask &tk) {
+                return S.opt.and_pairs && !S.env.filters && q.nterms == 2 && (S.P.qterms[q.term_base + 1] & QT_GROUP) && !S.P.qplane.empty() && S.P.qplane[q.term_base + 1] != PL_NONE &&
+                       tk.tile_end - tk.tile_begin <= CAND_HEAVY_TILES;
+        }
         inline uint32_t key_cand_rows(const PlanState &S, const Frag &f, const size_t i, const DevTask &tk) {
                 const DevQuery &q = S.P.plan[tk.slot];
                 uint32_t row = PL_NONE;
@@ -378,7 +382,9 @@
                         const uint32_t piece = (uint32_t)(f.b_tasks + i) % z.n;
                         queue = z.q[piece], sub = z.sub[piece];
                 } else
-                        queue = row % CAND_QUEUES, sub = CAND_SUBS - 1;
+                        queue = row % CAND_QUEUES, sub = CAND_ROW_SUBS - 1;
+                if (sub >= CAND_COST_SUBS && cand_pair_task(S, q, tk))
+                        sub += CAND_PAIR_SUB0;
                 return CAND_KEY0 + queue * CAND_SUBS + sub;
         }
         inline uint32_t schedule_key(const PlanState &S, const Frag &f, const size_t i) {
@@ -431,6 +437,8 @@
                                 for (uint32_t bk = CAND_KEY0; bk < PSET_KEY0; ++bk) {
                                         if ((bk - CAND_KEY0) % CAND_SUBS == 0)
                                                 S.cand_qat[(bk - CAND_KEY0) / CAND_SUBS] = at;
+                                        if ((bk - CAND_KEY0) % CAND_SUBS == CAND_PAIR_SUB0)
+                                                S.cand_pat[(bk - CAND_KEY0) / CAND_SUBS] = at;
                                         place(bk);
                                 }
                         for (uint32_t k = 0; k < TASK_KINDS; ++k)
@@ -482,9 +490,16 @@
                 BatchPlan &P = S.P;
                 const uint32_t nc = P.n_cand;
                 uint32_t *const sc = P.sched.p + S.cand_first;
+                std::fill(P.cand_q.p + CAND_PAIR_WORD, P.cand_q.p + CAND_Q_WORDS, 0u);
+                P.n_cand_pair = 0;
                 if (S.cand_rows) {
                         for (uint32_t x = 0; x <= CAND_QUEUES; ++x)
                                 P.cand_q[x] = x < CAND_QUEUES ? S.cand_qat[x] - S.cand_first : nc;
+                        for (uint32_t x = 0; x < CAND_QUEUES; ++x) {
+                                const uint32_t pb = S.cand_pat[x] - S.cand_first, pe = P.cand_q[x + 1];
+                                if (pe > pb)
+                                        P.cand_q[CAND_PAIR_WORD + 2 * x] = pb, P.cand_q[CAND_PAIR_WORD + 2 * x + 1] = pe, P.n_cand_pair += pe - pb;
+                        }
                 } else {
                         const std::vector<uint32_t> was(sc, sc + nc);
                         uint32_t pos = 0;
diff --git a/trinity_amd/csrc/planner_types.hpp b/trinity_amd/csrc/planner_types.hpp
--- a/trinity_amd/csrc/planner_types.hpp
+++ b/trinity_amd/csrc/planner_types.hpp
@@ -31,6 +31,7 @@
         uint64_t scatter_bitmap_slack = 4;
         uint64_t pset_order = 1;
         uint64_t cand_xcd = 1;
+        uint64_t and_pairs = 0;
         uint64_t plan_threads = 0;
         uint64_t plan_hot_us = 300;
         uint64_t plan_pin = 2;
@@ -47,6 +48,7 @@
         uint32_t cus = 256;
         uint32_t fus_wgs_per_cu = 2;
         uint32_t plk_wgs_per_cu = 2;
+        bool filters = false;
 };
 
 template <class T>
@@ -136,6 +138,7 @@
         uint64_t tree_scratch_bytes = 0;
         std::vector<uint32_t> slot_of_query;
         std::vector<int32_t> qstatus;
+        uint32_t n_cand_pair = 0;
         uint32_t n_dense = 0, n_pset = 0, n_probe = 0, n_cand = 0, n_fused = 0, n_fused16 = 0, n_fusedgen = 0, n_planes = 0, n_planes8 = 0;
         uint32_t plw = 0;
         uint32_t plane_rows = 0;
@@ -169,7 +172,7 @@
                 fn(P.ptasks, n.ptasks);
                 fn(P.units, n.units);
                 fn(P.pset_sched, n.units);
-                fn(P.cand_q, (size_t)CAND_QUEUES + 1);
+                fn(P.cand_q, (size_t)CAND_Q_WORDS);
                 fn(P.tree, n.tree);
                 fn(P.tree_terms, n.tree_terms);
                 fn(P.tree_hidden, n.tree_hidden);
@@ -192,7 +195,8 @@
         }
 
         constexpr uint32_t SCHED_NB = 64 * 4;
-        constexpr uint32_t CAND_SUBS = 128, CAND_COST_SUBS = 16;
+        constexpr uint32_t CAND_ROW_SUBS = 128, CAND_COST_SUBS = 16;
+        constexpr uint32_t CAND_PAIR_SUB0 = CAND_ROW_SUBS, CAND_SUBS = 2 * CAND_ROW_SUBS;
         constexpr uint32_t PSET_RANGE_BKS = 64, PSET_SUBS = 64;
         constexpr uint32_t CAND_KEY0 = TASK_KINDS * SCHED_NB, PSET_KEY0 = CAND_KEY0 + CAND_QUEUES * CAND_SUBS, SCHED_KEYS = PSET_KEY0 + PSET_RANGE_BKS * PSET_SUBS;
         inline uint32_t pset_sub(const uint32_t rank) { return rank < PSET_SUBS / 2 ? rank : std::min(PSET_SUBS / 2 + (rank - PSET_SUBS / 2) / 8, PSET_SUBS - 1); }
diff --git a/trinity_amd/csrc/trinity_hip.hip b/trinity_amd/csrc/trinity_hip.hip
--- a/trinity_amd/csrc/trinity_hip.hip
+++ b/trinity_amd/csrc/trinity_hip.hip
@@ -82,7 +82,8 @@
 static_assert(std::max({TICKET_DENSE_WORD, TICKET_PSET_WORD, TICKET_PROBE_WORD, TICKET_PLANES_WORD + 2, TICKET_SCORE_WORD, TICKET_RICH_COUNT_WORD + TICKET_RICH_WIDE, TICKET_RICH_WRITE_WORD + TICKET_RICH_WIDE,
                         TICKET_SCAT_WORD + 1, TICKET_PHRASE_WORD, TICKET_FUSED_WORD + 2 * 2}) < TICKET_CAND_WORD,
               "every kernel's ticket word lies below k_and's queues");
-constexpr size_t TICKET_BYTES = (TICKET_CAND_WORD + CAND_QUEUES * CAND_TICKET_STRIDE) * 4;
+constexpr size_t TICKET_PAIR_WORD = TICKET_CAND_WORD + CAND_QUEUES * CAND_TICKET_STRIDE;
+constexpr size_t TICKET_BYTES = (TICKET_PAIR_WORD + CAND_QUEUES * CAND_TICKET_STRIDE) * 4;
 constexpr size_t POOL_MIN_BYTES = 64u << 10;
 constexpr size_t POOL_IDLE_CAP = 64ull << 30;
 constexpr size_t PINNED_IDLE_MAX = 16;
@@ -487,6 +488,7 @@
                              {"plane_amortize", &tri_options::plane_amortize},
                              {"planes_rebuild", &tri_options::planes_rebuild},
                              {"cand_xcd", &tri_options::cand_xcd},
+                             {"and_pairs", &tri_options::and_pairs},
                              {"plan_threads", &tri_options::plan_threads},
                              {"probe_max_blocks", &tri_options::probe_max_blocks}, {"phrase_task_div", &tri_options::phrase_task_div}, {"plan_hot_us", &tri_options::plan_hot_us}, {"plan_pin", &tri_options::plan_pin}, {"planes_order", &tri_options::planes_order}, {"pset_order", &tri_options::pset_order}, {"scatter_bitmap_slack", &tri_options::scatter_bitmap_slack}, {"tree_max_bytes", &tri_options::tree_max_bytes}, {"tree_max_nodes", &tri_options::tree_max_nodes}, {"tree_wide_min_nodes", &tri_options::tree_wide_min_nodes}, {"rich_max_terms", &tri_options::rich_max_terms}, {"result_bitmaps", &tri_options::result_bitmaps}, {"cand_task_cost", &tri_options::cand_task_cost}, {"dense_window_cost", &tri_options::dense_window_cost}};
                 for (const auto &e : table)
@@ -1178,10 +1180,17 @@
                 HIP_TRY(hipGetLastError());
         }
         HIP_TRY(hipEventRecord(b->ev[EV_PROBE], dev->stream));
-        if (b->n_cand)
-                tri_launch_matching(b, FK_AND, 0, [](auto c) { return k_and<c.value>; }, dim3(std::min<uint32_t>(b->n_cand, (uint32_t)dev->cus * cand_wgs)), dim3(AND_WG), cand_stream, match_bytes, ix->d_blk_last, match_off,
+        const uint32_t n_pair = fsel.rows ? 0u : b->n_cand_pair, n_and = b->n_cand - n_pair;
+        const uint32_t *pair_q = n_pair ? b->dev_at(b->cand_q) + CAND_PAIR_WORD : nullptr;
+        if (n_and)
+                tri_launch_matching(b, FK_AND, 0, [&](auto c) { return n_pair ? k_and<c.value, true> : k_and<c.value, false>; }, dim3(std::min<uint32_t>(n_and, (uint32_t)dev->cus * cand_wgs)), dim3(AND_WG), cand_stream, match_bytes, ix->d_blk_last, match_off,
                            ix->d_win, ix->d_terms, b->dev_at(b->plan), b->dev_at(b->tasks), b->dev_at(b->sched) + trip::sched_first(*b, TASK_CAND), b->dev_at(b->qterms), b->dev_at(b->cand_q),
                            b->d_ticket + TICKET_CAND_WORD, b->d_out, b->d_counts, ix->d_masked, (const uint32_t *)b->dev_opt(b->qplane), (const uint32_t *)ix->d_pcache, b->plw);
+        HIP_TRY(hipGetLastError());
+        if (n_pair)
+                TRI_LAUNCH(k_and_pair, ix->codec, dim3(std::min<uint32_t>(n_pair, (uint32_t)dev->cus * TRI_PAIR_WAVES)), dim3(AND_WG), cand_stream, match_bytes, ix->d_blk_last, match_off, ix->d_terms,
+                           b->dev_at(b->plan), b->dev_at(b->tasks), b->dev_at(b->sched) + trip::sched_first(*b, TASK_CAND), b->dev_at(b->qterms), pair_q, b->d_ticket + TICKET_PAIR_WORD, b->d_out,
+                           b->d_counts, ix->d_masked, (const uint32_t *)b->dev_opt(b->qplane), (const uint32_t *)ix->d_pcache, b->plw);
         HIP_TRY(hipGetLastError());
         if (overlap) {
                 HIP_TRY(hipEventRecord(dev->ev_join, dev->stream2));
diff --git a/trinity_amd/hostplan.py b/trinity_amd/hostplan.py
--- a/trinity_amd/hostplan.py
+++ b/trinity_amd/hostplan.py
@@ -9,7 +9,7 @@
             "n_dense", "n_cand", "n_fused", "n_fused16", "n_fusedgen", "n_planes", "n_planes8", "plw", "sparse_cap", "out_capacity", "term_bytes", "term_bytes_dense",
             "dense_queries", "cand_queries", "fused_queries", "planes_queries", "unsupported_queries", "rich_R", "sizeof_query", "sizeof_task", "sizeof_fused", "sizeof_phrase",
             "cand_needed_term_bytes", "plane_decoded_bytes", "n_pset", "pset_queries", "n_probe", "probe_queries", "n_units", "off_units", "off_unit_sched", "sizeof_unit",
-            "n_tree", "tree_queries", "n_tree_words", "off_tree", "n_tree_terms", "off_tree_terms", "n_tree_hidden", "off_tree_hidden", "off_cand_q"]
+            "n_tree", "tree_queries", "n_tree_words", "off_tree", "n_tree_terms", "off_tree_terms", "n_tree_hidden", "off_tree_hidden", "off_cand_q", "n_cand_pair"]
 
 DEV_QUERY = np.dtype([("nterms", "<u4"), ("term_base", "<u4"), ("out_off", "<u8"), ("out_cap", "<u4"), ("qid", "<u4"), ("first_task", "<u4"), ("ntasks", "<u4"),
                       ("score_base", "<u4"), ("nscore", "<u4"), ("phrase_base", "<u4"), ("nphrases", "<u4"), ("fused_idx", "<u4"), ("form", "<u4")])
@@ -139,6 +139,10 @@
         return self._view("off_cand_q", 9, "<u4")
 
     @property
+    def cand_pair_q(self):
+        return self._view("off_cand_q", 9 + 16, "<u4")[9:].reshape(8, 2)
+
+    @property
     def qterms(self):
         return self._view("off_qterms", self.s["n_qterms"], "<u4")
 
```

Result: slower. 14.33 million (-1.6%).
